# DelphinusLab/halo2-gpu-specific

Hardware: AMD Instinct MI355X
Metric: NTT Fr-ops/s @ k=24 (forward+inverse 2^24 BN254 Fr NTT; MSM G1-adds/s under 'msm') (higher is better)
Workload: dtype u32x8 (254-bit Montgomery, integer)

## Files before the change

### halo2-gpu-specific_amd/csrc/field.hpp

```cpp
#pragma once
#ifdef __HIPCC_RTC__
typedef unsigned char uint8_t;
typedef unsigned short uint16_t;
typedef unsigned int uint32_t;
typedef unsigned long uint64_t;
typedef int int32_t;
typedef long int64_t;
#else
#include <hip/hip_runtime.h>
#include <stdint.h>
#endif

namespace h2 {

struct FrParams {
    static constexpr uint32_t MOD[8] = {0xf0000001u, 0x43e1f593u, 0x79b97091u, 0x2833e848u,
                                        0x8181585du, 0xb85045b6u, 0xe131a029u, 0x30644e72u};
    static constexpr uint32_t MOD2[8] = {0xe0000002u, 0x87c3eb27u, 0xf372e122u, 0x5067d090u,
                                         0x0302b0bau, 0x70a08b6du, 0xc2634053u, 0x60c89ce5u};
    static constexpr uint32_t NMOD[8] = {0x0fffffffu, 0xbc1e0a6cu, 0x86468f6eu, 0xd7cc17b7u,
                                         0x7e7ea7a2u, 0x47afba49u, 0x1ece5fd6u, 0xcf9bb18du};
    static constexpr uint32_t PINV256[8] = {0xefffffffu, 0xc2e1f593u, 0x4c6911b3u, 0x6586864bu,
                                         0x99062391u, 0xe39a9828u, 0x0d8341b2u, 0x73f82f1du};
    static constexpr uint32_t INV = 0xefffffffu;
    static constexpr uint32_t ONE[8] = {0x4ffffffbu, 0xac96341cu, 0x9f60cd29u, 0x36fc7695u,
                                        0x7879462eu, 0x666ea36fu, 0x9a07df2fu, 0x0e0a77c1u};
    static constexpr uint32_t RR[8] = {0xae216da7u, 0x1bb8e645u, 0xe35c59e3u, 0x53fe3ab1u,
                                       0x53bb8085u, 0x8c49833du, 0x7f4e44a5u, 0x0216d0b1u};
};

struct FqParams {
    static constexpr uint32_t MOD[8] = {0xd87cfd47u, 0x3c208c16u, 0x6871ca8du, 0x97816a91u,
                                        0x8181585du, 0xb85045b6u, 0xe131a029u, 0x30644e72u};
    static constexpr uint32_t MOD2[8] = {0xb0f9fa8eu, 0x7841182du, 0xd0e3951au, 0x2f02d522u,
                                         0x0302b0bbu, 0x70a08b6du, 0xc2634053u, 0x60c89ce5u};
    static constexpr uint32_t NMOD[8] = {0x278302b9u, 0xc3df73e9u, 0x978e3572u, 0x687e956eu,
                                         0x7e7ea7a2u, 0x47afba49u, 0x1ece5fd6u, 0xcf9bb18du};
    static constexpr uint32_t PINV256[8] = {0xe4866389u, 0x87d20782u, 0x1eca6ac9u, 0x9ede7d65u,
                                         0x1833da80u, 0xd8afcbd0u, 0x91888c6bu, 0xf57a22b7u};
    static constexpr uint32_t INV = 0xe4866389u;
    static constexpr uint32_t ONE[8] = {0xc58f0d9du, 0xd35d438du, 0xf5c70b3du, 0x0a78eb28u,
                                        0x7879462cu, 0x666ea36fu, 0x9a07df2fu, 0x0e0a77c1u};
    static constexpr uint32_t RR[8] = {0x538afa89u, 0xf32cfc5bu, 0xd44501fbu, 0xb5e71911u,
                                       0x0a417ff6u, 0x47ab1effu, 0xcab8351fu, 0x06d89f71u};
};

template <class P>
struct alignas(16) Fp {
    uint32_t l[8];
};
using Fr = Fp<FrParams>;
using Fq = Fp<FqParams>;

#define H2_DEV __host__ __device__ __forceinline__

template <class P>
H2_DEV Fp<P> fp_load(const Fp<P>* p) {
    const uint4* q = reinterpret_cast<const uint4*>(p);
    uint4 a = q[0], b = q[1];
    Fp<P> r;
    r.l[0] = a.x; r.l[1] = a.y; r.l[2] = a.z; r.l[3] = a.w;
    r.l[4] = b.x; r.l[5] = b.y; r.l[6] = b.z; r.l[7] = b.w;
    return r;
}
template <class P>
H2_DEV void fp_store(Fp<P>* p, const Fp<P>& v) {
    uint4* q = reinterpret_cast<uint4*>(p);
    q[0] = make_uint4(v.l[0], v.l[1], v.l[2], v.l[3]);
    q[1] = make_uint4(v.l[4], v.l[5], v.l[6], v.l[7]);
}

template <class P>
H2_DEV Fp<P> fp_zero() {
    Fp<P> r;
#pragma unroll
    for (int i = 0; i < 8; i++) r.l[i] = 0;
    return r;
}
template <class P>
H2_DEV Fp<P> fp_one() {
    Fp<P> r;
#pragma unroll
    for (int i = 0; i < 8; i++) r.l[i] = P::ONE[i];
    return r;
}
template <class P>
H2_DEV bool fp_is_zero(const Fp<P>& a) {
    uint32_t o = 0;
#pragma unroll
    for (int i = 0; i < 8; i++) o |= a.l[i];
    return o == 0;
}
template <class P>
H2_DEV bool fp_eq(const Fp<P>& a, const Fp<P>& b) {
    uint32_t o = 0;
#pragma unroll
    for (int i = 0; i < 8; i++) o |= a.l[i] ^ b.l[i];
    return o == 0;
}

#if defined(__HIP_DEVICE_COMPILE__) && !defined(H2_PORTABLE_MUL)
#define H2_ASM_CHAINS 1
H2_DEV uint32_t add_co(uint32_t a, uint32_t b, uint64_t& c) {
    uint32_t r;
    asm("v_add_co_u32 %0, %1, %2, %3" : "=v"(r), "=s"(c) : "v"(a), "v"(b));
    return r;
}
H2_DEV uint32_t addc_co(uint32_t a, uint32_t b, uint64_t& c) {
    uint32_t r;
    asm("v_addc_co_u32 %0, %1, %2, %3, %1" : "=v"(r), "+s"(c) : "v"(a), "v"(b));
    return r;
}
H2_DEV uint32_t sub_co(uint32_t a, uint32_t b, uint64_t& c) {
    uint32_t r;
    asm("v_sub_co_u32 %0, %1, %2, %3" : "=v"(r), "=s"(c) : "v"(a), "v"(b));
    return r;
}
H2_DEV uint32_t subb_co(uint32_t a, uint32_t b, uint64_t& c) {
    uint32_t r;
    asm("v_subb_co_u32 %0, %1, %2, %3, %1" : "=v"(r), "+s"(c) : "v"(a), "v"(b));
    return r;
}
H2_DEV uint32_t sel_co(uint32_t y, uint32_t x, uint64_t mask) {
    uint32_t r;
    asm("v_cndmask_b32 %0, %1, %2, %3" : "=v"(r) : "v"(y), "v"(x), "s"(mask));
    return r;
}
#endif

template <class P>
H2_DEV Fp<P> fp_reduce_once(const Fp<P>& a) {
#ifdef H2_ASM_CHAINS
    Fp<P> t, r;
    uint64_t cb;
    t.l[0] = sub_co(a.l[0], P::MOD[0], cb);
#pragma unroll
    for (int i = 1; i < 8; i++) t.l[i] = subb_co(a.l[i], P::MOD[i], cb);
#pragma unroll
    for (int i = 0; i < 8; i++) r.l[i] = sel_co(t.l[i], a.l[i], cb);
    return r;
#else
    Fp<P> d;
    uint64_t borrow = 0;
#pragma unroll
    for (int i = 0; i < 8; i++) {
        uint64_t t = (uint64_t)a.l[i] - P::MOD[i] - borrow;
        d.l[i] = (uint32_t)t;
        borrow = (t >> 32) & 1;
    }
    Fp<P> r;
#pragma unroll
    for (int i = 0; i < 8; i++) r.l[i] = borrow ? a.l[i] : d.l[i];
    return r;
#endif
}

template <class P>
H2_DEV Fp<P> fp_add(const Fp<P>& a, const Fp<P>& b) {
#ifdef H2_ASM_CHAINS
    Fp<P> s, t, r;
    uint64_t ca, cb;
    s.l[0] = add_co(a.l[0], b.l[0], ca);
    s.l[1] = addc_co(a.l[1], b.l[1], ca);
    t.l[0] = sub_co(s.l[0], P::MOD[0], cb);
#pragma unroll
    for (int i = 2; i < 8; i++) {
        s.l[i] = addc_co(a.l[i], b.l[i], ca);
        t.l[i - 1] = subb_co(s.l[i - 1], P::MOD[i - 1], cb);
    }
    t.l[7] = subb_co(s.l[7], P::MOD[7], cb);
#pragma unroll
    for (int i = 0; i < 8; i++) r.l[i] = sel_co(t.l[i], s.l[i], cb);
    return r;
#else
    Fp<P> s;
    uint64_t c = 0;
#pragma unroll
    for (int i = 0; i < 8; i++) {
        c += (uint64_t)a.l[i] + b.l[i];
        s.l[i] = (uint32_t)c;
        c >>= 32;
    }
    return fp_reduce_once(s);
#endif
}

template <class P>
H2_DEV Fp<P> fp_sub(const Fp<P>& a, const Fp<P>& b) {
#ifdef H2_ASM_CHAINS
    Fp<P> d, u, r;
    uint64_t ca, cb;
    d.l[0] = sub_co(a.l[0], b.l[0], ca);
    d.l[1] = subb_co(a.l[1], b.l[1], ca);
    u.l[0] = add_co(d.l[0], P::MOD[0], cb);
#pragma unroll
    for (int i = 2; i < 8; i++) {
        d.l[i] = subb_co(a.l[i], b.l[i], ca);
// ... 7 lines not shown
    Fp<P> d;
    uint64_t borrow = 0;
#pragma unroll
    for (int i = 0; i < 8; i++) {
        uint64_t t = (uint64_t)a.l[i] - b.l[i] - borrow;
        d.l[i] = (uint32_t)t;
        borrow = (t >> 32) & 1;
    }
    uint32_t mask = borrow ? 0xffffffffu : 0u;
    uint64_t c = 0;
    Fp<P> r;
#pragma unroll
    for (int i = 0; i < 8; i++) {
        c += (uint64_t)d.l[i] + (P::MOD[i] & mask);
        r.l[i] = (uint32_t)c;
        c >>= 32;
    }
    return r;
#endif
}

template <class P>
H2_DEV Fp<P> fp_neg(const Fp<P>& a) {
    return fp_sub(fp_zero<P>(), a);
}
template <class P>
H2_DEV Fp<P> fp_dbl(const Fp<P>& a) {
    return fp_add(a, a);
}

template <class P>
H2_DEV Fp<P> fp_lazy_red2p(const Fp<P>& a) {
#ifdef H2_ASM_CHAINS
    Fp<P> t, r;
    uint64_t cb;
    t.l[0] = sub_co(a.l[0], P::MOD2[0], cb);
#pragma unroll
    for (int i = 1; i < 8; i++) t.l[i] = subb_co(a.l[i], P::MOD2[i], cb);
#pragma unroll
    for (int i = 0; i < 8; i++) r.l[i] = sel_co(t.l[i], a.l[i], cb);
    return r;
#else
    Fp<P> d;
    uint64_t borrow = 0;
#pragma unroll
    for (int i = 0; i < 8; i++) {
        uint64_t t = (uint64_t)a.l[i] - P::MOD2[i] - borrow;
        d.l[i] = (uint32_t)t;
        borrow = (t >> 32) & 1;
    }
    Fp<P> r;
#pragma unroll
    for (int i = 0; i < 8; i++) r.l[i] = borrow ? a.l[i] : d.l[i];
    return r;
#endif
}
template <class P>
H2_DEV Fp<P> fp_lazy_add(const Fp<P>& a, const Fp<P>& b) {
    Fp<P> s;
#ifdef H2_ASM_CHAINS
    uint64_t c;
    s.l[0] = add_co(a.l[0], b.l[0], c);
#pragma unroll
    for (int i = 1; i < 8; i++) s.l[i] = addc_co(a.l[i], b.l[i], c);
#else
    uint64_t c = 0;
#pragma unroll
    for (int i = 0; i < 8; i++) {
        c += (uint64_t)a.l[i] + b.l[i];
        s.l[i] = (uint32_t)c;
        c >>= 32;
    }
#endif
    return s;
}
template <class P>
H2_DEV Fp<P> fp_lazy_sub(const Fp<P>& a, const Fp<P>& b) {
    Fp<P> d, u;
#ifdef H2_ASM_CHAINS
    uint64_t ca, cb;
    d.l[0] = sub_co(a.l[0], b.l[0], ca);
    d.l[1] = subb_co(a.l[1], b.l[1], ca);
    u.l[0] = add_co(d.l[0], P::MOD2[0], cb);
#pragma unroll
    for (int i = 2; i < 8; i++) {
        d.l[i] = subb_co(a.l[i], b.l[i], ca);
        u.l[i - 1] = addc_co(d.l[i - 1], P::MOD2[i - 1], cb);
    }
    u.l[7] = addc_co(d.l[7], P::MOD2[7], cb);
#else
    uint64_t borrow = 0, c = 0;
#pragma unroll
    for (int i = 0; i < 8; i++) {
        uint64_t t = (uint64_t)a.l[i] - b.l[i] - borrow;
        d.l[i] = (uint32_t)t;
        borrow = (t >> 32) & 1;
    }
#pragma unroll
    for (int i = 0; i < 8; i++) {
        c += (uint64_t)d.l[i] + P::MOD2[i];
        u.l[i] = (uint32_t)c;
        c >>= 32;
    }
#endif
    return u;
}
template <class P>
H2_DEV Fp<P> fp_lazy_add_red(const Fp<P>& a, const Fp<P>& b) {
#ifdef H2_ASM_CHAINS
    Fp<P> s, t, r;
    uint64_t ca, cb;
    s.l[0] = add_co(a.l[0], b.l[0], ca);
    s.l[1] = addc_co(a.l[1], b.l[1], ca);
    t.l[0] = sub_co(s.l[0], P::MOD2[0], cb);
#pragma unroll
    for (int i = 2; i < 8; i++) {
        s.l[i] = addc_co(a.l[i], b.l[i], ca);
        t.l[i - 1] = subb_co(s.l[i - 1], P::MOD2[i - 1], cb);
    }
    t.l[7] = subb_co(s.l[7], P::MOD2[7], cb);
#pragma unroll
    for (int i = 0; i < 8; i++) r.l[i] = sel_co(t.l[i], s.l[i], cb);
    return r;
#else
    return fp_lazy_red2p(fp_lazy_add(a, b));
#endif
}
template <class P>
H2_DEV Fp<P> fp_lazy_sub_red(const Fp<P>& a, const Fp<P>& b) {
#ifdef H2_ASM_CHAINS
    Fp<P> d, u, r;
    uint64_t ca, cb;
    d.l[0] = sub_co(a.l[0], b.l[0], ca);
    d.l[1] = subb_co(a.l[1], b.l[1], ca);
    u.l[0] = add_co(d.l[0], P::MOD2[0], cb);
#pragma unroll
    for (int i = 2; i < 8; i++) {
        d.l[i] = subb_co(a.l[i], b.l[i], ca);
        u.l[i - 1] = addc_co(d.l[i - 1], P::MOD2[i - 1], cb);
    }
    u.l[7] = addc_co(d.l[7], P::MOD2[7], cb);
#pragma unroll
    for (int i = 0; i < 8; i++) r.l[i] = sel_co(d.l[i], u.l[i], ca);
    return r;
#else
    return fp_lazy_red2p(fp_lazy_sub(a, b));
#endif
}
template <class P>
H2_DEV Fp<P> fp_lazy_canon(const Fp<P>& a) {
    return fp_reduce_once(fp_lazy_red2p(a));
}

H2_DEV void mad_acc(uint64_t& lo, uint32_t& hi, uint32_t a, uint32_t b) {
#if defined(H2_PORTABLE_MUL) || !defined(__HIP_DEVICE_COMPILE__)
    uint64_t p = (uint64_t)a * b;
    uint64_t s = lo + p;
    hi += (s < p) ? 1u : 0u;
    lo = s;
#else
    uint64_t carry;
    asm("v_mad_u64_u32 %0, %1, %2, %3, %0" : "+v"(lo), "=s"(carry) : "v"(a), "v"(b));
    asm("v_addc_co_u32 %0, %1, %0, 0, %1" : "+v"(hi), "+s"(carry));
#endif
}

template <class P>
__device__ __forceinline__ Fp<P> fp_mul_dev(const Fp<P>& a, const Fp<P>& b);
template <class P>
__device__ __forceinline__ Fp<P> fp_sqr_dev(const Fp<P>& a);
template <class P>
__device__ __forceinline__ Fp<P> fp_mul2_dev(const Fp<P>& a, const Fp<P>& b, const Fp<P>& c, const Fp<P>& d);
template <class P>
__device__ __forceinline__ Fp<P> fp_mul_wide_dev(const Fp<P>& a, const Fp<P>& b);
template <class P>
__device__ __forceinline__ Fp<P> fp_mul_const_dev(const Fp<P>& a, const Fp<P>& w, const Fp<P>& wq);
#if defined(__HIP_DEVICE_COMPILE__) && !defined(H2_PORTABLE_MUL)
#include "fp_mul_gen.hpp"
#endif

template <class P>
H2_DEV Fp<P> fp_mul(const Fp<P>& a, const Fp<P>& b) {
#if !defined(__HIP_DEVICE_COMPILE__)
    {
        typedef unsigned __int128 u128;
        uint64_t x[4], y[4], p[4];
        for (int i = 0; i < 4; i++) {
            x[i] = (uint64_t)a.l[2 * i] | ((uint64_t)a.l[2 * i + 1] << 32);
            y[i] = (uint64_t)b.l[2 * i] | ((uint64_t)b.l[2 * i + 1] << 32);
            p[i] = (uint64_t)P::MOD[2 * i] | ((uint64_t)P::MOD[2 * i + 1] << 32);
        }
        uint64_t inv = p[0];
        for (int i = 0; i < 6; i++) inv *= 2 - p[0] * inv;
        inv = 0 - inv;
        uint64_t t[6] = {0, 0, 0, 0, 0, 0};
        for (int i = 0; i < 4; i++) {
            u128 c = 0;
            for (int j = 0; j < 4; j++) {
                c += (u128)t[j] + (u128)x[j] * y[i];
                t[j] = (uint64_t)c;
                c >>= 64;
            }
            c += t[4];
            t[4] = (uint64_t)c;
            t[5] = (uint64_t)(c >> 64);
            const uint64_t m = t[0] * inv;
            c = ((u128)t[0] + (u128)m * p[0]) >> 64;
            for (int j = 1; j < 4; j++) {
                c += (u128)t[j] + (u128)m * p[j];
                t[j - 1] = (uint64_t)c;
                c >>= 64;
            }
            c += t[4];
            t[3] = (uint64_t)c;
            t[4] = t[5] + (uint64_t)(c >> 64);
        }
        Fp<P> r;
        for (int i = 0; i < 4; i++) {
            r.l[2 * i] = (uint32_t)t[i];
            r.l[2 * i + 1] = (uint32_t)(t[i] >> 32);
        }
        return fp_reduce_once(r);
    }
#elif !defined(H2_PORTABLE_MUL)
    return fp_mul_dev(a, b);
#endif
    Fp<P> r;
    uint64_t lo = 0;
    uint32_t hi = 0;
    uint32_t m[8];
#pragma unroll
    for (int i = 0; i < 8; i++) {
#pragma unroll
        for (int j = 0; j <= i; j++) mad_acc(lo, hi, a.l[j], b.l[i - j]);
#pragma unroll
        for (int j = 0; j < i; j++) mad_acc(lo, hi, m[j], P::MOD[i - j]);
        m[i] = (uint32_t)lo * P::INV;
        mad_acc(lo, hi, m[i], P::MOD[0]);
        lo = (lo >> 32) | ((uint64_t)hi << 32);
        hi = 0;
    }
#pragma unroll
    for (int i = 8; i < 16; i++) {
#pragma unroll
        for (int j = i - 7; j < 8; j++) mad_acc(lo, hi, a.l[j], b.l[i - j]);
#pragma unroll
        for (int j = i - 7; j < 8; j++) mad_acc(lo, hi, m[j], P::MOD[i - j]);
        r.l[i - 8] = (uint32_t)lo;
        lo = (lo >> 32) | ((uint64_t)hi << 32);
        hi = 0;
    }
    return fp_reduce_once(r);
}

template <class P>
H2_DEV Fp<P> fp_sqr(const Fp<P>& a) {
#if defined(__HIP_DEVICE_COMPILE__) && !defined(H2_PORTABLE_MUL) && !defined(H2_NO_SQR)
    return fp_sqr_dev(a);
#else
    return fp_mul(a, a);
#endif
}

template <class P>
H2_DEV Fp<P> fp_mul2(const Fp<P>& a, const Fp<P>& b, const Fp<P>& c, const Fp<P>& d) {
#if defined(__HIP_DEVICE_COMPILE__) && !defined(H2_PORTABLE_MUL) && !defined(H2_NO_MUL2)
    return fp_mul2_dev(a, b, c, d);
#else
    return fp_add(fp_mul(a, b), fp_mul(c, d));
#endif
}

template <class P>
H2_DEV Fp<P> fp_mul_wide(const Fp<P>& a, const Fp<P>& b) {
#if defined(__HIP_DEVICE_COMPILE__) && !defined(H2_PORTABLE_MUL)
    return fp_mul_wide_dev(a, b);
#else
    Fp<P> r;
    uint64_t lo = 0;
    uint32_t hi = 0;
    uint32_t m[8];
    for (int i = 0; i < 8; i++) {
        for (int j = 0; j <= i; j++) mad_acc(lo, hi, a.l[j], b.l[i - j]);
        for (int j = 0; j < i; j++) mad_acc(lo, hi, m[j], P::MOD[i - j]);
        m[i] = (uint32_t)lo * P::INV;
        mad_acc(lo, hi, m[i], P::MOD[0]);
        lo = (lo >> 32) | ((uint64_t)hi << 32);
        hi = 0;
    }
    for (int i = 8; i < 16; i++) {
        for (int j = i - 7; j < 8; j++) mad_acc(lo, hi, a.l[j], b.l[i - j]);
        for (int j = i - 7; j < 8; j++) mad_acc(lo, hi, m[j], P::MOD[i - j]);
        r.l[i - 8] = (uint32_t)lo;
        lo = (lo >> 32) | ((uint64_t)hi << 32);
        hi = 0;
    }
    return r;
#endif
}

template <class P>
H2_DEV Fp<P> fp_mul_const(const Fp<P>& x, const Fp<P>& w, const Fp<P>& wq) {
#if defined(__HIP_DEVICE_COMPILE__) && !defined(H2_PORTABLE_MUL)
    Fp<P> r = fp_mul_const_dev(x, w, wq);
    if (__builtin_expect(r.l[7] >= P::MOD2[7], 0)) r = fp_lazy_red2p(r);
    return r;
#else
    uint32_t q[8];
    {
        uint64_t lo = 0;
        uint32_t hi = 0;
        for (int i = 0; i < 15; i++) {
            for (int j = (i > 7 ? i - 7 : 0); j <= (i < 7 ? i : 7); j++) mad_acc(lo, hi, x.l[j], wq.l[i - j]);
            if (i >= 8) q[i - 8] = (uint32_t)lo;
            lo = (lo >> 32) | ((uint64_t)hi << 32);
            hi = 0;
        }
        q[7] = (uint32_t)lo;
    }
    Fp<P> r;
    uint64_t lo = 0;
    uint32_t hi = 0;
    for (int i = 0; i < 8; i++) {
        for (int j = 0; j <= i; j++) {
            mad_acc(lo, hi, x.l[j], w.l[i - j]);
            mad_acc(lo, hi, q[j], P::NMOD[i - j]);
        }
        r.l[i] = (uint32_t)lo;
        lo = (lo >> 32) | ((uint64_t)hi << 32);
        hi = 0;
    }
    return r;
#endif
}
template <class P>
H2_DEV void fp_const_pair(const Fp<P>& w_mont, Fp<P>& w_plain, Fp<P>& wq) {
    w_plain = fp_from_mont(w_mont);
    uint64_t lo = 0;
    uint32_t hi = 0;
    for (int i = 0; i < 8; i++) {
        for (int j = 0; j <= i; j++) mad_acc(lo, hi, w_mont.l[j], P::PINV256[i - j]);
        wq.l[i] = (uint32_t)lo;
        lo = (lo >> 32) | ((uint64_t)hi << 32);
        hi = 0;
    }
}

template <class P>
H2_DEV Fp<P> fp_to_mont(const Fp<P>& canon) {
    Fp<P> rr;
#pragma unroll
    for (int i = 0; i < 8; i++) rr.l[i] = P::RR[i];
    return fp_reduce_once(fp_mul_wide(canon, rr));
}
template <class P>
H2_DEV Fp<P> fp_from_mont(const Fp<P>& a) {
    Fp<P> one = fp_zero<P>();
    one.l[0] = 1;
    return fp_reduce_once(fp_mul_wide(a, one));
}

template <class P>
H2_DEV Fp<P> fp_inv(const Fp<P>& a) {
    uint32_t u[8], v[8], r[8], s[8];
    uint32_t nz = 0;
#pragma unroll
    for (int i = 0; i < 8; i++) {
        u[i] = P::MOD[i];
        v[i] = a.l[i];
        r[i] = 0;
        s[i] = i == 0 ? 1u : 0u;
        nz |= a.l[i];
    }
    if (nz == 0) return a;
    uint32_t k = 0;
    auto halve = [](uint32_t* x) {
#pragma unroll
        for (int i = 0; i < 8; i++) x[i] = (x[i] >> 1) | (i < 7 ? x[i + 1] << 31 : 0u);
    };
    auto dbl = [](uint32_t* x) {
#pragma unroll
        for (int i = 7; i >= 0; i--) x[i] = (x[i] << 1) | (i ? x[i - 1] >> 31 : 0u);
    };
    auto sub = [](uint32_t* x, const uint32_t* y) {
        uint32_t bw = 0;
#pragma unroll
        for (int i = 0; i < 8; i++) {
            const uint32_t d = x[i] - y[i], b1 = x[i] < y[i] ? 1u : 0u, e = d - bw, b2 = d < bw ? 1u : 0u;
            x[i] = e;
            bw = b1 | b2;
        }
    };
    auto add = [](uint32_t* x, const uint32_t* y) {
        uint32_t cy = 0;
#pragma unroll
        for (int i = 0; i < 8; i++) {
            const uint32_t t = x[i] + y[i], c1 = t < y[i] ? 1u : 0u, e = t + cy, c2 = e < cy ? 1u : 0u;
            x[i] = e;
            cy = c1 | c2;
        }
    };
    auto greater = [](const uint32_t* x, const uint32_t* y) {
#pragma unroll
        for (int i = 7; i >= 0; i--)
            if (x[i] != y[i]) return x[i] > y[i];
        return false;
    };
    for (;;) {
        uint32_t vnz = 0;
#pragma unroll
        for (int i = 0; i < 8; i++) vnz |= v[i];
        if (vnz == 0) break;
        if ((u[0] & 1) == 0) {
            halve(u);
            dbl(s);
        } else if ((v[0] & 1) == 0) {
            halve(v);
            dbl(r);
        } else if (greater(u, v)) {
            sub(u, v);
            halve(u);
            add(r, s);
            dbl(s);
        } else {
            sub(v, u);
            halve(v);
            add(s, r);
            dbl(r);
        }
        k++;
    }
    Fp<P> x;
    {
        uint32_t d[8];
        uint64_t bw = 0;
#pragma unroll
        for (int i = 0; i < 8; i++) {
            uint64_t e = (uint64_t)r[i] - P::MOD[i] - bw;
            d[i] = (uint32_t)e;
            bw = (e >> 32) & 1;
        }
        uint64_t bw2 = 0;
#pragma unroll
        for (int i = 0; i < 8; i++) {
            const uint32_t rr = bw ? r[i] : d[i];
            uint64_t e = (uint64_t)P::MOD[i] - rr - bw2;
            x.l[i] = (uint32_t)e;
            bw2 = (e >> 32) & 1;
        }
    }
    x = fp_reduce_once(x);
    for (uint32_t i = k; i < 512; i++) x = fp_dbl(x);
    return x;
}

template <class P>
H2_DEV Fp<P> fp_pow_u32(const Fp<P>& a, uint32_t e) {
    if (e == 0) return fp_one<P>();
    Fp<P> acc = a;
    for (int i = 30 - __builtin_clz(e); i >= 0; i--) {
        acc = fp_sqr(acc);
        if ((e >> i) & 1) acc = fp_mul(acc, a);
    }
    return acc;
}

}
```

### halo2-gpu-specific_amd/csrc/fp_mul_gen.hpp

```cpp

template <>
__device__ __forceinline__ Fp<FrParams> fp_mul_dev<FrParams>(const Fp<FrParams>& a, const Fp<FrParams>& b) {
    using P = FrParams;
    Fp<P> r;
    uint64_t lo = 0, cy0, cy1, cy2;
    uint32_t hi = 0;
    asm("v_mad_u64_u32 %[lo], %[cy0], %[x0], %[x1], %[lo]\n\t"
        : [lo] "+v"(lo), [cy0] "=&s"(cy0)
        : [x0] "v"(a.l[0]), [x1] "v"(b.l[0]));
    const uint32_t m0 = (uint32_t)lo * P::INV;
    asm("v_mad_u64_u32 %[lo], %[cy0], %[x0], %[x1], %[lo]\n\t"
        "s_nop 1\n\t"
        "v_cndmask_b32 %[hi], 0, 1, %[cy0]\n\t"
        : [lo] "+v"(lo), [hi] "=&v"(hi), [cy0] "=&s"(cy0)
        : [x0] "v"(m0), [x1] "s"(P::MOD[0]));
    lo = (lo >> 32) | ((uint64_t)hi << 32);
    asm("v_mad_u64_u32 %[lo], %[cy0], %[x0], %[x1], %[lo]\n\t"
        "v_mad_u64_u32 %[lo], %[cy1], %[x2], %[x3], %[lo]\n\t"
        "v_mad_u64_u32 %[lo], %[cy2], %[x4], %[x5], %[lo]\n\t"
        "s_nop 0\n\t"
        "v_cndmask_b32 %[hi], 0, 1, %[cy1]\n\t"
        "v_addc_co_u32 %[hi], %[cy2], %[hi], 0, %[cy2]\n\t"
        : [lo] "+v"(lo), [hi] "=&v"(hi), [cy0] "=&s"(cy0), [cy1] "=&s"(cy1), [cy2] "=&s"(cy2)
        : [x0] "v"(m0), [x1] "s"(P::MOD[1]), [x2] "v"(a.l[0]), [x3] "v"(b.l[1]), [x4] "v"(a.l[1]), [x5] "v"(b.l[0]));
// ... 1508 lines not shown
        : [x0] "v"(q0), [x1] "s"(P::NMOD[0]), [x2] "v"(a.l[0]), [x3] "v"(b.l[0]));
    r.l[0] = (uint32_t)lo;
    lo = (lo >> 32) | ((uint64_t)hi << 32);
    asm("v_mad_u64_u32 %[lo], %[cy0], %[x0], %[x1], %[lo]\n\t"
        "v_mad_u64_u32 %[lo], %[cy1], %[x2], %[x3], %[lo]\n\t"
        "v_mad_u64_u32 %[lo], %[cy2], %[x4], %[x5], %[lo]\n\t"
        "v_mad_u64_u32 %[lo], %[cy0], %[x6], %[x7], %[lo]\n\t"
        "s_nop 0\n\t"
        "v_cndmask_b32 %[hi], 0, 1, %[cy2]\n\t"
        "v_addc_co_u32 %[hi], %[cy0], %[hi], 0, %[cy0]\n\t"
        : [lo] "+v"(lo), [hi] "=&v"(hi), [cy0] "=&s"(cy0), [cy1] "=&s"(cy1), [cy2] "=&s"(cy2)
        : [x0] "v"(q1), [x1] "s"(P::NMOD[0]), [x2] "v"(q0), [x3] "s"(P::NMOD[1]), [x4] "v"(a.l[0]), [x5] "v"(b.l[1]), [x6] "v"(a.l[1]), [x7] "v"(b.l[0]));
    r.l[1] = (uint32_t)lo;
    lo = (lo >> 32) | ((uint64_t)hi << 32);
    asm("v_mad_u64_u32 %[lo], %[cy0], %[x0], %[x1], %[lo]\n\t"
        "v_mad_u64_u32 %[lo], %[cy1], %[x2], %[x3], %[lo]\n\t"
        "v_mad_u64_u32 %[lo], %[cy2], %[x4], %[x5], %[lo]\n\t"
        "v_mad_u64_u32 %[lo], %[cy0], %[x6], %[x7], %[lo]\n\t"
        "v_mad_u64_u32 %[lo], %[cy1], %[x8], %[x9], %[lo]\n\t"
        "v_cndmask_b32 %[hi], 0, 1, %[cy2]\n\t"
        "v_addc_co_u32 %[hi], %[cy0], %[hi], 0, %[cy0]\n\t"
        "v_addc_co_u32 %[hi], %[cy1], %[hi], 0, %[cy1]\n\t"
        "v_mad_u64_u32 %[lo], %[cy2], %[x10], %[x11], %[lo]\n\t"
        "s_nop 1\n\t"
        "v_addc_co_u32 %[hi], %[cy2], %[hi], 0, %[cy2]\n\t"
        : [lo] "+v"(lo), [hi] "=&v"(hi), [cy0] "=&s"(cy0), [cy1] "=&s"(cy1), [cy2] "=&s"(cy2)
        : [x0] "v"(q2), [x1] "s"(P::NMOD[0]), [x2] "v"(q0), [x3] "s"(P::NMOD[2]), [x4] "v"(q1), [x5] "s"(P::NMOD[1]), [x6] "v"(a.l[0]), [x7] "v"(b.l[2]), [x8] "v"(a.l[1]), [x9] "v"(b.l[1]), [x10] "v"(a.l[2]), [x11] "v"(b.l[0]));
    r.l[2] = (uint32_t)lo;
    lo = (lo >> 32) | ((uint64_t)hi << 32);
    asm("v_mad_u64_u32 %[lo], %[cy0], %[x0], %[x1], %[lo]\n\t"
        "v_mad_u64_u32 %[lo], %[cy1], %[x2], %[x3], %[lo]\n\t"
        "v_mad_u64_u32 %[lo], %[cy2], %[x4], %[x5], %[lo]\n\t"
        "v_mad_u64_u32 %[lo], %[cy0], %[x6], %[x7], %[lo]\n\t"
        "v_mad_u64_u32 %[lo], %[cy1], %[x8], %[x9], %[lo]\n\t"
        "v_cndmask_b32 %[hi], 0, 1, %[cy2]\n\t"
        "v_addc_co_u32 %[hi], %[cy0], %[hi], 0, %[cy0]\n\t"
        "v_addc_co_u32 %[hi], %[cy1], %[hi], 0, %[cy1]\n\t"
        "v_mad_u64_u32 %[lo], %[cy2], %[x10], %[x11], %[lo]\n\t"
        "v_mad_u64_u32 %[lo], %[cy0], %[x12], %[x13], %[lo]\n\t"
        "v_mad_u64_u32 %[lo], %[cy1], %[x14], %[x15], %[lo]\n\t"
        "v_addc_co_u32 %[hi], %[cy2], %[hi], 0, %[cy2]\n\t"
        "v_addc_co_u32 %[hi], %[cy0], %[hi], 0, %[cy0]\n\t"
        "v_addc_co_u32 %[hi], %[cy1], %[hi], 0, %[cy1]\n\t"
        : [lo] "+v"(lo), [hi] "=&v"(hi), [cy0] "=&s"(cy0), [cy1] "=&s"(cy1), [cy2] "=&s"(cy2)
        : [x0] "v"(q3), [x1] "s"(P::NMOD[0]), [x2] "v"(q1), [x3] "s"(P::NMOD[2]), [x4] "v"(q2), [x5] "s"(P::NMOD[1]), [x6] "v"(q0), [x7] "s"(P::NMOD[3]), [x8] "v"(a.l[0]), [x9] "v"(b.l[3]), [x10] "v"(a.l[1]), [x11] "v"(b.l[2]), [x12] "v"(a.l[2]), [x13] "v"(b.l[1]), [x14] "v"(a.l[3]), [x15] "v"(b.l[0]));
    r.l[3] = (uint32_t)lo;
    lo = (lo >> 32) | ((uint64_t)hi << 32);
    asm("v_mad_u64_u32 %[lo], %[cy0], %[x0], %[x1], %[lo]\n\t"
        "v_mad_u64_u32 %[lo], %[cy1], %[x2], %[x3], %[lo]\n\t"
        "v_mad_u64_u32 %[lo], %[cy2], %[x4], %[x5], %[lo]\n\t"
        "v_mad_u64_u32 %[lo], %[cy0], %[x6], %[x7], %[lo]\n\t"
        "v_mad_u64_u32 %[lo], %[cy1], %[x8], %[x9], %[lo]\n\t"
        "v_cndmask_b32 %[hi], 0, 1, %[cy2]\n\t"
        "v_addc_co_u32 %[hi], %[cy0], %[hi], 0, %[cy0]\n\t"
        "v_addc_co_u32 %[hi], %[cy1], %[hi], 0, %[cy1]\n\t"
        "v_mad_u64_u32 %[lo], %[cy2], %[x10], %[x11], %[lo]\n\t"
        "v_mad_u64_u32 %[lo], %[cy0], %[x12], %[x13], %[lo]\n\t"
        "v_mad_u64_u32 %[lo], %[cy1], %[x14], %[x15], %[lo]\n\t"
        "v_addc_co_u32 %[hi], %[cy2], %[hi], 0, %[cy2]\n\t"
        "v_addc_co_u32 %[hi], %[cy0], %[hi], 0, %[cy0]\n\t"
        "v_addc_co_u32 %[hi], %[cy1], %[hi], 0, %[cy1]\n\t"
        "v_mad_u64_u32 %[lo], %[cy2], %[x16], %[x17], %[lo]\n\t"
        "v_mad_u64_u32 %[lo], %[cy0], %[x18], %[x19], %[lo]\n\t"
        "s_nop 0\n\t"
        "v_addc_co_u32 %[hi], %[cy2], %[hi], 0, %[cy2]\n\t"
        "v_addc_co_u32 %[hi], %[cy0], %[hi], 0, %[cy0]\n\t"
        : [lo] "+v"(lo), [hi] "=&v"(hi), [cy0] "=&s"(cy0), [cy1] "=&s"(cy1), [cy2] "=&s"(cy2)
        : [x0] "v"(q4), [x1] "s"(P::NMOD[0]), [x2] "v"(q0), [x3] "s"(P::NMOD[4]), [x4] "v"(q2), [x5] "s"(P::NMOD[2]), [x6] "v"(q3), [x7] "s"(P::NMOD[1]), [x8] "v"(q1), [x9] "s"(P::NMOD[3]), [x10] "v"(a.l[0]), [x11] "v"(b.l[4]), [x12] "v"(a.l[1]), [x13] "v"(b.l[3]), [x14] "v"(a.l[2]), [x15] "v"(b.l[2]), [x16] "v"(a.l[3]), [x17] "v"(b.l[1]), [x18] "v"(a.l[4]), [x19] "v"(b.l[0]));
    r.l[4] = (uint32_t)lo;
    lo = (lo >> 32) | ((uint64_t)hi << 32);
    asm("v_mad_u64_u32 %[lo], %[cy0], %[x0], %[x1], %[lo]\n\t"
        "v_mad_u64_u32 %[lo], %[cy1], %[x2], %[x3], %[lo]\n\t"
        "v_mad_u64_u32 %[lo], %[cy2], %[x4], %[x5], %[lo]\n\t"
        "v_mad_u64_u32 %[lo], %[cy0], %[x6], %[x7], %[lo]\n\t"
        "v_mad_u64_u32 %[lo], %[cy1], %[x8], %[x9], %[lo]\n\t"
        "v_mad_u64_u32 %[lo], %[cy2], %[x10], %[x11], %[lo]\n\t"
        "v_cndmask_b32 %[hi], 0, 1, %[cy0]\n\t"
        "v_addc_co_u32 %[hi], %[cy1], %[hi], 0, %[cy1]\n\t"
        "v_addc_co_u32 %[hi], %[cy2], %[hi], 0, %[cy2]\n\t"
        "v_mad_u64_u32 %[lo], %[cy0], %[x12], %[x13], %[lo]\n\t"
        "v_mad_u64_u32 %[lo], %[cy1], %[x14], %[x15], %[lo]\n\t"
        "v_mad_u64_u32 %[lo], %[cy2], %[x16], %[x17], %[lo]\n\t"
        "v_addc_co_u32 %[hi], %[cy0], %[hi], 0, %[cy0]\n\t"
        "v_addc_co_u32 %[hi], %[cy1], %[hi], 0, %[cy1]\n\t"
        "v_addc_co_u32 %[hi], %[cy2], %[hi], 0, %[cy2]\n\t"
        "v_mad_u64_u32 %[lo], %[cy0], %[x18], %[x19], %[lo]\n\t"
        "v_mad_u64_u32 %[lo], %[cy1], %[x20], %[x21], %[lo]\n\t"
        "v_mad_u64_u32 %[lo], %[cy2], %[x22], %[x23], %[lo]\n\t"
        "v_addc_co_u32 %[hi], %[cy0], %[hi], 0, %[cy0]\n\t"
        "v_addc_co_u32 %[hi], %[cy1], %[hi], 0, %[cy1]\n\t"
        "v_addc_co_u32 %[hi], %[cy2], %[hi], 0, %[cy2]\n\t"
        : [lo] "+v"(lo), [hi] "=&v"(hi), [cy0] "=&s"(cy0), [cy1] "=&s"(cy1), [cy2] "=&s"(cy2)
        : [x0] "v"(q5), [x1] "s"(P::NMOD[0]), [x2] "v"(q0), [x3] "s"(P::NMOD[5]), [x4] "v"(q1), [x5] "s"(P::NMOD[4]), [x6] "v"(q3), [x7] "s"(P::NMOD[2]), [x8] "v"(q4), [x9] "s"(P::NMOD[1]), [x10] "v"(q2), [x11] "s"(P::NMOD[3]), [x12] "v"(a.l[0]), [x13] "v"(b.l[5]), [x14] "v"(a.l[1]), [x15] "v"(b.l[4]), [x16] "v"(a.l[2]), [x17] "v"(b.l[3]), [x18] "v"(a.l[3]), [x19] "v"(b.l[2]), [x20] "v"(a.l[4]), [x21] "v"(b.l[1]), [x22] "v"(a.l[5]), [x23] "v"(b.l[0]));
    r.l[5] = (uint32_t)lo;
    lo = (lo >> 32) | ((uint64_t)hi << 32);
    asm("v_mad_u64_u32 %[lo], %[cy0], %[x0], %[x1], %[lo]\n\t"
        "v_mad_u64_u32 %[lo], %[cy1], %[x2], %[x3], %[lo]\n\t"
        "v_mad_u64_u32 %[lo], %[cy2], %[x4], %[x5], %[lo]\n\t"
        "v_mad_u64_u32 %[lo], %[cy0], %[x6], %[x7], %[lo]\n\t"
        "v_mad_u64_u32 %[lo], %[cy1], %[x8], %[x9], %[lo]\n\t"
        "v_mad_u64_u32 %[lo], %[cy2], %[x10], %[x11], %[lo]\n\t"
        "v_mad_u64_u32 %[lo], %[cy0], %[x12], %[x13], %[lo]\n\t"
        "v_cndmask_b32 %[hi], 0, 1, %[cy1]\n\t"
        "v_addc_co_u32 %[hi], %[cy2], %[hi], 0, %[cy2]\n\t"
        "v_addc_co_u32 %[hi], %[cy0], %[hi], 0, %[cy0]\n\t"
        "v_mad_u64_u32 %[lo], %[cy1], %[x14], %[x15], %[lo]\n\t"
        "v_mad_u64_u32 %[lo], %[cy2], %[x16], %[x17], %[lo]\n\t"
        "v_mad_u64_u32 %[lo], %[cy0], %[x18], %[x19], %[lo]\n\t"
        "v_addc_co_u32 %[hi], %[cy1], %[hi], 0, %[cy1]\n\t"
        "v_addc_co_u32 %[hi], %[cy2], %[hi], 0, %[cy2]\n\t"
        "v_addc_co_u32 %[hi], %[cy0], %[hi], 0, %[cy0]\n\t"
        "v_mad_u64_u32 %[lo], %[cy1], %[x20], %[x21], %[lo]\n\t"
        "v_mad_u64_u32 %[lo], %[cy2], %[x22], %[x23], %[lo]\n\t"
        "s_nop 0\n\t"
        "v_addc_co_u32 %[hi], %[cy1], %[hi], 0, %[cy1]\n\t"
        "v_addc_co_u32 %[hi], %[cy2], %[hi], 0, %[cy2]\n\t"
        : [lo] "+v"(lo), [hi] "=&v"(hi), [cy0] "=&s"(cy0), [cy1] "=&s"(cy1), [cy2] "=&s"(cy2)
        : [x0] "v"(q6), [x1] "s"(P::NMOD[0]), [x2] "v"(q0), [x3] "s"(P::NMOD[6]), [x4] "v"(q1), [x5] "s"(P::NMOD[5]), [x6] "v"(q2), [x7] "s"(P::NMOD[4]), [x8] "v"(q4), [x9] "s"(P::NMOD[2]), [x10] "v"(q5), [x11] "s"(P::NMOD[1]), [x12] "v"(q3), [x13] "s"(P::NMOD[3]), [x14] "v"(a.l[0]), [x15] "v"(b.l[6]), [x16] "v"(a.l[1]), [x17] "v"(b.l[5]), [x18] "v"(a.l[2]), [x19] "v"(b.l[4]), [x20] "v"(a.l[3]), [x21] "v"(b.l[3]), [x22] "v"(a.l[4]), [x23] "v"(b.l[2]));
    asm("v_mad_u64_u32 %[lo], %[cy0], %[x0], %[x1], %[lo]\n\t"
        "v_mad_u64_u32 %[lo], %[cy1], %[x2], %[x3], %[lo]\n\t"
        "s_nop 0\n\t"
        "v_addc_co_u32 %[hi], %[cy0], %[hi], 0, %[cy0]\n\t"
        "v_addc_co_u32 %[hi], %[cy1], %[hi], 0, %[cy1]\n\t"
        : [lo] "+v"(lo), [hi] "+v"(hi), [cy0] "=&s"(cy0), [cy1] "=&s"(cy1)
        : [x0] "v"(a.l[5]), [x1] "v"(b.l[1]), [x2] "v"(a.l[6]), [x3] "v"(b.l[0]));
    r.l[6] = (uint32_t)lo;
    lo = (lo >> 32) | ((uint64_t)hi << 32);
    asm("v_mad_u64_u32 %[lo], %[cy0], %[x0], %[x1], %[lo]\n\t"
        "v_mad_u64_u32 %[lo], %[cy1], %[x2], %[x3], %[lo]\n\t"
        "v_mad_u64_u32 %[lo], %[cy2], %[x4], %[x5], %[lo]\n\t"
        "v_mad_u64_u32 %[lo], %[cy0], %[x6], %[x7], %[lo]\n\t"
        "v_mad_u64_u32 %[lo], %[cy1], %[x8], %[x9], %[lo]\n\t"
        "v_mad_u64_u32 %[lo], %[cy2], %[x10], %[x11], %[lo]\n\t"
        "v_mad_u64_u32 %[lo], %[cy0], %[x12], %[x13], %[lo]\n\t"
        "v_mad_u64_u32 %[lo], %[cy1], %[x14], %[x15], %[lo]\n\t"
        "v_mad_u64_u32 %[lo], %[cy2], %[x16], %[x17], %[lo]\n\t"
        "v_mad_u64_u32 %[lo], %[cy0], %[x18], %[x19], %[lo]\n\t"
        "v_mad_u64_u32 %[lo], %[cy1], %[x20], %[x21], %[lo]\n\t"
        "v_mad_u64_u32 %[lo], %[cy2], %[x22], %[x23], %[lo]\n\t"
        : [lo] "+v"(lo), [cy0] "=&s"(cy0), [cy1] "=&s"(cy1), [cy2] "=&s"(cy2)
        : [x0] "v"(q7), [x1] "s"(P::NMOD[0]), [x2] "v"(q1), [x3] "s"(P::NMOD[6]), [x4] "v"(a.l[0]), [x5] "v"(b.l[7]), [x6] "v"(q2), [x7] "s"(P::NMOD[5]), [x8] "v"(q3), [x9] "s"(P::NMOD[4]), [x10] "v"(q5), [x11] "s"(P::NMOD[2]), [x12] "v"(q6), [x13] "s"(P::NMOD[1]), [x14] "v"(q0), [x15] "s"(P::NMOD[7]), [x16] "v"(q4), [x17] "s"(P::NMOD[3]), [x18] "v"(a.l[1]), [x19] "v"(b.l[6]), [x20] "v"(a.l[2]), [x21] "v"(b.l[5]), [x22] "v"(a.l[3]), [x23] "v"(b.l[4]));
    asm("v_mad_u64_u32 %[lo], %[cy0], %[x0], %[x1], %[lo]\n\t"
        "v_mad_u64_u32 %[lo], %[cy1], %[x2], %[x3], %[lo]\n\t"
        "v_mad_u64_u32 %[lo], %[cy2], %[x4], %[x5], %[lo]\n\t"
        "v_mad_u64_u32 %[lo], %[cy0], %[x6], %[x7], %[lo]\n\t"
        : [lo] "+v"(lo), [cy0] "=&s"(cy0), [cy1] "=&s"(cy1), [cy2] "=&s"(cy2)
        : [x0] "v"(a.l[4]), [x1] "v"(b.l[3]), [x2] "v"(a.l[5]), [x3] "v"(b.l[2]), [x4] "v"(a.l[6]), [x5] "v"(b.l[1]), [x6] "v"(a.l[7]), [x7] "v"(b.l[0]));
    r.l[7] = (uint32_t)lo;
    (void)cy0; (void)cy1; (void)cy2; (void)hi;
    return r;
}

template <>
__device__ __forceinline__ Fp<FqParams> fp_mul_dev<FqParams>(const Fp<FqParams>& a, const Fp<FqParams>& b) {
    using P = FqParams;
    Fp<P> r;
    uint64_t lo = 0, cy0, cy1, cy2;
    uint32_t hi = 0;
    asm("v_mad_u64_u32 %[lo], %[cy0], %[x0], %[x1], %[lo]\n\t"
        : [lo] "+v"(lo), [cy0] "=&s"(cy0)
        : [x0] "v"(a.l[0]), [x1] "v"(b.l[0]));
    const uint32_t m0 = (uint32_t)lo * P::INV;
    asm("v_mad_u64_u32 %[lo], %[cy0], %[x0], %[x1], %[lo]\n\t"
        "s_nop 1\n\t"
        "v_cndmask_b32 %[hi], 0, 1, %[cy0]\n\t"
        : [lo] "+v"(lo), [hi] "=&v"(hi), [cy0] "=&s"(cy0)
        : [x0] "v"(m0), [x1] "s"(P::MOD[0]));
    lo = (lo >> 32) | ((uint64_t)hi << 32);
    asm("v_mad_u64_u32 %[lo], %[cy0], %[x0], %[x1], %[lo]\n\t"
        "v_mad_u64_u32 %[lo], %[cy1], %[x2], %[x3], %[lo]\n\t"
        "v_mad_u64_u32 %[lo], %[cy2], %[x4], %[x5], %[lo]\n\t"
        "s_nop 0\n\t"
        "v_cndmask_b32 %[hi], 0, 1, %[cy1]\n\t"
        "v_addc_co_u32 %[hi], %[cy2], %[hi], 0, %[cy2]\n\t"
        : [lo] "+v"(lo), [hi] "=&v"(hi), [cy0] "=&s"(cy0), [cy1] "=&s"(cy1), [cy2] "=&s"(cy2)
        : [x0] "v"(m0), [x1] "s"(P::MOD[1]), [x2] "v"(a.l[0]), [x3] "v"(b.l[1]), [x4] "v"(a.l[1]), [x5] "v"(b.l[0]));
    const uint32_t m1 = (uint32_t)lo * P::INV;
    asm("v_mad_u64_u32 %[lo], %[cy0], %[x0], %[x1], %[lo]\n\t"
        "s_nop 1\n\t"
        "v_addc_co_u32 %[hi], %[cy0], %[hi], 0, %[cy0]\n\t"
        : [lo] "+v"(lo), [hi] "+v"(hi), [cy0] "=&s"(cy0)
        : [x0] "v"(m1), [x1] "s"(P::MOD[0]));
    lo = (lo >> 32) | ((uint64_t)hi << 32);
    asm("v_mad_u64_u32 %[lo], %[cy0], %[x0], %[x1], %[lo]\n\t"
        "v_mad_u64_u32 %[lo], %[cy1], %[x2], %[x3], %[lo]\n\t"
        "v_mad_u64_u32 %[lo], %[cy2], %[x4], %[x5], %[lo]\n\t"
        "v_mad_u64_u32 %[lo], %[cy0], %[x6], %[x7], %[lo]\n\t"
        "v_mad_u64_u32 %[lo], %[cy1], %[x8], %[x9], %[lo]\n\t"
        "v_cndmask_b32 %[hi], 0, 1, %[cy2]\n\t"
        "v_addc_co_u32 %[hi], %[cy0], %[hi], 0, %[cy0]\n\t"
        "v_addc_co_u32 %[hi], %[cy1], %[hi], 0, %[cy1]\n\t"
        : [lo] "+v"(lo), [hi] "=&v"(hi), [cy0] "=&s"(cy0), [cy1] "=&s"(cy1), [cy2] "=&s"(cy2)
        : [x0] "v"(m1), [x1] "s"(P::MOD[1]), [x2] "v"(m0), [x3] "s"(P::MOD[2]), [x4] "v"(a.l[0]), [x5] "v"(b.l[2]), [x6] "v"(a.l[1]), [x7] "v"(b.l[1]), [x8] "v"(a.l[2]), [x9] "v"(b.l[0]));
    const uint32_t m2 = (uint32_t)lo * P::INV;
    asm("v_mad_u64_u32 %[lo], %[cy0], %[x0], %[x1], %[lo]\n\t"
        "s_nop 1\n\t"
        "v_addc_co_u32 %[hi], %[cy0], %[hi], 0, %[cy0]\n\t"
        : [lo] "+v"(lo), [hi] "+v"(hi), [cy0] "=&s"(cy0)
        : [x0] "v"(m2), [x1] "s"(P::MOD[0]));
    lo = (lo >> 32) | ((uint64_t)hi << 32);
    asm("v_mad_u64_u32 %[lo], %[cy0], %[x0], %[x1], %[lo]\n\t"
        "v_mad_u64_u32 %[lo], %[cy1], %[x2], %[x3], %[lo]\n\t"
        "v_mad_u64_u32 %[lo], %[cy2], %[x4], %[x5], %[lo]\n\t"
        "v_mad_u64_u32 %[lo], %[cy0], %[x6], %[x7], %[lo]\n\t"
        "v_mad_u64_u32 %[lo], %[cy1], %[x8], %[x9], %[lo]\n\t"
        "v_cndmask_b32 %[hi], 0, 1, %[cy2]\n\t"
        "v_addc_co_u32 %[hi], %[cy0], %[hi], 0, %[cy0]\n\t"
        "v_addc_co_u32 %[hi], %[cy1], %[hi], 0, %[cy1]\n\t"
        "v_mad_u64_u32 %[lo], %[cy2], %[x10], %[x11], %[lo]\n\t"
        "v_mad_u64_u32 %[lo], %[cy0], %[x12], %[x13], %[lo]\n\t"
        "s_nop 0\n\t"
        "v_addc_co_u32 %[hi], %[cy2], %[hi], 0, %[cy2]\n\t"
        "v_addc_co_u32 %[hi], %[cy0], %[hi], 0, %[cy0]\n\t"
        : [lo] "+v"(lo), [hi] "=&v"(hi), [cy0] "=&s"(cy0), [cy1] "=&s"(cy1), [cy2] "=&s"(cy2)
        : [x0] "v"(m2), [x1] "s"(P::MOD[1]), [x2] "v"(m1), [x3] "s"(P::MOD[2]), [x4] "v"(m0), [x5] "s"(P::MOD[3]), [x6] "v"(a.l[0]), [x7] "v"(b.l[3]), [x8] "v"(a.l[1]), [x9] "v"(b.l[2]), [x10] "v"(a.l[2]), [x11] "v"(b.l[1]), [x12] "v"(a.l[3]), [x13] "v"(b.l[0]));
    const uint32_t m3 = (uint32_t)lo * P::INV;
    asm("v_mad_u64_u32 %[lo], %[cy0], %[x0], %[x1], %[lo]\n\t"
        "s_nop 1\n\t"
        "v_addc_co_u32 %[hi], %[cy0], %[hi], 0, %[cy0]\n\t"
        : [lo] "+v"(lo), [hi] "+v"(hi), [cy0] "=&s"(cy0)
        : [x0] "v"(m3), [x1] "s"(P::MOD[0]));
    lo = (lo >> 32) | ((uint64_t)hi << 32);
    asm("v_mad_u64_u32 %[lo], %[cy0], %[x0], %[x1], %[lo]\n\t"
        "v_mad_u64_u32 %[lo], %[cy1], %[x2], %[x3], %[lo]\n\t"
        "v_mad_u64_u32 %[lo], %[cy2], %[x4], %[x5], %[lo]\n\t"
        "v_mad_u64_u32 %[lo], %[cy0], %[x6], %[x7], %[lo]\n\t"
        "v_mad_u64_u32 %[lo], %[cy1], %[x8], %[x9], %[lo]\n\t"
        "v_cndmask_b32 %[hi], 0, 1, %[cy2]\n\t"
        "v_addc_co_u32 %[hi], %[cy0], %[hi], 0, %[cy0]\n\t"
        "v_addc_co_u32 %[hi], %[cy1], %[hi], 0, %[cy1]\n\t"
        "v_mad_u64_u32 %[lo], %[cy2], %[x10], %[x11], %[lo]\n\t"
        "v_mad_u64_u32 %[lo], %[cy0], %[x12], %[x13], %[lo]\n\t"
        "v_mad_u64_u32 %[lo], %[cy1], %[x14], %[x15], %[lo]\n\t"
        "v_addc_co_u32 %[hi], %[cy2], %[hi], 0, %[cy2]\n\t"
        "v_addc_co_u32 %[hi], %[cy0], %[hi], 0, %[cy0]\n\t"
        "v_addc_co_u32 %[hi], %[cy1], %[hi], 0, %[cy1]\n\t"
        "v_mad_u64_u32 %[lo], %[cy2], %[x16], %[x17], %[lo]\n\t"
        "s_nop 1\n\t"
        "v_addc_co_u32 %[hi], %[cy2], %[hi], 0, %[cy2]\n\t"
        : [lo] "+v"(lo), [hi] "=&v"(hi), [cy0] "=&s"(cy0), [cy1] "=&s"(cy1), [cy2] "=&s"(cy2)
        : [x0] "v"(m3), [x1] "s"(P::MOD[1]), [x2] "v"(m2), [x3] "s"(P::MOD[2]), [x4] "v"(m0), [x5] "s"(P::MOD[4]), [x6] "v"(m1), [x7] "s"(P::MOD[3]), [x8] "v"(a.l[0]), [x9] "v"(b.l[4]), [x10] "v"(a.l[1]), [x11] "v"(b.l[3]), [x12] "v"(a.l[2]), [x13] "v"(b.l[2]), [x14] "v"(a.l[3]), [x15] "v"(b.l[1]), [x16] "v"(a.l[4]), [x17] "v"(b.l[0]));
    const uint32_t m4 = (uint32_t)lo * P::INV;
    asm("v_mad_u64_u32 %[lo], %[cy0], %[x0], %[x1], %[lo]\n\t"
        "s_nop 1\n\t"
        "v_addc_co_u32 %[hi], %[cy0], %[hi], 0, %[cy0]\n\t"
        : [lo] "+v"(lo), [hi] "+v"(hi), [cy0] "=&s"(cy0)
        : [x0] "v"(m4), [x1] "s"(P::MOD[0]));
    lo = (lo >> 32) | ((uint64_t)hi << 32);
    asm("v_mad_u64_u32 %[lo], %[cy0], %[x0], %[x1], %[lo]\n\t"
        "v_mad_u64_u32 %[lo], %[cy1], %[x2], %[x3], %[lo]\n\t"
        "v_mad_u64_u32 %[lo], %[cy2], %[x4], %[x5], %[lo]\n\t"
        "v_mad_u64_u32 %[lo], %[cy0], %[x6], %[x7], %[lo]\n\t"
        "v_mad_u64_u32 %[lo], %[cy1], %[x8], %[x9], %[lo]\n\t"
        "v_cndmask_b32 %[hi], 0, 1, %[cy2]\n\t"
        "v_addc_co_u32 %[hi], %[cy0], %[hi], 0, %[cy0]\n\t"
        "v_addc_co_u32 %[hi], %[cy1], %[hi], 0, %[cy1]\n\t"
        "v_mad_u64_u32 %[lo], %[cy2], %[x10], %[x11], %[lo]\n\t"
        "v_mad_u64_u32 %[lo], %[cy0], %[x12], %[x13], %[lo]\n\t"
        "v_mad_u64_u32 %[lo], %[cy1], %[x14], %[x15], %[lo]\n\t"
        "v_addc_co_u32 %[hi], %[cy2], %[hi], 0, %[cy2]\n\t"
        "v_addc_co_u32 %[hi], %[cy0], %[hi], 0, %[cy0]\n\t"
        "v_addc_co_u32 %[hi], %[cy1], %[hi], 0, %[cy1]\n\t"
        "v_mad_u64_u32 %[lo], %[cy2], %[x16], %[x17], %[lo]\n\t"
        "v_mad_u64_u32 %[lo], %[cy0], %[x18], %[x19], %[lo]\n\t"
        "v_mad_u64_u32 %[lo], %[cy1], %[x20], %[x21], %[lo]\n\t"
        "v_addc_co_u32 %[hi], %[cy2], %[hi], 0, %[cy2]\n\t"
        "v_addc_co_u32 %[hi], %[cy0], %[hi], 0, %[cy0]\n\t"
        "v_addc_co_u32 %[hi], %[cy1], %[hi], 0, %[cy1]\n\t"
        : [lo] "+v"(lo), [hi] "=&v"(hi), [cy0] "=&s"(cy0), [cy1] "=&s"(cy1), [cy2] "=&s"(cy2)
        : [x0] "v"(m4), [x1] "s"(P::MOD[1]), [x2] "v"(m3), [x3] "s"(P::MOD[2]), [x4] "v"(m1), [x5] "s"(P::MOD[4]), [x6] "v"(m2), [x7] "s"(P::MOD[3]), [x8] "v"(m0), [x9] "s"(P::MOD[5]), [x10] "v"(a.l[0]), [x11] "v"(b.l[5]), [x12] "v"(a.l[1]), [x13] "v"(b.l[4]), [x14] "v"(a.l[2]), [x15] "v"(b.l[3]), [x16] "v"(a.l[3]), [x17] "v"(b.l[2]), [x18] "v"(a.l[4]), [x19] "v"(b.l[1]), [x20] "v"(a.l[5]), [x21] "v"(b.l[0]));
    const uint32_t m5 = (uint32_t)lo * P::INV;
    asm("v_mad_u64_u32 %[lo], %[cy0], %[x0], %[x1], %[lo]\n\t"
        "s_nop 1\n\t"
        "v_addc_co_u32 %[hi], %[cy0], %[hi], 0, %[cy0]\n\t"
        : [lo] "+v"(lo), [hi] "+v"(hi), [cy0] "=&s"(cy0)
        : [x0] "v"(m5), [x1] "s"(P::MOD[0]));
    lo = (lo >> 32) | ((uint64_t)hi << 32);
    asm("v_mad_u64_u32 %[lo], %[cy0], %[x0], %[x1], %[lo]\n\t"
        "v_mad_u64_u32 %[lo], %[cy1], %[x2], %[x3], %[lo]\n\t"
        "v_mad_u64_u32 %[lo], %[cy2], %[x4], %[x5], %[lo]\n\t"
        "v_mad_u64_u32 %[lo], %[cy0], %[x6], %[x7], %[lo]\n\t"
        "v_mad_u64_u32 %[lo], %[cy1], %[x8], %[x9], %[lo]\n\t"
        "v_cndmask_b32 %[hi], 0, 1, %[cy2]\n\t"
        "v_addc_co_u32 %[hi], %[cy0], %[hi], 0, %[cy0]\n\t"
        "v_addc_co_u32 %[hi], %[cy1], %[hi], 0, %[cy1]\n\t"
        "v_mad_u64_u32 %[lo], %[cy2], %[x10], %[x11], %[lo]\n\t"
        "v_mad_u64_u32 %[lo], %[cy0], %[x12], %[x13], %[lo]\n\t"
        "v_mad_u64_u32 %[lo], %[cy1], %[x14], %[x15], %[lo]\n\t"
        "v_addc_co_u32 %[hi], %[cy2], %[hi], 0, %[cy2]\n\t"
        "v_addc_co_u32 %[hi], %[cy0], %[hi], 0, %[cy0]\n\t"
        "v_addc_co_u32 %[hi], %[cy1], %[hi], 0, %[cy1]\n\t"
        "v_mad_u64_u32 %[lo], %[cy2], %[x16], %[x17], %[lo]\n\t"
        "v_mad_u64_u32 %[lo], %[cy0], %[x18], %[x19], %[lo]\n\t"
        "v_mad_u64_u32 %[lo], %[cy1], %[x20], %[x21], %[lo]\n\t"
        "v_addc_co_u32 %[hi], %[cy2], %[hi], 0, %[cy2]\n\t"
        "v_addc_co_u32 %[hi], %[cy0], %[hi], 0, %[cy0]\n\t"
        "v_addc_co_u32 %[hi], %[cy1], %[hi], 0, %[cy1]\n\t"
        "v_mad_u64_u32 %[lo], %[cy2], %[x22], %[x23], %[lo]\n\t"
        "s_nop 1\n\t"
        "v_addc_co_u32 %[hi], %[cy2], %[hi], 0, %[cy2]\n\t"
        : [lo] "+v"(lo), [hi] "=&v"(hi), [cy0] "=&s"(cy0), [cy1] "=&s"(cy1), [cy2] "=&s"(cy2)
        : [x0] "v"(m5), [x1] "s"(P::MOD[1]), [x2] "v"(m4), [x3] "s"(P::MOD[2]), [x4] "v"(m2), [x5] "s"(P::MOD[4]), [x6] "v"(m3), [x7] "s"(P::MOD[3]), [x8] "v"(m1), [x9] "s"(P::MOD[5]), [x10] "v"(m0), [x11] "s"(P::MOD[6]), [x12] "v"(a.l[0]), [x13] "v"(b.l[6]), [x14] "v"(a.l[1]), [x15] "v"(b.l[5]), [x16] "v"(a.l[2]), [x17] "v"(b.l[4]), [x18] "v"(a.l[3]), [x19] "v"(b.l[3]), [x20] "v"(a.l[4]), [x21] "v"(b.l[2]), [x22] "v"(a.l[5]), [x23] "v"(b.l[1]));
    asm("v_mad_u64_u32 %[lo], %[cy0], %[x0], %[x1], %[lo]\n\t"
        "s_nop 1\n\t"
        "v_addc_co_u32 %[hi], %[cy0], %[hi], 0, %[cy0]\n\t"
        : [lo] "+v"(lo), [hi] "+v"(hi), [cy0] "=&s"(cy0)
// ... 1398 lines not shown
        "v_cndmask_b32 %[hi], 0, 1, %[cy1]\n\t"
        : [lo] "+v"(lo), [hi] "=&v"(hi), [cy0] "=&s"(cy0), [cy1] "=&s"(cy1)
        : [x0] "v"(q0), [x1] "s"(P::NMOD[0]), [x2] "v"(a.l[0]), [x3] "v"(b.l[0]));
    r.l[0] = (uint32_t)lo;
    lo = (lo >> 32) | ((uint64_t)hi << 32);
    asm("v_mad_u64_u32 %[lo], %[cy0], %[x0], %[x1], %[lo]\n\t"
        "v_mad_u64_u32 %[lo], %[cy1], %[x2], %[x3], %[lo]\n\t"
        "v_mad_u64_u32 %[lo], %[cy2], %[x4], %[x5], %[lo]\n\t"
        "v_mad_u64_u32 %[lo], %[cy0], %[x6], %[x7], %[lo]\n\t"
        "s_nop 0\n\t"
        "v_cndmask_b32 %[hi], 0, 1, %[cy2]\n\t"
        "v_addc_co_u32 %[hi], %[cy0], %[hi], 0, %[cy0]\n\t"
        : [lo] "+v"(lo), [hi] "=&v"(hi), [cy0] "=&s"(cy0), [cy1] "=&s"(cy1), [cy2] "=&s"(cy2)
        : [x0] "v"(q1), [x1] "s"(P::NMOD[0]), [x2] "v"(q0), [x3] "s"(P::NMOD[1]), [x4] "v"(a.l[0]), [x5] "v"(b.l[1]), [x6] "v"(a.l[1]), [x7] "v"(b.l[0]));
    r.l[1] = (uint32_t)lo;
    lo = (lo >> 32) | ((uint64_t)hi << 32);
    asm("v_mad_u64_u32 %[lo], %[cy0], %[x0], %[x1], %[lo]\n\t"
        "v_mad_u64_u32 %[lo], %[cy1], %[x2], %[x3], %[lo]\n\t"
        "v_mad_u64_u32 %[lo], %[cy2], %[x4], %[x5], %[lo]\n\t"
        "v_mad_u64_u32 %[lo], %[cy0], %[x6], %[x7], %[lo]\n\t"
        "v_mad_u64_u32 %[lo], %[cy1], %[x8], %[x9], %[lo]\n\t"
        "v_cndmask_b32 %[hi], 0, 1, %[cy2]\n\t"
        "v_addc_co_u32 %[hi], %[cy0], %[hi], 0, %[cy0]\n\t"
        "v_addc_co_u32 %[hi], %[cy1], %[hi], 0, %[cy1]\n\t"
        "v_mad_u64_u32 %[lo], %[cy2], %[x10], %[x11], %[lo]\n\t"
        "s_nop 1\n\t"
        "v_addc_co_u32 %[hi], %[cy2], %[hi], 0, %[cy2]\n\t"
        : [lo] "+v"(lo), [hi] "=&v"(hi), [cy0] "=&s"(cy0), [cy1] "=&s"(cy1), [cy2] "=&s"(cy2)
        : [x0] "v"(q2), [x1] "s"(P::NMOD[0]), [x2] "v"(q0), [x3] "s"(P::NMOD[2]), [x4] "v"(q1), [x5] "s"(P::NMOD[1]), [x6] "v"(a.l[0]), [x7] "v"(b.l[2]), [x8] "v"(a.l[1]), [x9] "v"(b.l[1]), [x10] "v"(a.l[2]), [x11] "v"(b.l[0]));
    r.l[2] = (uint32_t)lo;
    lo = (lo >> 32) | ((uint64_t)hi << 32);
    asm("v_mad_u64_u32 %[lo], %[cy0], %[x0], %[x1], %[lo]\n\t"
        "v_mad_u64_u32 %[lo], %[cy1], %[x2], %[x3], %[lo]\n\t"
        "v_mad_u64_u32 %[lo], %[cy2], %[x4], %[x5], %[lo]\n\t"
        "v_mad_u64_u32 %[lo], %[cy0], %[x6], %[x7], %[lo]\n\t"
        "v_mad_u64_u32 %[lo], %[cy1], %[x8], %[x9], %[lo]\n\t"
        "v_cndmask_b32 %[hi], 0, 1, %[cy2]\n\t"
        "v_addc_co_u32 %[hi], %[cy0], %[hi], 0, %[cy0]\n\t"
        "v_addc_co_u32 %[hi], %[cy1], %[hi], 0, %[cy1]\n\t"
        "v_mad_u64_u32 %[lo], %[cy2], %[x10], %[x11], %[lo]\n\t"
        "v_mad_u64_u32 %[lo], %[cy0], %[x12], %[x13], %[lo]\n\t"
        "v_mad_u64_u32 %[lo], %[cy1], %[x14], %[x15], %[lo]\n\t"
        "v_addc_co_u32 %[hi], %[cy2], %[hi], 0, %[cy2]\n\t"
        "v_addc_co_u32 %[hi], %[cy0], %[hi], 0, %[cy0]\n\t"
        "v_addc_co_u32 %[hi], %[cy1], %[hi], 0, %[cy1]\n\t"
        : [lo] "+v"(lo), [hi] "=&v"(hi), [cy0] "=&s"(cy0), [cy1] "=&s"(cy1), [cy2] "=&s"(cy2)
        : [x0] "v"(q3), [x1] "s"(P::NMOD[0]), [x2] "v"(q0), [x3] "s"(P::NMOD[3]), [x4] "v"(q1), [x5] "s"(P::NMOD[2]), [x6] "v"(q2), [x7] "s"(P::NMOD[1]), [x8] "v"(a.l[0]), [x9] "v"(b.l[3]), [x10] "v"(a.l[1]), [x11] "v"(b.l[2]), [x12] "v"(a.l[2]), [x13] "v"(b.l[1]), [x14] "v"(a.l[3]), [x15] "v"(b.l[0]));
    r.l[3] = (uint32_t)lo;
    lo = (lo >> 32) | ((uint64_t)hi << 32);
    asm("v_mad_u64_u32 %[lo], %[cy0], %[x0], %[x1], %[lo]\n\t"
        "v_mad_u64_u32 %[lo], %[cy1], %[x2], %[x3], %[lo]\n\t"
        "v_mad_u64_u32 %[lo], %[cy2], %[x4], %[x5], %[lo]\n\t"
        "v_mad_u64_u32 %[lo], %[cy0], %[x6], %[x7], %[lo]\n\t"
        "v_mad_u64_u32 %[lo], %[cy1], %[x8], %[x9], %[lo]\n\t"
        "v_cndmask_b32 %[hi], 0, 1, %[cy2]\n\t"
        "v_addc_co_u32 %[hi], %[cy0], %[hi], 0, %[cy0]\n\t"
        "v_addc_co_u32 %[hi], %[cy1], %[hi], 0, %[cy1]\n\t"
        "v_mad_u64_u32 %[lo], %[cy2], %[x10], %[x11], %[lo]\n\t"
        "v_mad_u64_u32 %[lo], %[cy0], %[x12], %[x13], %[lo]\n\t"
        "v_mad_u64_u32 %[lo], %[cy1], %[x14], %[x15], %[lo]\n\t"
        "v_addc_co_u32 %[hi], %[cy2], %[hi], 0, %[cy2]\n\t"
        "v_addc_co_u32 %[hi], %[cy0], %[hi], 0, %[cy0]\n\t"
        "v_addc_co_u32 %[hi], %[cy1], %[hi], 0, %[cy1]\n\t"
        "v_mad_u64_u32 %[lo], %[cy2], %[x16], %[x17], %[lo]\n\t"
        "v_mad_u64_u32 %[lo], %[cy0], %[x18], %[x19], %[lo]\n\t"
        "s_nop 0\n\t"
        "v_addc_co_u32 %[hi], %[cy2], %[hi], 0, %[cy2]\n\t"
        "v_addc_co_u32 %[hi], %[cy0], %[hi], 0, %[cy0]\n\t"
        : [lo] "+v"(lo), [hi] "=&v"(hi), [cy0] "=&s"(cy0), [cy1] "=&s"(cy1), [cy2] "=&s"(cy2)
        : [x0] "v"(q4), [x1] "s"(P::NMOD[0]), [x2] "v"(q1), [x3] "s"(P::NMOD[3]), [x4] "v"(q0), [x5] "s"(P::NMOD[4]), [x6] "v"(q2), [x7] "s"(P::NMOD[2]), [x8] "v"(q3), [x9] "s"(P::NMOD[1]), [x10] "v"(a.l[0]), [x11] "v"(b.l[4]), [x12] "v"(a.l[1]), [x13] "v"(b.l[3]), [x14] "v"(a.l[2]), [x15] "v"(b.l[2]), [x16] "v"(a.l[3]), [x17] "v"(b.l[1]), [x18] "v"(a.l[4]), [x19] "v"(b.l[0]));
    r.l[4] = (uint32_t)lo;
    lo = (lo >> 32) | ((uint64_t)hi << 32);
    asm("v_mad_u64_u32 %[lo], %[cy0], %[x0], %[x1], %[lo]\n\t"
        "v_mad_u64_u32 %[lo], %[cy1], %[x2], %[x3], %[lo]\n\t"
        "v_mad_u64_u32 %[lo], %[cy2], %[x4], %[x5], %[lo]\n\t"
        "v_mad_u64_u32 %[lo], %[cy0], %[x6], %[x7], %[lo]\n\t"
        "v_mad_u64_u32 %[lo], %[cy1], %[x8], %[x9], %[lo]\n\t"
        "v_mad_u64_u32 %[lo], %[cy2], %[x10], %[x11], %[lo]\n\t"
        "v_cndmask_b32 %[hi], 0, 1, %[cy0]\n\t"
        "v_addc_co_u32 %[hi], %[cy1], %[hi], 0, %[cy1]\n\t"
        "v_addc_co_u32 %[hi], %[cy2], %[hi], 0, %[cy2]\n\t"
        "v_mad_u64_u32 %[lo], %[cy0], %[x12], %[x13], %[lo]\n\t"
        "v_mad_u64_u32 %[lo], %[cy1], %[x14], %[x15], %[lo]\n\t"
        "v_mad_u64_u32 %[lo], %[cy2], %[x16], %[x17], %[lo]\n\t"
        "v_addc_co_u32 %[hi], %[cy0], %[hi], 0, %[cy0]\n\t"
        "v_addc_co_u32 %[hi], %[cy1], %[hi], 0, %[cy1]\n\t"
        "v_addc_co_u32 %[hi], %[cy2], %[hi], 0, %[cy2]\n\t"
        "v_mad_u64_u32 %[lo], %[cy0], %[x18], %[x19], %[lo]\n\t"
        "v_mad_u64_u32 %[lo], %[cy1], %[x20], %[x21], %[lo]\n\t"
        "v_mad_u64_u32 %[lo], %[cy2], %[x22], %[x23], %[lo]\n\t"
        "v_addc_co_u32 %[hi], %[cy0], %[hi], 0, %[cy0]\n\t"
        "v_addc_co_u32 %[hi], %[cy1], %[hi], 0, %[cy1]\n\t"
        "v_addc_co_u32 %[hi], %[cy2], %[hi], 0, %[cy2]\n\t"
        : [lo] "+v"(lo), [hi] "=&v"(hi), [cy0] "=&s"(cy0), [cy1] "=&s"(cy1), [cy2] "=&s"(cy2)
        : [x0] "v"(q5), [x1] "s"(P::NMOD[0]), [x2] "v"(q0), [x3] "s"(P::NMOD[5]), [x4] "v"(q2), [x5] "s"(P::NMOD[3]), [x6] "v"(q1), [x7] "s"(P::NMOD[4]), [x8] "v"(q3), [x9] "s"(P::NMOD[2]), [x10] "v"(q4), [x11] "s"(P::NMOD[1]), [x12] "v"(a.l[0]), [x13] "v"(b.l[5]), [x14] "v"(a.l[1]), [x15] "v"(b.l[4]), [x16] "v"(a.l[2]), [x17] "v"(b.l[3]), [x18] "v"(a.l[3]), [x19] "v"(b.l[2]), [x20] "v"(a.l[4]), [x21] "v"(b.l[1]), [x22] "v"(a.l[5]), [x23] "v"(b.l[0]));
    r.l[5] = (uint32_t)lo;
    lo = (lo >> 32) | ((uint64_t)hi << 32);
    asm("v_mad_u64_u32 %[lo], %[cy0], %[x0], %[x1], %[lo]\n\t"
        "v_mad_u64_u32 %[lo], %[cy1], %[x2], %[x3], %[lo]\n\t"
        "v_mad_u64_u32 %[lo], %[cy2], %[x4], %[x5], %[lo]\n\t"
        "v_mad_u64_u32 %[lo], %[cy0], %[x6], %[x7], %[lo]\n\t"
        "v_mad_u64_u32 %[lo], %[cy1], %[x8], %[x9], %[lo]\n\t"
        "v_mad_u64_u32 %[lo], %[cy2], %[x10], %[x11], %[lo]\n\t"
        "v_mad_u64_u32 %[lo], %[cy0], %[x12], %[x13], %[lo]\n\t"
        "v_cndmask_b32 %[hi], 0, 1, %[cy1]\n\t"
        "v_addc_co_u32 %[hi], %[cy2], %[hi], 0, %[cy2]\n\t"
        "v_addc_co_u32 %[hi], %[cy0], %[hi], 0, %[cy0]\n\t"
        "v_mad_u64_u32 %[lo], %[cy1], %[x14], %[x15], %[lo]\n\t"
        "v_mad_u64_u32 %[lo], %[cy2], %[x16], %[x17], %[lo]\n\t"
        "v_mad_u64_u32 %[lo], %[cy0], %[x18], %[x19], %[lo]\n\t"
        "v_addc_co_u32 %[hi], %[cy1], %[hi], 0, %[cy1]\n\t"
        "v_addc_co_u32 %[hi], %[cy2], %[hi], 0, %[cy2]\n\t"
        "v_addc_co_u32 %[hi], %[cy0], %[hi], 0, %[cy0]\n\t"
        "v_mad_u64_u32 %[lo], %[cy1], %[x20], %[x21], %[lo]\n\t"
        "v_mad_u64_u32 %[lo], %[cy2], %[x22], %[x23], %[lo]\n\t"
        "s_nop 0\n\t"
        "v_addc_co_u32 %[hi], %[cy1], %[hi], 0, %[cy1]\n\t"
        "v_addc_co_u32 %[hi], %[cy2], %[hi], 0, %[cy2]\n\t"
        : [lo] "+v"(lo), [hi] "=&v"(hi), [cy0] "=&s"(cy0), [cy1] "=&s"(cy1), [cy2] "=&s"(cy2)
        : [x0] "v"(q0), [x1] "s"(P::NMOD[6]), [x2] "v"(q6), [x3] "s"(P::NMOD[0]), [x4] "v"(q1), [x5] "s"(P::NMOD[5]), [x6] "v"(q3), [x7] "s"(P::NMOD[3]), [x8] "v"(q2), [x9] "s"(P::NMOD[4]), [x10] "v"(q4), [x11] "s"(P::NMOD[2]), [x12] "v"(q5), [x13] "s"(P::NMOD[1]), [x14] "v"(a.l[0]), [x15] "v"(b.l[6]), [x16] "v"(a.l[1]), [x17] "v"(b.l[5]), [x18] "v"(a.l[2]), [x19] "v"(b.l[4]), [x20] "v"(a.l[3]), [x21] "v"(b.l[3]), [x22] "v"(a.l[4]), [x23] "v"(b.l[2]));
    asm("v_mad_u64_u32 %[lo], %[cy0], %[x0], %[x1], %[lo]\n\t"
        "v_mad_u64_u32 %[lo], %[cy1], %[x2], %[x3], %[lo]\n\t"
        "s_nop 0\n\t"
        "v_addc_co_u32 %[hi], %[cy0], %[hi], 0, %[cy0]\n\t"
        "v_addc_co_u32 %[hi], %[cy1], %[hi], 0, %[cy1]\n\t"
        : [lo] "+v"(lo), [hi] "+v"(hi), [cy0] "=&s"(cy0), [cy1] "=&s"(cy1)
        : [x0] "v"(a.l[5]), [x1] "v"(b.l[1]), [x2] "v"(a.l[6]), [x3] "v"(b.l[0]));
    r.l[6] = (uint32_t)lo;
    lo = (lo >> 32) | ((uint64_t)hi << 32);
    asm("v_mad_u64_u32 %[lo], %[cy0], %[x0], %[x1], %[lo]\n\t"
        "v_mad_u64_u32 %[lo], %[cy1], %[x2], %[x3], %[lo]\n\t"
        "v_mad_u64_u32 %[lo], %[cy2], %[x4], %[x5], %[lo]\n\t"
        "v_mad_u64_u32 %[lo], %[cy0], %[x6], %[x7], %[lo]\n\t"
        "v_mad_u64_u32 %[lo], %[cy1], %[x8], %[x9], %[lo]\n\t"
        "v_mad_u64_u32 %[lo], %[cy2], %[x10], %[x11], %[lo]\n\t"
        "v_mad_u64_u32 %[lo], %[cy0], %[x12], %[x13], %[lo]\n\t"
        "v_mad_u64_u32 %[lo], %[cy1], %[x14], %[x15], %[lo]\n\t"
        "v_mad_u64_u32 %[lo], %[cy2], %[x16], %[x17], %[lo]\n\t"
        "v_mad_u64_u32 %[lo], %[cy0], %[x18], %[x19], %[lo]\n\t"
        "v_mad_u64_u32 %[lo], %[cy1], %[x20], %[x21], %[lo]\n\t"
        "v_mad_u64_u32 %[lo], %[cy2], %[x22], %[x23], %[lo]\n\t"
        : [lo] "+v"(lo), [cy0] "=&s"(cy0), [cy1] "=&s"(cy1), [cy2] "=&s"(cy2)
        : [x0] "v"(q1), [x1] "s"(P::NMOD[6]), [x2] "v"(q7), [x3] "s"(P::NMOD[0]), [x4] "v"(a.l[0]), [x5] "v"(b.l[7]), [x6] "v"(q2), [x7] "s"(P::NMOD[5]), [x8] "v"(q4), [x9] "s"(P::NMOD[3]), [x10] "v"(q3), [x11] "s"(P::NMOD[4]), [x12] "v"(q5), [x13] "s"(P::NMOD[2]), [x14] "v"(q6), [x15] "s"(P::NMOD[1]), [x16] "v"(q0), [x17] "s"(P::NMOD[7]), [x18] "v"(a.l[1]), [x19] "v"(b.l[6]), [x20] "v"(a.l[2]), [x21] "v"(b.l[5]), [x22] "v"(a.l[3]), [x23] "v"(b.l[4]));
    asm("v_mad_u64_u32 %[lo], %[cy0], %[x0], %[x1], %[lo]\n\t"
        "v_mad_u64_u32 %[lo], %[cy1], %[x2], %[x3], %[lo]\n\t"
        "v_mad_u64_u32 %[lo], %[cy2], %[x4], %[x5], %[lo]\n\t"
        "v_mad_u64_u32 %[lo], %[cy0], %[x6], %[x7], %[lo]\n\t"
        : [lo] "+v"(lo), [cy0] "=&s"(cy0), [cy1] "=&s"(cy1), [cy2] "=&s"(cy2)
        : [x0] "v"(a.l[4]), [x1] "v"(b.l[3]), [x2] "v"(a.l[5]), [x3] "v"(b.l[2]), [x4] "v"(a.l[6]), [x5] "v"(b.l[1]), [x6] "v"(a.l[7]), [x7] "v"(b.l[0]));
    r.l[7] = (uint32_t)lo;
    (void)cy0; (void)cy1; (void)cy2; (void)hi;
    return r;
}
```

### halo2-gpu-specific_amd/csrc/ntt.hip

```cpp
#include <algorithm>
#include <cstdlib>

#include "common.hpp"
#include "ntt.hpp"

namespace h2 {

static constexpr int NTT_BATCH_MAX = 16;
static constexpr int LO_BITS = 12;

__device__ __forceinline__ void tw_store(Fr* out, uint32_t i, const Fr& w_mont, uint32_t pair) {
    if (!pair) {
        fp_store(out + i, w_mont);
        return;
    }
    Fr w, q;
    fp_const_pair(w_mont, w, q);
    fp_store(out + 2 * (size_t)i, w);
    fp_store(out + 2 * (size_t)i + 1, q);
}

__global__ void __launch_bounds__(256) k_pow_table(Fr* out, Fr base, uint32_t mul, uint32_t count, uint32_t pair) {
    uint32_t i = blockIdx.x * blockDim.x + threadIdx.x;
    if (i >= count) return;
    tw_store(out, i, fp_pow_u32(base, i * mul), pair);
}

__global__ void __launch_bounds__(256) k_direct_table(Fr* out, Fr base, uint32_t kbits, uint32_t s_log, uint32_t log_n,
                                                      uint32_t count, uint32_t pair) {
    uint32_t i = blockIdx.x * blockDim.x + threadIdx.x;
    if (i >= count) return;
    uint32_t rho = i >> kbits, K = i & ((1u << kbits) - 1);
    uint32_t e = (uint32_t)(((uint64_t)rho * K) << s_log) & ((1u << log_n) - 1);
    tw_store(out, i, fp_pow_u32(base, e), pair);
}

__global__ void __launch_bounds__(256) k_last_table(Fr* out, Fr base, uint32_t bits, uint32_t log_n, Fr d, uint32_t scale,
                                                    uint32_t pair) {
    const uint32_t i = blockIdx.x * blockDim.x + threadIdx.x;
    const uint32_t rho = i & ((1u << bits) - 1), K = i >> bits;
    const uint32_t e = (uint32_t)((uint64_t)rho * K) & ((1u << log_n) - 1);
    Fr w = fp_pow_u32(base, e);
    if (scale) w = fp_mul(w, d);
    tw_store(out, i, w, pair);
}

__global__ void __launch_bounds__(256) k_scale_table(Fr* out, const Fr* in, Fr d, uint32_t count) {
    uint32_t i = blockIdx.x * blockDim.x + threadIdx.x;
    if (i < count) fp_store(out + i, fp_mul(fp_load(in + i), d));
}

struct PassArgs {
    const Fr* in;
    Fr* out;
    const Fr* tw_bfly;
    const Fr* tw_lo;
    const Fr* tw_hi;
    const Fr* tw_direct;
    uint32_t direct_kmajor;
    uint32_t hi_scaled;
    Fr pre3[3];
    Fr post3[3];
    uint32_t has_pre3, has_post3, post3_uniform;
    uint32_t log_n, B, s_log, t_log;
    uint32_t nprev;
    uint32_t prevB[4];
    uint32_t prevT[4];
    uint32_t is_last, in_len, log_c;
    const Fr* sc_lo;
    const Fr* sc_hi;
    uint32_t scale_mode;
    uint32_t batch;
    const Fr* in_b[NTT_BATCH_MAX];
    Fr* out_b[NTT_BATCH_MAX];
    uint32_t zskip;
    uint32_t radix4;
};

__device__ __forceinline__ uint32_t bitrev(uint32_t x, uint32_t bits) {
    return bits == 0 ? 0u : (__brev(x) >> (32 - bits));
}

__device__ __forceinline__ uint32_t hi_to_K(uint32_t hi, const PassArgs& a) {
    uint32_t K = 0;
    for (int q = (int)a.nprev - 1; q >= 0; q--) {
        uint32_t d = hi & ((1u << a.prevB[q]) - 1);
        hi >>= a.prevB[q];
        K |= d << a.prevT[q];
    }
    return K;
}
__device__ __forceinline__ uint32_t K_to_hi(uint32_t K, const PassArgs& a) {
    uint32_t hi = 0;
    for (uint32_t q = 0; q < a.nprev; q++) {
        uint32_t d = (K >> a.prevT[q]) & ((1u << a.prevB[q]) - 1);
        hi = (hi << a.prevB[q]) | d;
    }
    return hi;
}

__device__ __forceinline__ Fr twiddle_pow(const PassArgs& a, uint32_t e) {
    if (a.log_n <= LO_BITS) return fp_load(a.tw_lo + e);
    Fr lo = fp_load(a.tw_lo + (e & ((1u << LO_BITS) - 1)));
    Fr hi = fp_load(a.tw_hi + (e >> LO_BITS));
    return fp_mul(lo, hi);
}

extern __shared__ __attribute__((aligned(16))) uint4 h2_smem[];

__device__ __forceinline__ Fr lds_get(const uint4* lo, const uint4* hi, uint32_t i) {
    uint4 a = lo[i], b = hi[i];
    Fr r;
    r.l[0] = a.x; r.l[1] = a.y; r.l[2] = a.z; r.l[3] = a.w;
    r.l[4] = b.x; r.l[5] = b.y; r.l[6] = b.z; r.l[7] = b.w;
    return r;
}
__device__ __forceinline__ void lds_put(uint4* lo, uint4* hi, uint32_t i, const Fr& v) {
    lo[i] = make_uint4(v.l[0], v.l[1], v.l[2], v.l[3]);
    hi[i] = make_uint4(v.l[4], v.l[5], v.l[6], v.l[7]);
}

template <bool RADIX4, bool DP = false>
__global__ void __launch_bounds__(512, 4) k_ntt_pass(PassArgs a) {
    constexpr bool CW = RADIX4;
    static_assert(!DP || CW, "pairs in tw_direct only next to pairs in tw_bfly");
    auto tmul = [](const Fr& x, const Fr& w) -> Fr { return fp_mul_wide(x, w); };
    const uint32_t B = a.B, R = 1u << B, log_c = a.log_c, C = 1u << log_c;
    const uint32_t zskip = a.zskip;
    uint4* t_lo = h2_smem;
    uint4* t_hi = t_lo + (R << log_c);
    uint4* w_lo = t_hi + (R << log_c);
    uint4* w_hi = w_lo + (R >> 1) + (CW ? 0 : 1);
    uint4* q_lo = w_hi + (R >> 1);
    uint4* q_hi = q_lo + (R >> 1);
    struct Tw {
        Fr w, q;
    };
    auto tw_get = [&](uint32_t i) __attribute__((always_inline)) -> Tw {
        Tw t;
        t.w = lds_get(w_lo, w_hi, i);
        if constexpr (CW) t.q = lds_get(q_lo, q_hi, i);
        return t;
    };
    auto bmul = [](const Fr& x, const Tw& t) __attribute__((always_inline)) -> Fr {
        if constexpr (CW) return fp_mul_const(x, t.w, t.q);
        else return fp_mul_wide(x, t.w);
    };
    const uint32_t nthreads = blockDim.x;
    const uint32_t tid = threadIdx.x;
    const Fr* const in_p = a.batch ? a.in_b[blockIdx.y] : a.in;
    Fr* const out_p = a.batch ? a.out_b[blockIdx.y] : a.out;
    const uint32_t n_mask = (a.log_n >= 32) ? 0xffffffffu : ((1u << a.log_n) - 1);

    for (uint32_t i = tid; i < (R >> 1); i += nthreads) {
        if constexpr (CW) {
            lds_put(w_lo, w_hi, i, fp_load(a.tw_bfly + 2 * i));
            lds_put(q_lo, q_hi, i, fp_load(a.tw_bfly + 2 * i + 1));
        } else {
            lds_put(w_lo, w_hi, i, fp_load(a.tw_bfly + i));
        }
    }

    const uint32_t tile_id = blockIdx.x;
    const uint32_t total = R << log_c;

    uint32_t base = 0, K_uniform = 0;
    const uint32_t S = 1u << a.s_log;
    if (!a.is_last) {
        uint32_t chunks_per_hi = S >> log_c;
        uint32_t hi = tile_id / chunks_per_hi, lo0 = (tile_id % chunks_per_hi) << log_c;
        base = (hi << (B + a.s_log)) + lo0;
        K_uniform = hi_to_K(hi, a);
    }

    constexpr uint32_t NE = RADIX4 ? 4 : 2;
    for (uint32_t e0 = tid; e0 < total; e0 += NE * nthreads) {
        uint32_t rho[NE], col[NE], idx[NE], Kk[NE];
        bool live[NE];
        Fr x[NE];
#pragma unroll
        for (uint32_t q = 0; q < NE; q++) {
            const uint32_t e = e0 + q * nthreads;
            if (!a.is_last) {
                col[q] = e & (C - 1);
                rho[q] = (e >> log_c) & (R - 1);
                idx[q] = base + (rho[q] << a.s_log) + col[q];
                Kk[q] = K_uniform;
            } else {
                rho[q] = e & (R - 1);
                col[q] = (e >> B) & (C - 1);
                Kk[q] = (tile_id << log_c) + col[q];
                idx[q] = (K_to_hi(Kk[q], a) << B) + rho[q];
            }
            live[q] = e < total && !(zskip && rho[q] >= (R >> zskip));
        }
#pragma unroll
        for (uint32_t q = 0; q < NE; q++) {
            x[q] = fp_zero<FrParams>();
            if (live[q] && idx[q] < a.in_len) x[q] = fp_load(in_p + idx[q]);
        }
        if (a.has_pre3) {
#pragma unroll
            for (uint32_t q = 0; q < NE; q++) {
                const uint32_t m = idx[q] % 3;
                Fr w;
#pragma unroll
                for (int l = 0; l < 8; l++) w.l[l] = m == 1 ? a.pre3[1].l[l] : a.pre3[2].l[l];
                if (m != 0) x[q] = tmul(x[q], w);
// ... 24 lines not shown
#pragma unroll
                for (uint32_t q = 0; q < NE; q++) {
                    const uint32_t ex = (uint32_t)(((uint64_t)rho[q] * Kk[q]) << a.s_log) & n_mask;
                    x[q] = tmul(x[q], fp_load(a.tw_lo + ex));
                }
            } else {
                const Fr* const two_lo = pre_scale ? a.sc_lo : a.tw_lo;
                const Fr* const two_hi = pre_scale ? a.sc_hi : a.tw_hi;
#pragma unroll
                for (uint32_t q0 = 0; q0 < NE; q0 += 2) {
                    Fr wl[2], wh[2];
#pragma unroll
                    for (uint32_t q = 0; q < 2; q++) {
                        const uint32_t ex = pre_scale ? (idx[q0 + q] & n_mask)
                                                      : ((uint32_t)(((uint64_t)rho[q0 + q] * Kk[q0 + q]) << a.s_log) & n_mask);
                        wl[q] = fp_load(two_lo + (ex & ((1u << LO_BITS) - 1)));
                        wh[q] = fp_load(two_hi + (ex >> LO_BITS));
                    }
#pragma unroll
                    for (uint32_t q = 0; q < 2; q++) x[q0 + q] = tmul(x[q0 + q], fp_mul(wl[q], wh[q]));
                }
            }
        }
#pragma unroll
        for (uint32_t q = 0; q < NE; q++) {
            const uint32_t e = e0 + q * nthreads;
            const uint32_t r_q = a.is_last ? (e & (R - 1)) : ((e >> log_c) & (R - 1));
            const uint32_t c_q = a.is_last ? ((e >> B) & (C - 1)) : (e & (C - 1));
            if (e >= total || (zskip && r_q >= (R >> zskip))) continue;
            if (zskip) {
                for (uint32_t m = 0; m < (1u << zskip); m++) lds_put(t_lo, t_hi, ((bitrev(r_q, B) | m) << log_c) + c_q, x[q]);
            } else {
                lds_put(t_lo, t_hi, (bitrev(r_q, B) << log_c) + c_q, x[q]);
            }
        }
    }
    __syncthreads();

    uint32_t s0 = zskip;
    if constexpr (RADIX4) {
        const uint32_t nunits = total >> 2;
        auto round4 = [&](const uint32_t s) __attribute__((always_inline)) {
            const uint32_t h = 1u << s;
            const uint32_t log_per = (B - 2 + log_c) - s;
            const bool by_r = s != 0 && log_per >= 6 && (nthreads & 63) == 0;
            for (uint32_t t = tid; t < nunits; t += nthreads) {
                uint32_t c, r, p;
                if (by_r) {
                    r = t >> log_per;
                    const uint32_t j = t & ((1u << log_per) - 1);
                    c = j & (C - 1);
                    p = ((j >> log_c) << (s + 2)) | r;
                } else {
                    c = t & (C - 1);
                    const uint32_t b = t >> log_c;
                    r = b & (h - 1);
                    p = ((b >> s) << (s + 2)) | r;
                }
                const uint32_t i0 = (p << log_c) + c, step = h << log_c;
                Fr x0 = lds_get(t_lo, t_hi, i0), x1 = lds_get(t_lo, t_hi, i0 + step);
                Fr x2 = lds_get(t_lo, t_hi, i0 + 2 * step), x3 = lds_get(t_lo, t_hi, i0 + 3 * step);
                const bool unit = s == 0 || (by_r && r == 0);
                x0 = fp_lazy_red2p(x0);
                x2 = fp_lazy_red2p(x2);
                if (!unit) {
                    const Tw wa = tw_get(r << (B - 1 - s));
                    x1 = bmul(x1, wa);
                    x3 = bmul(x3, wa);
                } else {
                    x1 = fp_lazy_red2p(x1);
                    x3 = fp_lazy_red2p(x3);
                }
                const Fr y0 = fp_lazy_add_red(x0, x1), y1 = fp_lazy_sub_red(x0, x1);
                Fr y2 = fp_lazy_add(x2, x3), y3 = fp_lazy_sub(x2, x3);
                y2 = unit ? fp_lazy_red2p(y2) : bmul(y2, tw_get(r << (B - 2 - s)));
                y3 = bmul(y3, tw_get((r + h) << (B - 2 - s)));
                lds_put(t_lo, t_hi, i0, fp_lazy_add(y0, y2));
                lds_put(t_lo, t_hi, i0 + 2 * step, fp_lazy_sub(y0, y2));
                lds_put(t_lo, t_hi, i0 + step, fp_lazy_add(y1, y3));
                lds_put(t_lo, t_hi, i0 + 3 * step, fp_lazy_sub(y1, y3));
            }
            __syncthreads();
        };
        for (; s0 + 1 < B; s0 += 2) round4(s0);
    }
    const uint32_t nbf = total >> 1;
    for (uint32_t s = s0; s < B; s++) {
        const uint32_t h = 1u << s;
        const uint32_t log_per = (B - 1 + log_c) - s;
        const bool by_r = s != 0 && log_per >= 6 && (nthreads & 63) == 0;
        for (uint32_t t = tid; t < nbf; t += nthreads) {
            uint32_t c, r, i;
            if (by_r) {
                r = t >> log_per;
                uint32_t j = t & ((1u << log_per) - 1);
                c = j & (C - 1);
                i = ((j >> log_c) << (s + 1)) | r;
            } else {
                c = t & (C - 1);
                uint32_t b = t >> log_c;
                r = b & (h - 1);
                i = ((b >> s) << (s + 1)) | r;
            }
            const uint32_t iu = (i << log_c) + c, iv = ((i + h) << log_c) + c;
            Fr u = lds_get(t_lo, t_hi, iu), v = lds_get(t_lo, t_hi, iv);
            const bool skip = s == 0 || (by_r && r == 0);
            u = fp_lazy_red2p(u);
            v = skip ? fp_lazy_red2p(v) : bmul(v, tw_get(r << (B - 1 - s)));
            lds_put(t_lo, t_hi, iu, fp_lazy_add(u, v));
            lds_put(t_lo, t_hi, iv, fp_lazy_sub(u, v));
        }
        __syncthreads();
    }

    for (uint32_t e0 = tid; e0 < total; e0 += NE * nthreads) {
        Fr y[NE];
        uint32_t idx[NE];
#pragma unroll
        for (uint32_t q = 0; q < NE; q++) {
            const uint32_t e = e0 + q * nthreads;
            const uint32_t c = e & (C - 1), k = (e >> log_c) & (R - 1);
            if (!a.is_last)
                idx[q] = base + (k << a.s_log) + c;
            else
                idx[q] = ((tile_id << log_c) + c) + (k << a.t_log);
            y[q] = lds_get(t_lo, t_hi, (k << log_c) + c);
        }
        if (a.is_last && a.scale_mode == 2u) {
#pragma unroll
            for (uint32_t q = 0; q < NE; q++) {
                const uint32_t i = idx[q] & n_mask;
                const Fr w = fp_mul(fp_load(a.sc_lo + (i & ((1u << LO_BITS) - 1))), fp_load(a.sc_hi + (i >> LO_BITS)));
                y[q] = fp_reduce_once(fp_mul_wide(y[q], w));
            }
        } else if (a.is_last && a.has_post3 && !a.hi_scaled) {
#pragma unroll
            for (uint32_t q = 0; q < NE; q++) {
                const uint32_t m = idx[q] % 3;
                Fr w;
#pragma unroll
                for (int l = 0; l < 8; l++) w.l[l] = m == 0 ? a.post3[0].l[l] : (m == 1 ? a.post3[1].l[l] : a.post3[2].l[l]);
                y[q] = fp_reduce_once(fp_mul_wide(y[q], w));
            }
        } else if (a.is_last) {
#pragma unroll
            for (uint32_t q = 0; q < NE; q++) y[q] = fp_lazy_canon(y[q]);
        }
#pragma unroll
        for (uint32_t q = 0; q < NE; q++)
            if (e0 + q * nthreads < total) fp_store(out_p + idx[q], y[q]);
    }
}

template <bool DP>
__global__ void __launch_bounds__(256, 4) k_ntt_pass8(PassArgs a) {
    constexpr uint32_t B = 8, R = 1u << B, log_c = 2, C = 1u << log_c;
    auto tmul = [](const Fr& x, const Fr& w) -> Fr { return fp_mul_wide(x, w); };
    uint4* t_lo = h2_smem;
    uint4* t_hi = t_lo + (R << log_c);
    uint4* w_lo = t_hi + (R << log_c);
    uint4* w_hi = w_lo + (R >> 1);
    uint4* q_lo = w_hi + (R >> 1);
    uint4* q_hi = q_lo + (R >> 1);
    struct Tw {
        Fr w, q;
    };
    auto tw_get = [&](uint32_t i) __attribute__((always_inline)) -> Tw {
        Tw t;
        t.w = lds_get(w_lo, w_hi, i);
        t.q = lds_get(q_lo, q_hi, i);
        return t;
    };
    auto bmul = [](const Fr& x, const Tw& t) __attribute__((always_inline)) -> Fr { return fp_mul_const(x, t.w, t.q); };
    auto unit4 = [&](Fr& x0, Fr& x1, Fr& x2, Fr& x3, const uint32_t s, const uint32_t r, const bool unit, const Tw* w3 = nullptr) __attribute__((always_inline)) {
        const uint32_t h = 1u << s;
        x0 = fp_lazy_red2p(x0);
        x2 = fp_lazy_red2p(x2);
        if (!unit) {
            const Tw wa = tw_get(r << (B - 1 - s));
            x1 = bmul(x1, wa);
            x3 = bmul(x3, wa);
        } else {
            x1 = fp_lazy_red2p(x1);
            x3 = fp_lazy_red2p(x3);
        }
        const Fr y0 = fp_lazy_add_red(x0, x1), y1 = fp_lazy_sub_red(x0, x1);
        Fr y2 = fp_lazy_add(x2, x3), y3 = fp_lazy_sub(x2, x3);
        y2 = unit ? fp_lazy_red2p(y2) : bmul(y2, tw_get(r << (B - 2 - s)));
        y3 = bmul(y3, w3 ? *w3 : tw_get((r + h) << (B - 2 - s)));
        x0 = fp_lazy_add(y0, y2);
        x1 = fp_lazy_add(y1, y3);
        x2 = fp_lazy_sub(y0, y2);
        x3 = fp_lazy_sub(y1, y3);
    };
    auto unit_of = [](const uint32_t tid, const uint32_t s, uint32_t& i0, uint32_t& r, bool& unit) __attribute__((always_inline)) {
        const uint32_t h = 1u << s, log_per = (B - 2 + log_c) - s;
        const bool by_r = s != 0 && log_per >= 6;
        uint32_t c, p;
        if (by_r) {
            r = tid >> log_per;
            const uint32_t j = tid & ((1u << log_per) - 1);
            c = j & (C - 1);
            p = ((j >> log_c) << (s + 2)) | r;
        } else {
            c = tid & (C - 1);
            const uint32_t b = tid >> log_c;
            r = b & (h - 1);
            p = ((b >> s) << (s + 2)) | r;
        }
        i0 = (p << log_c) + c;
        unit = s == 0 || (by_r && r == 0);
    };
    const uint32_t tid = threadIdx.x;
    auto round4 = [&](const uint32_t s) __attribute__((always_inline)) {
        uint32_t i0, r;
        bool unit;
        unit_of(tid, s, i0, r, unit);
        const uint32_t step = (1u << s) << log_c;
        Fr x0 = lds_get(t_lo, t_hi, i0), x1 = lds_get(t_lo, t_hi, i0 + step);
        Fr x2 = lds_get(t_lo, t_hi, i0 + 2 * step), x3 = lds_get(t_lo, t_hi, i0 + 3 * step);
        unit4(x0, x1, x2, x3, s, r, unit);
        lds_put(t_lo, t_hi, i0, x0);
        lds_put(t_lo, t_hi, i0 + 2 * step, x2);
        lds_put(t_lo, t_hi, i0 + step, x1);
        lds_put(t_lo, t_hi, i0 + 3 * step, x3);
        __syncthreads();
    };
    const bool is_last = DP ? false : a.is_last != 0;
    const uint32_t n_mask = (a.log_n >= 32) ? 0xffffffffu : ((1u << a.log_n) - 1);

    if (tid < (R >> 1)) {
        lds_put(w_lo, w_hi, tid, fp_load(a.tw_bfly + 2 * tid));
        lds_put(q_lo, q_hi, tid, fp_load(a.tw_bfly + 2 * tid + 1));
    }

    Tw tw64;
    tw64.w = fp_load(a.tw_bfly + 2 * (R >> 2));
    tw64.q = fp_load(a.tw_bfly + 2 * (R >> 2) + 1);

    constexpr uint32_t NE = 4;
    {
        const uint32_t tile_id = blockIdx.x;
        const Fr* const in_p = a.batch ? a.in_b[blockIdx.y] : a.in;
        Fr* const out_p = a.batch ? a.out_b[blockIdx.y] : a.out;
        uint32_t base = 0, K_uniform = 0;
        if (!is_last) {
            const uint32_t chunks_per_hi = (1u << a.s_log) >> log_c;
            const uint32_t hi = tile_id / chunks_per_hi, lo0 = (tile_id % chunks_per_hi) << log_c;
            base = (hi << (B + a.s_log)) + lo0;
            K_uniform = hi_to_K(hi, a);
        }

        {
            uint32_t rho[NE], col[NE], idx[NE], Kk[NE];
            Fr x[NE];
#pragma unroll
            for (uint32_t q = 0; q < NE; q++) {
                if (!is_last) {
                    col[q] = tid & (C - 1);
                    rho[q] = bitrev(tid >> log_c, B - 2) + (q << (B - 2));
                    idx[q] = base + (rho[q] << a.s_log) + col[q];
                    Kk[q] = K_uniform;
                } else {
                    rho[q] = (tid & 63) + (q << (B - 2));
                    col[q] = tid >> 6;
                    Kk[q] = (tile_id << log_c) + col[q];
                    idx[q] = (K_to_hi(Kk[q], a) << B) + rho[q];
                }
            }
#pragma unroll
            for (uint32_t q = 0; q < NE; q++) {
                x[q] = fp_zero<FrParams>();
                if (idx[q] < a.in_len) x[q] = fp_load(in_p + idx[q]);
            }
            if (a.has_pre3) {
#pragma unroll
                for (uint32_t q = 0; q < NE; q++) {
                    const uint32_t m = idx[q] % 3;
                    Fr w;
#pragma unroll
                    for (int l = 0; l < 8; l++) w.l[l] = m == 1 ? a.pre3[1].l[l] : a.pre3[2].l[l];
                    if (m != 0) x[q] = tmul(x[q], w);
                }
            }
            const bool pre_scale = a.scale_mode == 1u && a.nprev == 0;
            if (a.nprev != 0 || pre_scale) {
                if (a.tw_direct != nullptr && !pre_scale) {
#pragma unroll
                    for (uint32_t q0 = 0; q0 < NE; q0 += 2) {
                        if constexpr (DP) {
#pragma unroll
                            for (uint32_t q = q0; q < q0 + 2; q++) {
                                const size_t at = a.direct_kmajor ? ((Kk[q] << B) | rho[q]) : ((rho[q] << a.t_log) | Kk[q]);
                                const Fr w = fp_load(a.tw_direct + 2 * at), wq = fp_load(a.tw_direct + 2 * at + 1);
                                x[q] = fp_mul_const(x[q], w, wq);
                            }
                        } else {
                            Fr w[2];
#pragma unroll
                            for (uint32_t q = 0; q < 2; q++)
                                w[q] = fp_load(a.tw_direct + (a.direct_kmajor ? ((Kk[q0 + q] << B) | rho[q0 + q]) : ((rho[q0 + q] << a.t_log) | Kk[q0 + q])));
#pragma unroll
                            for (uint32_t q = 0; q < 2; q++) x[q0 + q] = tmul(x[q0 + q], w[q]);
                        }
                    }
                } else if (a.log_n <= LO_BITS && !pre_scale) {
#pragma unroll
                    for (uint32_t q = 0; q < NE; q++) {
                        const uint32_t ex = (uint32_t)(((uint64_t)rho[q] * Kk[q]) << a.s_log) & n_mask;
                        x[q] = tmul(x[q], fp_load(a.tw_lo + ex));
                    }
                } else {
                    const Fr* const two_lo = pre_scale ? a.sc_lo : a.tw_lo;
                    const Fr* const two_hi = pre_scale ? a.sc_hi : a.tw_hi;
#pragma unroll
                    for (uint32_t q0 = 0; q0 < NE; q0 += 2) {
                        Fr wl[2], wh[2];
#pragma unroll
                        for (uint32_t q = 0; q < 2; q++) {
                            const uint32_t ex = pre_scale ? (idx[q0 + q] & n_mask)
                                                          : ((uint32_t)(((uint64_t)rho[q0 + q] * Kk[q0 + q]) << a.s_log) & n_mask);
                            wl[q] = fp_load(two_lo + (ex & ((1u << LO_BITS) - 1)));
                            wh[q] = fp_load(two_hi + (ex >> LO_BITS));
                        }
#pragma unroll
                        for (uint32_t q = 0; q < 2; q++) x[q0 + q] = tmul(x[q0 + q], fp_mul(wl[q], wh[q]));
                    }
                }
            }
            const uint32_t b = is_last ? bitrev(tid & 63, B - 2) : (tid >> log_c);
            const uint32_t i0 = (b << (2 + log_c)) + (is_last ? (tid >> 6) : (tid & (C - 1)));
            unit4(x[0], x[2], x[1], x[3], 0, 0, true, &tw64);
            lds_put(t_lo, t_hi, i0, x[0]);
            lds_put(t_lo, t_hi, i0 + 2 * C, x[1]);
            lds_put(t_lo, t_hi, i0 + C, x[2]);
            lds_put(t_lo, t_hi, i0 + 3 * C, x[3]);
        }
        __syncthreads();
        round4(2);
        round4(4);

        Fr y[NE];
        {
            uint32_t i0, r;
            bool unit;
            unit_of(tid, 6, i0, r, unit);
#pragma unroll
            for (uint32_t q = 0; q < NE; q++) y[q] = lds_get(t_lo, t_hi, i0 + q * (R << log_c) / NE);
            unit4(y[0], y[1], y[2], y[3], 6, r, unit);
        }
        uint32_t idx[NE];
#pragma unroll
        for (uint32_t q = 0; q < NE; q++) {
            const uint32_t c = tid & (C - 1), k = (tid >> log_c) + q * (R / NE);
            if (!is_last)
                idx[q] = base + (k << a.s_log) + c;
            else
                idx[q] = ((tile_id << log_c) + c) + (k << a.t_log);
        }
        if (is_last && a.scale_mode == 2u) {
#pragma unroll
            for (uint32_t q = 0; q < NE; q++) {
                const uint32_t i = idx[q] & n_mask;
                const Fr w = fp_mul(fp_load(a.sc_lo + (i & ((1u << LO_BITS) - 1))), fp_load(a.sc_hi + (i >> LO_BITS)));
                y[q] = fp_reduce_once(fp_mul_wide(y[q], w));
            }
        } else if (is_last && a.has_post3 && !a.hi_scaled) {
#pragma unroll
            for (uint32_t q = 0; q < NE; q++) {
                const uint32_t m = idx[q] % 3;
                Fr w;
#pragma unroll
                for (int l = 0; l < 8; l++) w.l[l] = m == 0 ? a.post3[0].l[l] : (m == 1 ? a.post3[1].l[l] : a.post3[2].l[l]);
                y[q] = fp_reduce_once(fp_mul_wide(y[q], w));
            }
        } else if (is_last) {
#pragma unroll
            for (uint32_t q = 0; q < NE; q++) y[q] = fp_lazy_canon(y[q]);
        }
#pragma unroll
        for (uint32_t q = 0; q < NE; q++) fp_store(out_p + idx[q], y[q]);
    }
}


struct PassShape {
    uint32_t log_c, threads;
    bool radix4;
    bool fixed;
};
static PassShape pass_shape(uint32_t L, uint32_t B, uint32_t avail) {
// ... 134 lines not shown
        it = ctx->plans.erase(it);
    }
    return bytes;
}

void ntt_free_plans(std::vector<NttPlan*>& gone) {
    if (gone.empty()) return;
    hipError_t e = hipDeviceSynchronize();
    for (NttPlan* pl : gone) free_plan(pl);
    gone.clear();
    H2_HIP(e);
}

size_t ntt_release_plans(DeviceCtx* ctx) {
    std::vector<NttPlan*> gone;
    size_t bytes = ntt_detach_idle_plans(ctx, gone);
    ntt_free_plans(gone);
    return bytes;
}

size_t ntt_plan_bytes(DeviceCtx* ctx) {
    std::lock_guard<std::mutex> g(g_tab_mu);
    size_t bytes = 0;
    for (auto& kv : ctx->plans) {
        NttPlan* pl = kv.second;
        bytes += pl->table_bytes;
        for (auto& t : pl->last_direct) bytes += t.second.bytes;
        bytes += pl->scaled_hi.size() * ((sizeof(Fr) << pl->log_n) >> LO_BITS);
    }
    return bytes;
}

static bool last_table_make_room(DeviceCtx* ctx, size_t need, bool allow_evict) {
    const size_t budget = ntt_table_budget(ctx);
    if (need > budget) return false;
    std::vector<Fr*> gone;
    {
        std::lock_guard<std::mutex> g(g_tab_mu);
        if (!allow_evict) return ctx->ntt_last_table_bytes + need <= budget;
        while (ctx->ntt_last_table_bytes + need > budget) {
            NttPlan::LastTable* victim = nullptr;
            NttPlan* owner = nullptr;
            std::string vkey;
            for (auto& pk : ctx->plans)
                for (auto& kv : pk.second->last_direct)
                    if (kv.second.ptr && kv.second.users == 0 && (!victim || kv.second.last_use < victim->last_use)) {
                        victim = &kv.second;
                        owner = pk.second;
                        vkey = kv.first;
                    }
            if (!victim) break;
            gone.push_back(victim->ptr);
            ctx->ntt_last_table_bytes -= victim->bytes;
            owner->last_direct.erase(vkey);
        }
        if (ctx->ntt_last_table_bytes + need > budget && gone.empty()) return false;
    }
    if (!gone.empty()) {
        H2_HIP(hipDeviceSynchronize());
        for (Fr* t : gone) (void)hipFree(t);
    }
    std::lock_guard<std::mutex> g(g_tab_mu);
    return ctx->ntt_last_table_bytes + need <= budget;
}

struct LastTablePin {
    NttPlan::LastTable* t = nullptr;
    LastTablePin() = default;
    LastTablePin(LastTablePin&& o) noexcept : t(o.t) { o.t = nullptr; }
    LastTablePin& operator=(LastTablePin&& o) noexcept {
        std::swap(t, o.t);
        return *this;
    }
    ~LastTablePin() {
        if (t) {
            std::lock_guard<std::mutex> g(g_tab_mu);
            t->users--;
        }
    }
};

static LastTablePin last_table_pin(DeviceCtx* ctx, NttPlan* pl, uint32_t B, const Fr* d, hipStream_t stream) {
    static const bool last_table = !(getenv("H2_NTT_LAST_TABLE") && atoi(getenv("H2_NTT_LAST_TABLE")) == 0);
    static const uint32_t last_table_max = getenv("H2_NTT_LAST_TABLE_MAX_LOG") ? (uint32_t)atoi(getenv("H2_NTT_LAST_TABLE_MAX_LOG")) : 26u;
    const uint32_t L = pl->log_n;
    LastTablePin pinned;
    if (!last_table || L < 18 || L > last_table_max) return pinned;
    const std::string key = d ? fr_key(*d) : std::string();
    const size_t bytes = sizeof(Fr) << L;
    auto pin = [&]() -> NttPlan::LastTable* {
        auto it = pl->last_direct.find(key);
        if (it == pl->last_direct.end() || it->second.ptr == nullptr) return nullptr;
        it->second.users++;
        it->second.last_use = ++g_tick;
        return &it->second;
    };
    bool may_evict = false;
    {
        std::lock_guard<std::mutex> g(g_tab_mu);
        pinned.t = pin();
        if (!pinned.t) may_evict = ++pl->last_misses[key] >= 2;
    }
    if (pinned.t || !last_table_make_room(ctx, bytes, may_evict)) return pinned;
    Fr* tab = nullptr;
    if (hipMalloc(&tab, bytes) != hipSuccess) {
        (void)hipGetLastError();
        tab = nullptr;
    } else {
        hipLaunchKernelGGL(k_last_table, dim3((1u << L) / 256), dim3(256), 0, stream, tab, pl->w, B, L, d ? *d : pl->w,
                           d ? 1u : 0u, 0u);
        H2_HIP(hipStreamSynchronize(stream));
    }
    Fr* loser = nullptr;
    {
        std::lock_guard<std::mutex> g(g_tab_mu);
        pinned.t = pin();
        if (pinned.t) {
            loser = tab;
        } else if (tab) {
            NttPlan::LastTable& e = pl->last_direct[key];
            e.ptr = tab;
            e.bytes = bytes;
            ctx->ntt_last_table_bytes += bytes;
            pl->last_misses[key] = 0;
            pinned.t = pin();
        }
    }
    if (loser) (void)hipFree(loser);
    return pinned;
}

PlanRef ntt_get_plan(DeviceCtx* ctx, uint32_t log_n, const uint64_t omega[4], hipStream_t stream) {
    std::string key = plan_key(log_n, omega);
    {
        std::lock_guard<std::mutex> g(g_tab_mu);
        auto it = ctx->plans.find(key);
        if (it != ctx->plans.end()) {
            it->second->users.fetch_add(1);
            it->second->last_use = ++g_tick;
            return PlanRef(it->second);
        }
    }

    NttPlan* pl = new NttPlan();
    pl->log_n = log_n;
    ntt_split(log_n, pl->bits);
    Fr w = fr_from_u64x4(omega);
    pl->w = w;
    const uint32_t n = 1u << log_n;
    uint32_t lo_count = n < (1u << LO_BITS) ? n : (1u << LO_BITS);
    uint32_t hi_count = log_n > LO_BITS ? (n >> LO_BITS) : 0;
    size_t total = lo_count + hi_count;
    std::vector<uint32_t> bf_off;
    {
        uint32_t consumed = 0;
        for (size_t p = 0; p < pl->bits.size(); p++) {
            const uint32_t B = pl->bits[p];
            const bool last = p + 1 == pl->bits.size();
            pl->cw.push_back(pass_shape(log_n, B, last ? consumed : log_n - consumed - B).radix4 ? 1 : 0);
            consumed += B;
        }
    }
    for (size_t p = 0; p < pl->bits.size(); p++) {
        const uint32_t b = pl->bits[p];
        bf_off.push_back((uint32_t)total);
        total += ((1u << b) >> 1 ? (1u << b) >> 1 : 1) * (pl->cw[p] ? 2u : 1u);
    }
    H2_HIP(hipMalloc(&pl->tables, total * sizeof(Fr)));
    pl->table_bytes = total * sizeof(Fr);
    pl->tw_lo = pl->tables;
    pl->tw_hi = pl->tables + lo_count;
    hipLaunchKernelGGL(k_pow_table, dim3((lo_count + 255) / 256), dim3(256), 0, stream, pl->tables, w, 1u, lo_count, 0u);
    if (hi_count)
        hipLaunchKernelGGL(k_pow_table, dim3((hi_count + 255) / 256), dim3(256), 0, stream, pl->tables + lo_count, w,
                           1u << LO_BITS, hi_count, 0u);
    for (size_t p = 0; p < pl->bits.size(); p++) {
        uint32_t R = 1u << pl->bits[p], half = R >> 1;
        pl->tw_bfly.push_back(pl->tables + bf_off[p]);
        if (half)
            hipLaunchKernelGGL(k_pow_table, dim3((half + 255) / 256), dim3(256), 0, stream, pl->tables + bf_off[p], w,
                               n >> pl->bits[p], half, (uint32_t)pl->cw[p]);
    }
    {
        uint32_t consumed = 0;
        for (size_t p = 0; p < pl->bits.size(); p++) {
            const uint32_t B = pl->bits[p];
            const bool last = p + 1 == pl->bits.size();
            Fr* tab = nullptr;
            if (p > 0 && !last && B + consumed <= 16) {
                uint32_t cnt = 1u << (B + consumed);
                const size_t tab_bytes = (size_t)cnt * sizeof(Fr) * (pl->cw[p] ? 2 : 1);
                H2_HIP(hipMalloc(&tab, tab_bytes));
                pl->table_bytes += tab_bytes;
                hipLaunchKernelGGL(k_direct_table, dim3((cnt + 255) / 256), dim3(256), 0, stream, tab, w, consumed,
                                   log_n - consumed - B, log_n, cnt, (uint32_t)pl->cw[p]);
            }
            pl->tw_direct.push_back(tab);
            consumed += B;
        }
    }
    H2_HIP(hipGetLastError());
    H2_HIP(hipStreamSynchronize(stream));
    std::lock_guard<std::mutex> g(g_tab_mu);
    auto raced = ctx->plans.find(key);
    if (raced != ctx->plans.end()) {
        free_plan(pl);
        raced->second->users.fetch_add(1);
        raced->second->last_use = ++g_tick;
        return PlanRef(raced->second);
    }
    pl->users.fetch_add(1);
    pl->last_use = ++g_tick;
    ctx->plans[key] = pl;
    return PlanRef(pl);
}

static void set_scale3(PassArgs& a, const Fr* pre3, const Fr* post3) {
    a.has_pre3 = pre3 != nullptr;
    a.has_post3 = post3 != nullptr;
    a.post3_uniform = post3 && fp_eq(post3[0], post3[1]) && fp_eq(post3[0], post3[2]);
    for (int i = 0; i < 3; i++) {
        if (pre3) a.pre3[i] = pre3[i];
        if (post3) a.post3[i] = post3[i];
    }
}

static void ntt_run_chunk(DeviceCtx* ctx, NttPlan* pl, const Fr* const* srcs, Fr* const* dsts, Fr* const* tmps, uint32_t cnt,
                          uint32_t in_len, const Fr* pre3, const Fr* post3, hipStream_t stream, const Fr* scale_tab,
                          uint32_t scale_mode);

ScaleTabRef ntt_scale_table(NttPlan* pl, const Fr& g, const Fr* d, hipStream_t stream) {
    const std::string key = d ? fr_key(g) + '*' + fr_key(*d) : fr_key(g) + '.';
    {
        std::lock_guard<std::mutex> lk(pl->mu);
        auto it = pl->scale_tabs.find(key);
        if (it != pl->scale_tabs.end()) {
            it->second.users++;
            it->second.last_use = ++pl->scale_clock;
            return ScaleTabRef(pl, &it->second);
        }
    }
    const uint32_t n = 1u << pl->log_n;
    const uint32_t lo_count = n < (1u << LO_BITS) ? n : (1u << LO_BITS);
    const uint32_t hi_count = pl->log_n > LO_BITS ? (n >> LO_BITS) : 1u;
    const size_t bytes = ((size_t)(1u << LO_BITS) + hi_count) * sizeof(Fr);
    struct Block {
        Fr* p = nullptr;
        ~Block() {
            if (p) (void)hipFree(p);
        }
    } block;
    H2_HIP(hipMalloc((void**)&block.p, bytes));
    hipLaunchKernelGGL(k_pow_table, dim3((lo_count + 255) / 256), dim3(256), 0, stream, block.p, g, 1u, lo_count, 0u);
    Fr* hi = block.p + (1u << LO_BITS);
    hipLaunchKernelGGL(k_pow_table, dim3((hi_count + 255) / 256), dim3(256), 0, stream, hi, g, 1u << LO_BITS, hi_count, 0u);
    if (d) hipLaunchKernelGGL(k_scale_table, dim3((hi_count + 255) / 256), dim3(256), 0, stream, hi, hi, *d, hi_count);
    H2_HIP(hipGetLastError());
    H2_HIP(hipStreamSynchronize(stream));
    std::vector<Fr*> evicted;
    size_t evicted_bytes = 0;
    NttPlan::ScaleTab* entry = nullptr;
    {
        std::lock_guard<std::mutex> lk(pl->mu);
        auto it = pl->scale_tabs.find(key);
        if (it != pl->scale_tabs.end()) {
            it->second.users++;
            it->second.last_use = ++pl->scale_clock;
            return ScaleTabRef(pl, &it->second);
        }
        while (pl->scale_tabs.size() >= NttPlan::SCALE_TABS_MAX) {
            auto lru = pl->scale_tabs.end();
            for (auto jt = pl->scale_tabs.begin(); jt != pl->scale_tabs.end(); ++jt)
                if (jt->second.users == 0 && (lru == pl->scale_tabs.end() || jt->second.last_use < lru->second.last_use)) lru = jt;
            if (lru == pl->scale_tabs.end()) break;
            evicted.push_back(lru->second.ptr);
            evicted_bytes += lru->second.bytes;
            pl->scale_tabs.erase(lru);
        }
        NttPlan::ScaleTab& e = pl->scale_tabs[key];
        e.ptr = block.p;
        e.bytes = bytes;
        e.users = 1;
        e.last_use = ++pl->scale_clock;
        block.p = nullptr;
        entry = &e;
    }
    {
        std::lock_guard<std::mutex> g2(g_tab_mu);
        pl->table_bytes += bytes;
        pl->table_bytes -= std::min(pl->table_bytes, evicted_bytes);
    }
    for (Fr* q : evicted) (void)hipFree(q);
    return ScaleTabRef(pl, entry);
}

void ntt_run(DeviceCtx* ctx, NttPlan* pl, const Fr* src, Fr* dst, Fr* tmp, uint32_t in_len, const Fr* pre3,
             const Fr* post3, hipStream_t stream, const Fr* scale_tab, uint32_t scale_mode) {
    ntt_run_many(ctx, pl, &src, &dst, &tmp, 1, in_len, pre3, post3, stream, scale_tab, scale_mode);
}

void ntt_run_many(DeviceCtx* ctx, NttPlan* pl, const Fr* const* srcs, Fr* const* dsts, Fr* const* tmps, size_t count,
                  uint32_t in_len, const Fr* pre3, const Fr* post3, hipStream_t stream, const Fr* scale_tab,
                  uint32_t scale_mode) {
    for (size_t c0 = 0; c0 < count; c0 += NTT_BATCH_MAX) {
        const uint32_t cnt = (uint32_t)std::min<size_t>(NTT_BATCH_MAX, count - c0);
        ntt_run_chunk(ctx, pl, srcs + c0, dsts + c0, tmps + c0, cnt, in_len, pre3, post3, stream, scale_tab, scale_mode);
    }
}

static void ntt_run_chunk(DeviceCtx* ctx, NttPlan* pl, const Fr* const* srcs, Fr* const* dsts, Fr* const* tmps, uint32_t cnt,
                          uint32_t in_len, const Fr* pre3, const Fr* post3, hipStream_t stream, const Fr* scale_tab,
                          uint32_t scale_mode) {
    const Fr* const src = srcs[0];
    Fr* const dst = dsts[0];
    Fr* const tmp = tmps[0];
    const uint32_t L = pl->log_n;
    if (L == 0) {
        PassArgs a{};
        a.in = src; a.out = dst; a.tw_bfly = pl->tables; a.tw_lo = pl->tw_lo; a.tw_hi = pl->tw_hi;
        set_scale3(a, pre3, post3); a.log_n = 0; a.B = 0; a.s_log = 0; a.t_log = 0; a.nprev = 0;
        a.is_last = 1; a.in_len = in_len; a.log_c = 0;
        a.sc_lo = scale_tab; a.sc_hi = scale_tab ? scale_tab + (1u << LO_BITS) : nullptr; a.scale_mode = scale_tab ? scale_mode : 0u;
        if (cnt > 1) {
            a.batch = cnt;
            for (uint32_t i = 0; i < cnt; i++) { a.in_b[i] = srcs[i]; a.out_b[i] = dsts[i]; }
        }
        hipLaunchKernelGGL(pass_fn[NK_R2], dim3(1, cnt), dim3(64), 4 * sizeof(Fr), stream, a);
        H2_HIP(hipGetLastError());
        return;
    }
    const size_t P = pl->bits.size();
    Fr* work = (P >= 2) ? tmp : nullptr;
    uint32_t consumed = 0;
    for (size_t p = 0; p < P; p++) {
        PassArgs a{};
        const uint32_t B = pl->bits[p];
        const bool last = (p + 1 == P);
        a.in = (p == 0) ? src : work;
        a.out = last ? dst : work;
        if (cnt > 1) {
            a.batch = cnt;
            for (uint32_t i = 0; i < cnt; i++) {
                Fr* const work_i = (P >= 2) ? tmps[i] : nullptr;
                a.in_b[i] = (p == 0) ? srcs[i] : work_i;
                a.out_b[i] = last ? dsts[i] : work_i;
            }
        }
        a.tw_bfly = pl->tw_bfly[p];
        a.tw_lo = pl->tw_lo;
        a.tw_hi = pl->tw_hi;
        a.tw_direct = pl->tw_direct[p];
        set_scale3(a, (p == 0) ? pre3 : nullptr, last ? post3 : nullptr);
        a.log_n = L;
        a.B = B;
        a.s_log = L - consumed - B;
        a.t_log = consumed;
        a.nprev = (uint32_t)p;
        uint32_t t = 0;
        for (size_t q = 0; q < p; q++) {
            a.prevB[q] = pl->bits[q];
            a.prevT[q] = t;
            t += pl->bits[q];
        }
        a.is_last = last ? 1 : 0;
        a.in_len = (p == 0) ? in_len : (1u << L);
        a.sc_lo = scale_tab;
        a.sc_hi = scale_tab ? scale_tab + (1u << LO_BITS) : nullptr;
        a.scale_mode = (scale_tab && ((scale_mode == 1u && p == 0) || (scale_mode == 2u && last))) ? scale_mode : 0u;
        a.zskip = pass_zskip(L, B, p, last, in_len);
        if (last && p > 0 && a.post3_uniform && L > LO_BITS) {
            const std::string key = fr_key(post3[0]);
            Fr* scaled = nullptr;
            {
                std::lock_guard<std::mutex> g(pl->mu);
                auto it = pl->scaled_hi.find(key);
                if (it == pl->scaled_hi.end()) {
                    uint32_t cnt = (1u << L) >> LO_BITS;
                    H2_HIP(hipMalloc(&scaled, cnt * sizeof(Fr)));
                    hipLaunchKernelGGL(k_scale_table, dim3((cnt + 255) / 256), dim3(256), 0, stream, scaled, pl->tw_hi,
                                       post3[0], cnt);
                    H2_HIP(hipStreamSynchronize(stream));
                    pl->scaled_hi[key] = scaled;
                } else {
                    scaled = it->second;
                }
            }
            a.tw_hi = scaled;
            a.hi_scaled = 1;
        }
        LastTablePin last_tab;
        if (last && p > 0) last_tab = last_table_pin(ctx, pl, B, a.hi_scaled ? &post3[0] : nullptr, stream);
        if (last_tab.t != nullptr) {
            a.tw_direct = last_tab.t->ptr;
            a.direct_kmajor = 1;
        }
        {
            const PassShape sh = pass_shape(L, B, last ? consumed : a.s_log);
            const bool cw = pl->cw[p] != 0;
            a.log_c = sh.log_c;
            a.radix4 = sh.radix4 ? 1u : 0u;
            const uint32_t R = 1u << B, C = 1u << sh.log_c, threads = sh.threads;
            const uint32_t ntiles = (1u << L) / (R * C);
            const size_t lds = cw ? ((size_t)R * C + R) * sizeof(Fr) : ((size_t)R * C + (R >> 1) + 2) * sizeof(Fr);
            if (lds > 64 * 1024) {
                static bool raised[64] = {};
                const int dev = ctx->device;
                if (dev < 0 || dev >= 64 || !raised[dev]) {
                    for (NttKernel k : {NK_R4_DP, NK_R4, NK_R2})
                        H2_HIP(hipFuncSetAttribute((const void*)pass_fn[k], hipFuncAttributeMaxDynamicSharedMemorySize, 160 * 1024));
                    if (dev >= 0 && dev < 64) raised[dev] = true;
                }
            }
            hipLaunchKernelGGL(pass_fn[pass_kernel(sh, a.zskip, last)], dim3(ntiles, cnt), dim3(threads), lds, stream, a);
        }
        consumed += B;
    }
    H2_HIP(hipGetLastError());
}

size_t ntt_shape_query(uint32_t log_n, uint32_t in_log, uint32_t* out, size_t cap) {
    std::vector<uint32_t> bits;
    ntt_split(log_n, bits);
    uint32_t consumed = 0;
    for (size_t p = 0; p < bits.size() && p < cap; p++) {
        const uint32_t B = bits[p];
        const bool last = p + 1 == bits.size();
        const PassShape sh = pass_shape(log_n, B, last ? consumed : log_n - consumed - B);
        const uint32_t zskip = pass_zskip(log_n, B, p, last, 1u << in_log);
        const uint32_t row[7] = {B, sh.log_c, sh.threads, sh.radix4, sh.fixed, zskip, (uint32_t)pass_kernel(sh, zskip, last)};
        for (int i = 0; i < 7; i++) out[7 * p + i] = row[i];
        consumed += B;
    }
    return bits.size();
}

}
```

### halo2-gpu-specific_amd/csrc/ntt.hpp

```cpp
#pragma once
#include <atomic>
#include <vector>

#include "common.hpp"

namespace h2 {

struct NttPlan {
    uint32_t log_n = 0;
    Fr w;
    std::vector<uint32_t> bits;
    Fr* tables = nullptr;
    const Fr* tw_lo = nullptr;
    const Fr* tw_hi = nullptr;
    std::vector<const Fr*> tw_bfly;
    std::vector<const Fr*> tw_direct;
    std::vector<uint8_t> cw;
    size_t table_bytes = 0;
    std::mutex mu;
    std::map<std::string, Fr*> scaled_hi;
    struct ScaleTab {
        Fr* ptr = nullptr;
        size_t bytes = 0;
        uint64_t last_use = 0;
        int users = 0;
    };
    static constexpr size_t SCALE_TABS_MAX = 32;
    std::map<std::string, ScaleTab> scale_tabs;
    uint64_t scale_clock = 0;
    struct LastTable {
        Fr* ptr = nullptr;
        size_t bytes = 0;
        uint64_t last_use = 0;
        int users = 0;
    };
    std::map<std::string, LastTable> last_direct;
    std::map<std::string, int> last_misses;
    std::atomic<int> users{0};
    uint64_t last_use = 0;
};

struct PlanRef {
    NttPlan* pl = nullptr;
    PlanRef() = default;
    explicit PlanRef(NttPlan* p) : pl(p) {}
    PlanRef(PlanRef&& o) noexcept : pl(o.pl) { o.pl = nullptr; }
    PlanRef& operator=(PlanRef&& o) noexcept {
        if (this != &o) {
            if (pl) pl->users.fetch_sub(1);
            pl = o.pl;
            o.pl = nullptr;
        }
        return *this;
    }
    PlanRef(const PlanRef&) = delete;
    PlanRef& operator=(const PlanRef&) = delete;
    ~PlanRef() {
        if (pl) pl->users.fetch_sub(1);
    }
    NttPlan* operator->() const { return pl; }
    NttPlan* get() const { return pl; }
};

void ntt_split(uint32_t log_n, std::vector<uint32_t>& bits);
PlanRef ntt_get_plan(DeviceCtx* ctx, uint32_t log_n, const uint64_t omega[4], hipStream_t stream);
size_t ntt_release_plans(DeviceCtx* ctx);
size_t ntt_detach_idle_plans(DeviceCtx* ctx, std::vector<NttPlan*>& gone);
void ntt_free_plans(std::vector<NttPlan*>& gone);
size_t ntt_plan_bytes(DeviceCtx* ctx);
size_t ntt_table_budget(DeviceCtx* ctx);
void ntt_set_table_budget(size_t bytes);
void ntt_run(DeviceCtx* ctx, NttPlan* pl, const Fr* src, Fr* dst, Fr* tmp, uint32_t in_len, const Fr* pre3,
             const Fr* post3, hipStream_t stream, const Fr* scale_tab = nullptr, uint32_t scale_mode = 0);
struct ScaleTabRef {
    NttPlan* pl = nullptr;
    NttPlan::ScaleTab* tab = nullptr;
    ScaleTabRef() = default;
    ScaleTabRef(NttPlan* p, NttPlan::ScaleTab* t) : pl(p), tab(t) {}
    ScaleTabRef(ScaleTabRef&& o) noexcept : pl(o.pl), tab(o.tab) { o.pl = nullptr; o.tab = nullptr; }
    ScaleTabRef& operator=(ScaleTabRef&& o) noexcept {
        if (this != &o) {
            drop();
            pl = o.pl;
            tab = o.tab;
            o.pl = nullptr;
            o.tab = nullptr;
        }
        return *this;
    }
    ScaleTabRef(const ScaleTabRef&) = delete;
    ScaleTabRef& operator=(const ScaleTabRef&) = delete;
    ~ScaleTabRef() { drop(); }
    const Fr* get() const { return tab ? tab->ptr : nullptr; }
    void drop() {
        if (tab) {
            std::lock_guard<std::mutex> g(pl->mu);
            tab->users--;
        }
        tab = nullptr;
    }
};
ScaleTabRef ntt_scale_table(NttPlan* pl, const Fr& g, const Fr* d, hipStream_t stream);
void ntt_run_many(DeviceCtx* ctx, NttPlan* pl, const Fr* const* srcs, Fr* const* dsts, Fr* const* tmps, size_t count,
                  uint32_t in_len, const Fr* pre3, const Fr* post3, hipStream_t stream, const Fr* scale_tab = nullptr,
                  uint32_t scale_mode = 0);
Fr fr_from_u64x4(const uint64_t v[4]);
size_t ntt_shape_query(uint32_t log_n, uint32_t in_log, uint32_t* out, size_t cap);

}
```

Before: 389.5 billion.

## Use chunked precomputed twiddle tables for constant multiplication in radix-256 NTT pass

Adds a new constant-multiplication form in which each twiddle is expanded into a 2-limb-chunk table (w times powers of 2^64 shifts, precomputed per twiddle), so Montgomery reduction needs only 3 quotient digits instead of 8. Twiddle tables for the fixed-geometry passes are generated in this format. The pass8 kernel loads a subset of them into LDS and reads the last-stage twiddles directly from global memory. This trades a larger twiddle table (4 Fr per twiddle) and more memory or LDS traffic for fewer multiply-adds per butterfly, and it sets a fixed LDS size per launch.

```diff
diff --git a/halo2-gpu-specific_amd/csrc/field.hpp b/halo2-gpu-specific_amd/csrc/field.hpp
--- a/halo2-gpu-specific_amd/csrc/field.hpp
+++ b/halo2-gpu-specific_amd/csrc/field.hpp
@@ -27,6 +27,15 @@
                                         0x7879462eu, 0x666ea36fu, 0x9a07df2fu, 0x0e0a77c1u};
     static constexpr uint32_t RR[8] = {0xae216da7u, 0x1bb8e645u, 0xe35c59e3u, 0x53fe3ab1u,
                                        0x53bb8085u, 0x8c49833du, 0x7f4e44a5u, 0x0216d0b1u};
+    static constexpr uint32_t CHUNK_POW[8][8] = {
+        {0x7c5fb586u, 0xb4c6edf9u, 0xbfeb93beu, 0x708c8d50u, 0x04f7e0efu, 0x9ffd1de4u, 0x9a392866u, 0x215b02acu},
+        {0xaf8b5a7au, 0x54c81065u, 0x97aa45f6u, 0x2b82a1efu, 0x330a5a6du, 0xbe492693u, 0x8229aff4u, 0x1847e486u},
+        {0xef8cfeb9u, 0xb075da81u, 0xa5b6cd8cu, 0xa7f12accu, 0x7957bf7bu, 0x32c47504u, 0x48ffa25eu, 0x03d581d7u},
+        {0xebb7ae00u, 0xee881bd8u, 0x483e9406u, 0x076add9cu, 0x184bf72du, 0xe590c2b8u, 0xff54fbf4u, 0x1df79fc3u},
+        {0xc177f51au, 0x5665c3b5u, 0xde75c713u, 0x00e7f02au, 0x2f747168u, 0xb09192e5u, 0xcccdc65du, 0x0621c0bbu},
+        {0x8f8fc595u, 0x41a9cbe4u, 0x0a58dc0fu, 0x9f36d601u, 0x440ad260u, 0xa6132126u, 0x093f81ddu, 0x2ab23b99u},
+        {0xae216da7u, 0x1bb8e645u, 0xe35c59e3u, 0x53fe3ab1u, 0x53bb8085u, 0x8c49833du, 0x7f4e44a5u, 0x0216d0b1u},
+        {0x04f2bf4fu, 0x6dae765eu, 0xa11298d6u, 0x347d7b17u, 0xf603929eu, 0x70f88a97u, 0x83e5893eu, 0x0ad4bd84u}};
 };
 
 struct FqParams {
@@ -43,6 +52,15 @@
                                         0x7879462cu, 0x666ea36fu, 0x9a07df2fu, 0x0e0a77c1u};
     static constexpr uint32_t RR[8] = {0x538afa89u, 0xf32cfc5bu, 0xd44501fbu, 0xb5e71911u,
                                        0x0a417ff6u, 0x47ab1effu, 0xcab8351fu, 0x06d89f71u};
+    static constexpr uint32_t CHUNK_POW[8][8] = {
+        {0xb1d8c62au, 0x2d9e3b3fu, 0xeb3c74f7u, 0x1be5d753u, 0x5d840e23u, 0x532e2dcfu, 0x9a392864u, 0x215b02acu},
+        {0x8b28a9d6u, 0x0f54b1e8u, 0x492b8e82u, 0xf21d65b8u, 0x91aba3c7u, 0x16d553c6u, 0x355abfe0u, 0x1847e484u},
+        {0x2fcc56eau, 0x70bb1707u, 0x583ff802u, 0xe0e407c3u, 0x9bab3e80u, 0xed7948a3u, 0x1110f1afu, 0x2c1e8d98u},
+        {0xcfc4da46u, 0xcd9e8446u, 0xd3cf3fbcu, 0x608145f0u, 0x74c97a69u, 0x7c85e319u, 0x599e034bu, 0x1798cd75u},
+        {0xcdd22cd6u, 0xd9e291c2u, 0xa40f0271u, 0xc722ccf2u, 0x11a2ac87u, 0xa49e35d6u, 0x8c993ec8u, 0x2e104397u},
+        {0xd86ece59u, 0xa021026fu, 0x6b59411bu, 0xb4c74c43u, 0x4bce7022u, 0xcd5b0ab0u, 0xaef5cf59u, 0x1d7bcfc4u},
+        {0x538afa89u, 0xf32cfc5bu, 0xd44501fbu, 0xb5e71911u, 0x0a417ff6u, 0x47ab1effu, 0xcab8351fu, 0x06d89f71u},
+        {0x83478424u, 0x52592227u, 0x602ec2ddu, 0xd71cacedu, 0xcede48f3u, 0x541fc3cfu, 0x96a02082u, 0x0fc6dd09u}};
 };
 
 template <class P>
@@ -356,6 +374,11 @@
     return fp_reduce_once(fp_lazy_red2p(a));
 }
 
+template <int CL>
+struct alignas(16) FpChunk {
+    uint32_t w[64 / CL];
+};
+
 H2_DEV void mad_acc(uint64_t& lo, uint32_t& hi, uint32_t a, uint32_t b) {
 #if defined(H2_PORTABLE_MUL) || !defined(__HIP_DEVICE_COMPILE__)
     uint64_t p = (uint64_t)a * b;
@@ -379,6 +402,8 @@
 __device__ __forceinline__ Fp<P> fp_mul_wide_dev(const Fp<P>& a, const Fp<P>& b);
 template <class P>
 __device__ __forceinline__ Fp<P> fp_mul_const_dev(const Fp<P>& a, const Fp<P>& w, const Fp<P>& wq);
+template <class P, int CL>
+__device__ __forceinline__ Fp<P> fp_mul_chunk_dev(const Fp<P>& a, const FpChunk<CL>& t);
 #if defined(__HIP_DEVICE_COMPILE__) && !defined(H2_PORTABLE_MUL)
 #include "fp_mul_gen.hpp"
 #endif
@@ -550,6 +575,48 @@
     }
 }
 
+template <int CL, class P>
+H2_DEV Fp<P> fp_mul_chunk(const Fp<P>& x, const FpChunk<CL>& t) {
+#if defined(__HIP_DEVICE_COMPILE__) && !defined(H2_PORTABLE_MUL)
+    return fp_mul_chunk_dev<P, CL>(x, t);
+#else
+    constexpr int NC = 8 / CL, NM = CL + 1;
+    Fp<P> r;
+    uint64_t lo = 0;
+    uint32_t hi = 0;
+    uint32_t m[NM];
+    for (int i = 0; i < NM + 7; i++) {
+        for (int j = 0; j < 8; j++) {
+            const int l = i - j % CL;
+            if (l >= 0 && l <= 7) mad_acc(lo, hi, x.l[j], t.w[l * NC + j / CL]);
+        }
+        for (int j = 0; j < NM && j < i; j++)
+            if (i - j <= 7) mad_acc(lo, hi, m[j], P::MOD[i - j]);
+        if (i < NM) {
+            m[i] = (uint32_t)lo * P::INV;
+            mad_acc(lo, hi, m[i], P::MOD[0]);
+        } else {
+            r.l[i - NM] = (uint32_t)lo;
+        }
+        lo = (lo >> 32) | ((uint64_t)hi << 32);
+        hi = 0;
+    }
+    r.l[7] = (uint32_t)lo;
+    return r;
+#endif
+}
+template <int CL, class P>
+H2_DEV void fp_chunk_table(const Fp<P>& w_mont, FpChunk<CL>& out) {
+    constexpr int NC = 8 / CL;
+    const Fp<P> w_plain = fp_from_mont(w_mont);
+    for (int k = 0; k < NC; k++) {
+        Fp<P> c;
+        for (int l = 0; l < 8; l++) c.l[l] = P::CHUNK_POW[CL * k + CL - 1][l];
+        const Fp<P> t = fp_mul(w_plain, c);
+        for (int l = 0; l < 8; l++) out.w[l * NC + k] = t.l[l];
+    }
+}
+
 template <class P>
 H2_DEV Fp<P> fp_to_mont(const Fp<P>& canon) {
     Fp<P> rr;
diff --git a/halo2-gpu-specific_amd/csrc/fp_mul_gen.hpp b/halo2-gpu-specific_amd/csrc/fp_mul_gen.hpp
--- a/halo2-gpu-specific_amd/csrc/fp_mul_gen.hpp
+++ b/halo2-gpu-specific_amd/csrc/fp_mul_gen.hpp
@@ -1684,6 +1684,224 @@
 }
 
 template <>
+__device__ __forceinline__ Fp<FrParams> fp_mul_chunk_dev<FrParams, 2>(const Fp<FrParams>& a, const FpChunk<2>& t) {
+    using P = FrParams;
+    Fp<P> r;
+    uint64_t lo = 0, cy0, cy1, cy2;
+    uint32_t hi = 0;
+    asm("v_mad_u64_u32 %[lo], %[cy0], %[x0], %[x1], %[lo]\n\t"
+        "v_mad_u64_u32 %[lo], %[cy1], %[x2], %[x3], %[lo]\n\t"
+        "v_mad_u64_u32 %[lo], %[cy2], %[x4], %[x5], %[lo]\n\t"
+        "v_mad_u64_u32 %[lo], %[cy0], %[x6], %[x7], %[lo]\n\t"
+        "v_cndmask_b32 %[hi], 0, 1, %[cy1]\n\t"
+        "v_addc_co_u32 %[hi], %[cy2], %[hi], 0, %[cy2]\n\t"
+        "v_addc_co_u32 %[hi], %[cy0], %[hi], 0, %[cy0]\n\t"
+        : [lo] "+v"(lo), [hi] "=&v"(hi), [cy0] "=&s"(cy0), [cy1] "=&s"(cy1), [cy2] "=&s"(cy2)
+        : [x0] "v"(a.l[0]), [x1] "v"(t.w[0]), [x2] "v"(a.l[2]), [x3] "v"(t.w[1]), [x4] "v"(a.l[4]), [x5] "v"(t.w[2]), [x6] "v"(a.l[6]), [x7] "v"(t.w[3]));
+    const uint32_t m0 = (uint32_t)lo * P::INV;
+    asm("v_mad_u64_u32 %[lo], %[cy0], %[x0], %[x1], %[lo]\n\t"
+        "s_nop 1\n\t"
+        "v_addc_co_u32 %[hi], %[cy0], %[hi], 0, %[cy0]\n\t"
+        : [lo] "+v"(lo), [hi] "+v"(hi), [cy0] "=&s"(cy0)
+        : [x0] "v"(m0), [x1] "s"(P::MOD[0]));
+    lo = (lo >> 32) | ((uint64_t)hi << 32);
+    asm("v_mad_u64_u32 %[lo], %[cy0], %[x0], %[x1], %[lo]\n\t"
+        "v_mad_u64_u32 %[lo], %[cy1], %[x2], %[x3], %[lo]\n\t"
+        "v_mad_u64_u32 %[lo], %[cy2], %[x4], %[x5], %[lo]\n\t"
+        "v_mad_u64_u32 %[lo], %[cy0], %[x6], %[x7], %[lo]\n\t"
+        "v_cndmask_b32 %[hi], 0, 1, %[cy1]\n\t"
+        "v_addc_co_u32 %[hi], %[cy2], %[hi], 0, %[cy2]\n\t"
+        "v_addc_co_u32 %[hi], %[cy0], %[hi], 0, %[cy0]\n\t"
+        "v_mad_u64_u32 %[lo], %[cy1], %[x8], %[x9], %[lo]\n\t"
+        "v_mad_u64_u32 %[lo], %[cy2], %[x10], %[x11], %[lo]\n\t"
+        "v_mad_u64_u32 %[lo], %[cy0], %[x12], %[x13], %[lo]\n\t"
+        "v_addc_co_u32 %[hi], %[cy1], %[hi], 0, %[cy1]\n\t"
+        "v_addc_co_u32 %[hi], %[cy2], %[hi], 0, %[cy2]\n\t"
+        "v_addc_co_u32 %[hi], %[cy0], %[hi], 0, %[cy0]\n\t"
+        "v_mad_u64_u32 %[lo], %[cy1], %[x14], %[x15], %[lo]\n\t"
+        "v_mad_u64_u32 %[lo], %[cy2], %[x16], %[x17], %[lo]\n\t"
+        "s_nop 0\n\t"
+        "v_addc_co_u32 %[hi], %[cy1], %[hi], 0, %[cy1]\n\t"
+        "v_addc_co_u32 %[hi], %[cy2], %[hi], 0, %[cy2]\n\t"
+        : [lo] "+v"(lo), [hi] "=&v"(hi), [cy0] "=&s"(cy0), [cy1] "=&s"(cy1), [cy2] "=&s"(cy2)
+        : [x0] "v"(m0), [x1] "s"(P::MOD[1]), [x2] "v"(a.l[0]), [x3] "v"(t.w[4]), [x4] "v"(a.l[1]), [x5] "v"(t.w[0]), [x6] "v"(a.l[2]), [x7] "v"(t.w[5]), [x8] "v"(a.l[3]), [x9] "v"(t.w[1]), [x10] "v"(a.l[4]), [x11] "v"(t.w[6]), [x12] "v"(a.l[5]), [x13] "v"(t.w[2]), [x14] "v"(a.l[6]), [x15] "v"(t.w[7]), [x16] "v"(a.l[7]), [x17] "v"(t.w[3]));
+    const uint32_t m1 = (uint32_t)lo * P::INV;
+    asm("v_mad_u64_u32 %[lo], %[cy0], %[x0], %[x1], %[lo]\n\t"
+        "s_nop 1\n\t"
+        "v_addc_co_u32 %[hi], %[cy0], %[hi], 0, %[cy0]\n\t"
+        : [lo] "+v"(lo), [hi] "+v"(hi), [cy0] "=&s"(cy0)
+        : [x0] "v"(m1), [x1] "s"(P::MOD[0]));
+    lo = (lo >> 32) | ((uint64_t)hi << 32);
+    asm("v_mad_u64_u32 %[lo], %[cy0], %[x0], %[x1], %[lo]\n\t"
+        "v_mad_u64_u32 %[lo], %[cy1], %[x2], %[x3], %[lo]\n\t"
+        "v_mad_u64_u32 %[lo], %[cy2], %[x4], %[x5], %[lo]\n\t"
+        "v_mad_u64_u32 %[lo], %[cy0], %[x6], %[x7], %[lo]\n\t"
+        "v_mad_u64_u32 %[lo], %[cy1], %[x8], %[x9], %[lo]\n\t"
+        "v_cndmask_b32 %[hi], 0, 1, %[cy2]\n\t"
+        "v_addc_co_u32 %[hi], %[cy0], %[hi], 0, %[cy0]\n\t"
+        "v_addc_co_u32 %[hi], %[cy1], %[hi], 0, %[cy1]\n\t"
+        "v_mad_u64_u32 %[lo], %[cy2], %[x10], %[x11], %[lo]\n\t"
+        "v_mad_u64_u32 %[lo], %[cy0], %[x12], %[x13], %[lo]\n\t"
+        "v_mad_u64_u32 %[lo], %[cy1], %[x14], %[x15], %[lo]\n\t"
+        "v_addc_co_u32 %[hi], %[cy2], %[hi], 0, %[cy2]\n\t"
+        "v_addc_co_u32 %[hi], %[cy0], %[hi], 0, %[cy0]\n\t"
+        "v_addc_co_u32 %[hi], %[cy1], %[hi], 0, %[cy1]\n\t"
+        "v_mad_u64_u32 %[lo], %[cy2], %[x16], %[x17], %[lo]\n\t"
+        "v_mad_u64_u32 %[lo], %[cy0], %[x18], %[x19], %[lo]\n\t"
+        "s_nop 0\n\t"
+        "v_addc_co_u32 %[hi], %[cy2], %[hi], 0, %[cy2]\n\t"
+        "v_addc_co_u32 %[hi], %[cy0], %[hi], 0, %[cy0]\n\t"
+        : [lo] "+v"(lo), [hi] "=&v"(hi), [cy0] "=&s"(cy0), [cy1] "=&s"(cy1), [cy2] "=&s"(cy2)
+        : [x0] "v"(m1), [x1] "s"(P::MOD[1]), [x2] "v"(m0), [x3] "s"(P::MOD[2]), [x4] "v"(a.l[0]), [x5] "v"(t.w[8]), [x6] "v"(a.l[1]), [x7] "v"(t.w[4]), [x8] "v"(a.l[2]), [x9] "v"(t.w[9]), [x10] "v"(a.l[3]), [x11] "v"(t.w[5]), [x12] "v"(a.l[4]), [x13] "v"(t.w[10]), [x14] "v"(a.l[5]), [x15] "v"(t.w[6]), [x16] "v"(a.l[6]), [x17] "v"(t.w[11]), [x18] "v"(a.l[7]), [x19] "v"(t.w[7]));
+    const uint32_t m2 = (uint32_t)lo * P::INV;
+    asm("v_mad_u64_u32 %[lo], %[cy0], %[x0], %[x1], %[lo]\n\t"
+        "s_nop 1\n\t"
+        "v_addc_co_u32 %[hi], %[cy0], %[hi], 0, %[cy0]\n\t"
+        : [lo] "+v"(lo), [hi] "+v"(hi), [cy0] "=&s"(cy0)
+        : [x0] "v"(m2), [x1] "s"(P::MOD[0]));
+    lo = (lo >> 32) | ((uint64_t)hi << 32);
+    asm("v_mad_u64_u32 %[lo], %[cy0], %[x0], %[x1], %[lo]\n\t"
+        "v_mad_u64_u32 %[lo], %[cy1], %[x2], %[x3], %[lo]\n\t"
+        "v_mad_u64_u32 %[lo], %[cy2], %[x4], %[x5], %[lo]\n\t"
+        "v_mad_u64_u32 %[lo], %[cy0], %[x6], %[x7], %[lo]\n\t"
+        "v_mad_u64_u32 %[lo], %[cy1], %[x8], %[x9], %[lo]\n\t"
+        "v_mad_u64_u32 %[lo], %[cy2], %[x10], %[x11], %[lo]\n\t"
+        "v_cndmask_b32 %[hi], 0, 1, %[cy0]\n\t"
+        "v_addc_co_u32 %[hi], %[cy1], %[hi], 0, %[cy1]\n\t"
+        "v_addc_co_u32 %[hi], %[cy2], %[hi], 0, %[cy2]\n\t"
+        "v_mad_u64_u32 %[lo], %[cy0], %[x12], %[x13], %[lo]\n\t"
+        "v_mad_u64_u32 %[lo], %[cy1], %[x14], %[x15], %[lo]\n\t"
+        "v_mad_u64_u32 %[lo], %[cy2], %[x16], %[x17], %[lo]\n\t"
+        "v_addc_co_u32 %[hi], %[cy0], %[hi], 0, %[cy0]\n\t"
+        "v_addc_co_u32 %[hi], %[cy1], %[hi], 0, %[cy1]\n\t"
+        "v_addc_co_u32 %[hi], %[cy2], %[hi], 0, %[cy2]\n\t"
+        "v_mad_u64_u32 %[lo], %[cy0], %[x18], %[x19], %[lo]\n\t"
+        "v_mad_u64_u32 %[lo], %[cy1], %[x20], %[x21], %[lo]\n\t"
+        "s_nop 0\n\t"
+        "v_addc_co_u32 %[hi], %[cy0], %[hi], 0, %[cy0]\n\t"
+        "v_addc_co_u32 %[hi], %[cy1], %[hi], 0, %[cy1]\n\t"
+        : [lo] "+v"(lo), [hi] "=&v"(hi), [cy0] "=&s"(cy0), [cy1] "=&s"(cy1), [cy2] "=&s"(cy2)
+        : [x0] "v"(m0), [x1] "s"(P::MOD[3]), [x2] "v"(m2), [x3] "s"(P::MOD[1]), [x4] "v"(m1), [x5] "s"(P::MOD[2]), [x6] "v"(a.l[0]), [x7] "v"(t.w[12]), [x8] "v"(a.l[1]), [x9] "v"(t.w[8]), [x10] "v"(a.l[2]), [x11] "v"(t.w[13]), [x12] "v"(a.l[3]), [x13] "v"(t.w[9]), [x14] "v"(a.l[4]), [x15] "v"(t.w[14]), [x16] "v"(a.l[5]), [x17] "v"(t.w[10]), [x18] "v"(a.l[6]), [x19] "v"(t.w[15]), [x20] "v"(a.l[7]), [x21] "v"(t.w[11]));
+    r.l[0] = (uint32_t)lo;
+    lo = (lo >> 32) | ((uint64_t)hi << 32);
+    asm("v_mad_u64_u32 %[lo], %[cy0], %[x0], %[x1], %[lo]\n\t"
+        "v_mad_u64_u32 %[lo], %[cy1], %[x2], %[x3], %[lo]\n\t"
+        "v_mad_u64_u32 %[lo], %[cy2], %[x4], %[x5], %[lo]\n\t"
+        "v_mad_u64_u32 %[lo], %[cy0], %[x6], %[x7], %[lo]\n\t"
+        "v_mad_u64_u32 %[lo], %[cy1], %[x8], %[x9], %[lo]\n\t"
+        "v_cndmask_b32 %[hi], 0, 1, %[cy2]\n\t"
+        "v_addc_co_u32 %[hi], %[cy0], %[hi], 0, %[cy0]\n\t"
+        "v_addc_co_u32 %[hi], %[cy1], %[hi], 0, %[cy1]\n\t"
+        "v_mad_u64_u32 %[lo], %[cy2], %[x10], %[x11], %[lo]\n\t"
+        "v_mad_u64_u32 %[lo], %[cy0], %[x12], %[x13], %[lo]\n\t"
+        "v_mad_u64_u32 %[lo], %[cy1], %[x14], %[x15], %[lo]\n\t"
+        "v_addc_co_u32 %[hi], %[cy2], %[hi], 0, %[cy2]\n\t"
+        "v_addc_co_u32 %[hi], %[cy0], %[hi], 0, %[cy0]\n\t"
+        "v_addc_co_u32 %[hi], %[cy1], %[hi], 0, %[cy1]\n\t"
+        "v_mad_u64_u32 %[lo], %[cy2], %[x16], %[x17], %[lo]\n\t"
+        "v_mad_u64_u32 %[lo], %[cy0], %[x18], %[x19], %[lo]\n\t"
+        "v_mad_u64_u32 %[lo], %[cy1], %[x20], %[x21], %[lo]\n\t"
+        "v_addc_co_u32 %[hi], %[cy2], %[hi], 0, %[cy2]\n\t"
+        "v_addc_co_u32 %[hi], %[cy0], %[hi], 0, %[cy0]\n\t"
+        "v_addc_co_u32 %[hi], %[cy1], %[hi], 0, %[cy1]\n\t"
+        : [lo] "+v"(lo), [hi] "=&v"(hi), [cy0] "=&s"(cy0), [cy1] "=&s"(cy1), [cy2] "=&s"(cy2)
+        : [x0] "v"(m1), [x1] "s"(P::MOD[3]), [x2] "v"(m2), [x3] "s"(P::MOD[2]), [x4] "v"(m0), [x5] "s"(P::MOD[4]), [x6] "v"(a.l[0]), [x7] "v"(t.w[16]), [x8] "v"(a.l[1]), [x9] "v"(t.w[12]), [x10] "v"(a.l[2]), [x11] "v"(t.w[17]), [x12] "v"(a.l[3]), [x13] "v"(t.w[13]), [x14] "v"(a.l[4]), [x15] "v"(t.w[18]), [x16] "v"(a.l[5]), [x17] "v"(t.w[14]), [x18] "v"(a.l[6]), [x19] "v"(t.w[19]), [x20] "v"(a.l[7]), [x21] "v"(t.w[15]));
+    r.l[1] = (uint32_t)lo;
+    lo = (lo >> 32) | ((uint64_t)hi << 32);
+    asm("v_mad_u64_u32 %[lo], %[cy0], %[x0], %[x1], %[lo]\n\t"
+        "v_mad_u64_u32 %[lo], %[cy1], %[x2], %[x3], %[lo]\n\t"
+        "v_mad_u64_u32 %[lo], %[cy2], %[x4], %[x5], %[lo]\n\t"
+        "v_mad_u64_u32 %[lo], %[cy0], %[x6], %[x7], %[lo]\n\t"
+        "v_mad_u64_u32 %[lo], %[cy1], %[x8], %[x9], %[lo]\n\t"
+        "v_cndmask_b32 %[hi], 0, 1, %[cy2]\n\t"
+        "v_addc_co_u32 %[hi], %[cy0], %[hi], 0, %[cy0]\n\t"
+        "v_addc_co_u32 %[hi], %[cy1], %[hi], 0, %[cy1]\n\t"
+        "v_mad_u64_u32 %[lo], %[cy2], %[x10], %[x11], %[lo]\n\t"
+        "v_mad_u64_u32 %[lo], %[cy0], %[x12], %[x13], %[lo]\n\t"
+        "v_mad_u64_u32 %[lo], %[cy1], %[x14], %[x15], %[lo]\n\t"
+        "v_addc_co_u32 %[hi], %[cy2], %[hi], 0, %[cy2]\n\t"
+        "v_addc_co_u32 %[hi], %[cy0], %[hi], 0, %[cy0]\n\t"
+        "v_addc_co_u32 %[hi], %[cy1], %[hi], 0, %[cy1]\n\t"
+        "v_mad_u64_u32 %[lo], %[cy2], %[x16], %[x17], %[lo]\n\t"
+        "v_mad_u64_u32 %[lo], %[cy0], %[x18], %[x19], %[lo]\n\t"
+        "v_mad_u64_u32 %[lo], %[cy1], %[x20], %[x21], %[lo]\n\t"
+        "v_addc_co_u32 %[hi], %[cy2], %[hi], 0, %[cy2]\n\t"
+        "v_addc_co_u32 %[hi], %[cy0], %[hi], 0, %[cy0]\n\t"
+        "v_addc_co_u32 %[hi], %[cy1], %[hi], 0, %[cy1]\n\t"
+        : [lo] "+v"(lo), [hi] "=&v"(hi), [cy0] "=&s"(cy0), [cy1] "=&s"(cy1), [cy2] "=&s"(cy2)
+        : [x0] "v"(m2), [x1] "s"(P::MOD[3]), [x2] "v"(m1), [x3] "s"(P::MOD[4]), [x4] "v"(m0), [x5] "s"(P::MOD[5]), [x6] "v"(a.l[0]), [x7] "v"(t.w[20]), [x8] "v"(a.l[1]), [x9] "v"(t.w[16]), [x10] "v"(a.l[2]), [x11] "v"(t.w[21]), [x12] "v"(a.l[3]), [x13] "v"(t.w[17]), [x14] "v"(a.l[4]), [x15] "v"(t.w[22]), [x16] "v"(a.l[5]), [x17] "v"(t.w[18]), [x18] "v"(a.l[6]), [x19] "v"(t.w[23]), [x20] "v"(a.l[7]), [x21] "v"(t.w[19]));
+    r.l[2] = (uint32_t)lo;
+    lo = (lo >> 32) | ((uint64_t)hi << 32);
+    asm("v_mad_u64_u32 %[lo], %[cy0], %[x0], %[x1], %[lo]\n\t"
+        "v_mad_u64_u32 %[lo], %[cy1], %[x2], %[x3], %[lo]\n\t"
+        "v_mad_u64_u32 %[lo], %[cy2], %[x4], %[x5], %[lo]\n\t"
+        "v_mad_u64_u32 %[lo], %[cy0], %[x6], %[x7], %[lo]\n\t"
+        "v_cndmask_b32 %[hi], 0, 1, %[cy1]\n\t"
+        "v_addc_co_u32 %[hi], %[cy2], %[hi], 0, %[cy2]\n\t"
+        "v_addc_co_u32 %[hi], %[cy0], %[hi], 0, %[cy0]\n\t"
+        "v_mad_u64_u32 %[lo], %[cy1], %[x8], %[x9], %[lo]\n\t"
+        "v_mad_u64_u32 %[lo], %[cy2], %[x10], %[x11], %[lo]\n\t"
+        "v_mad_u64_u32 %[lo], %[cy0], %[x12], %[x13], %[lo]\n\t"
+        "v_addc_co_u32 %[hi], %[cy1], %[hi], 0, %[cy1]\n\t"
+        "v_addc_co_u32 %[hi], %[cy2], %[hi], 0, %[cy2]\n\t"
+        "v_addc_co_u32 %[hi], %[cy0], %[hi], 0, %[cy0]\n\t"
+        "v_mad_u64_u32 %[lo], %[cy1], %[x14], %[x15], %[lo]\n\t"
+        "v_mad_u64_u32 %[lo], %[cy2], %[x16], %[x17], %[lo]\n\t"
+        "v_mad_u64_u32 %[lo], %[cy0], %[x18], %[x19], %[lo]\n\t"
+        "v_addc_co_u32 %[hi], %[cy1], %[hi], 0, %[cy1]\n\t"
+        "v_addc_co_u32 %[hi], %[cy2], %[hi], 0, %[cy2]\n\t"
+        "v_addc_co_u32 %[hi], %[cy0], %[hi], 0, %[cy0]\n\t"
+        "v_mad_u64_u32 %[lo], %[cy1], %[x20], %[x21], %[lo]\n\t"
+        "s_nop 1\n\t"
+        "v_addc_co_u32 %[hi], %[cy1], %[hi], 0, %[cy1]\n\t"
+        : [lo] "+v"(lo), [hi] "=&v"(hi), [cy0] "=&s"(cy0), [cy1] "=&s"(cy1), [cy2] "=&s"(cy2)
+        : [x0] "v"(m2), [x1] "s"(P::MOD[4]), [x2] "v"(m1), [x3] "s"(P::MOD[5]), [x4] "v"(m0), [x5] "s"(P::MOD[6]), [x6] "v"(a.l[0]), [x7] "v"(t.w[24]), [x8] "v"(a.l[1]), [x9] "v"(t.w[20]), [x10] "v"(a.l[2]), [x11] "v"(t.w[25]), [x12] "v"(a.l[3]), [x13] "v"(t.w[21]), [x14] "v"(a.l[4]), [x15] "v"(t.w[26]), [x16] "v"(a.l[5]), [x17] "v"(t.w[22]), [x18] "v"(a.l[6]), [x19] "v"(t.w[27]), [x20] "v"(a.l[7]), [x21] "v"(t.w[23]));
+    r.l[3] = (uint32_t)lo;
+    lo = (lo >> 32) | ((uint64_t)hi << 32);
+    asm("v_mad_u64_u32 %[lo], %[cy0], %[x0], %[x1], %[lo]\n\t"
+        "v_mad_u64_u32 %[lo], %[cy1], %[x2], %[x3], %[lo]\n\t"
+        "v_mad_u64_u32 %[lo], %[cy2], %[x4], %[x5], %[lo]\n\t"
+        "v_mad_u64_u32 %[lo], %[cy0], %[x6], %[x7], %[lo]\n\t"
+        "v_mad_u64_u32 %[lo], %[cy1], %[x8], %[x9], %[lo]\n\t"
+        "v_mad_u64_u32 %[lo], %[cy2], %[x10], %[x11], %[lo]\n\t"
+        "v_mad_u64_u32 %[lo], %[cy0], %[x12], %[x13], %[lo]\n\t"
+        "v_mad_u64_u32 %[lo], %[cy1], %[x14], %[x15], %[lo]\n\t"
+        "v_cndmask_b32 %[hi], 0, 1, %[cy2]\n\t"
+        "v_addc_co_u32 %[hi], %[cy0], %[hi], 0, %[cy0]\n\t"
+        "v_addc_co_u32 %[hi], %[cy1], %[hi], 0, %[cy1]\n\t"
+        "v_mad_u64_u32 %[lo], %[cy2], %[x16], %[x17], %[lo]\n\t"
+        "v_mad_u64_u32 %[lo], %[cy0], %[x18], %[x19], %[lo]\n\t"
+        "v_mad_u64_u32 %[lo], %[cy1], %[x20], %[x21], %[lo]\n\t"
+        "v_addc_co_u32 %[hi], %[cy2], %[hi], 0, %[cy2]\n\t"
+        "v_addc_co_u32 %[hi], %[cy0], %[hi], 0, %[cy0]\n\t"
+        "v_addc_co_u32 %[hi], %[cy1], %[hi], 0, %[cy1]\n\t"
+        : [lo] "+v"(lo), [hi] "=&v"(hi), [cy0] "=&s"(cy0), [cy1] "=&s"(cy1), [cy2] "=&s"(cy2)
+        : [x0] "v"(a.l[0]), [x1] "v"(t.w[28]), [x2] "v"(a.l[2]), [x3] "v"(t.w[29]), [x4] "v"(a.l[4]), [x5] "v"(t.w[30]), [x6] "v"(a.l[6]), [x7] "v"(t.w[31]), [x8] "v"(m0), [x9] "s"(P::MOD[7]), [x10] "v"(m2), [x11] "s"(P::MOD[5]), [x12] "v"(m1), [x13] "s"(P::MOD[6]), [x14] "v"(a.l[1]), [x15] "v"(t.w[24]), [x16] "v"(a.l[3]), [x17] "v"(t.w[25]), [x18] "v"(a.l[5]), [x19] "v"(t.w[26]), [x20] "v"(a.l[7]), [x21] "v"(t.w[27]));
+    r.l[4] = (uint32_t)lo;
+    lo = (lo >> 32) | ((uint64_t)hi << 32);
+    asm("v_mad_u64_u32 %[lo], %[cy0], %[x0], %[x1], %[lo]\n\t"
+        "v_mad_u64_u32 %[lo], %[cy1], %[x2], %[x3], %[lo]\n\t"
+        "v_mad_u64_u32 %[lo], %[cy2], %[x4], %[x5], %[lo]\n\t"
+        "v_mad_u64_u32 %[lo], %[cy0], %[x6], %[x7], %[lo]\n\t"
+        "v_mad_u64_u32 %[lo], %[cy1], %[x8], %[x9], %[lo]\n\t"
+        "v_mad_u64_u32 %[lo], %[cy2], %[x10], %[x11], %[lo]\n\t"
+        "s_nop 1\n\t"
+        "v_cndmask_b32 %[hi], 0, 1, %[cy2]\n\t"
+        : [lo] "+v"(lo), [hi] "=&v"(hi), [cy0] "=&s"(cy0), [cy1] "=&s"(cy1), [cy2] "=&s"(cy2)
+        : [x0] "v"(a.l[1]), [x1] "v"(t.w[28]), [x2] "v"(a.l[3]), [x3] "v"(t.w[29]), [x4] "v"(a.l[5]), [x5] "v"(t.w[30]), [x6] "v"(a.l[7]), [x7] "v"(t.w[31]), [x8] "v"(m1), [x9] "s"(P::MOD[7]), [x10] "v"(m2), [x11] "s"(P::MOD[6]));
+    r.l[5] = (uint32_t)lo;
+    lo = (lo >> 32) | ((uint64_t)hi << 32);
+    asm("v_mad_u64_u32 %[lo], %[cy0], %[x0], %[x1], %[lo]\n\t"
+        : [lo] "+v"(lo), [cy0] "=&s"(cy0)
+        : [x0] "v"(m2), [x1] "s"(P::MOD[7]));
+    r.l[6] = (uint32_t)lo;
+    lo >>= 32;
+    r.l[7] = (uint32_t)lo;
+    (void)cy0; (void)cy1; (void)cy2; (void)hi;
+    return r;
+}
+
+template <>
 __device__ __forceinline__ Fp<FqParams> fp_mul_dev<FqParams>(const Fp<FqParams>& a, const Fp<FqParams>& b) {
     using P = FqParams;
     Fp<P> r;
@@ -3388,3 +3606,223 @@
     (void)cy0; (void)cy1; (void)cy2; (void)hi;
     return r;
 }
+
+template <>
+__device__ __forceinline__ Fp<FqParams> fp_mul_chunk_dev<FqParams, 2>(const Fp<FqParams>& a, const FpChunk<2>& t) {
+    using P = FqParams;
+    Fp<P> r;
+    uint64_t lo = 0, cy0, cy1, cy2;
+    uint32_t hi = 0;
+    asm("v_mad_u64_u32 %[lo], %[cy0], %[x0], %[x1], %[lo]\n\t"
+        "v_mad_u64_u32 %[lo], %[cy1], %[x2], %[x3], %[lo]\n\t"
+        "v_mad_u64_u32 %[lo], %[cy2], %[x4], %[x5], %[lo]\n\t"
+        "v_mad_u64_u32 %[lo], %[cy0], %[x6], %[x7], %[lo]\n\t"
+        "v_cndmask_b32 %[hi], 0, 1, %[cy1]\n\t"
+        "v_addc_co_u32 %[hi], %[cy2], %[hi], 0, %[cy2]\n\t"
+        "v_addc_co_u32 %[hi], %[cy0], %[hi], 0, %[cy0]\n\t"
+        : [lo] "+v"(lo), [hi] "=&v"(hi), [cy0] "=&s"(cy0), [cy1] "=&s"(cy1), [cy2] "=&s"(cy2)
+        : [x0] "v"(a.l[0]), [x1] "v"(t.w[0]), [x2] "v"(a.l[2]), [x3] "v"(t.w[1]), [x4] "v"(a.l[4]), [x5] "v"(t.w[2]), [x6] "v"(a.l[6]), [x7] "v"(t.w[3]));
+    const uint32_t m0 = (uint32_t)lo * P::INV;
+    asm("v_mad_u64_u32 %[lo], %[cy0], %[x0], %[x1], %[lo]\n\t"
+        "s_nop 1\n\t"
+        "v_addc_co_u32 %[hi], %[cy0], %[hi], 0, %[cy0]\n\t"
+        : [lo] "+v"(lo), [hi] "+v"(hi), [cy0] "=&s"(cy0)
+        : [x0] "v"(m0), [x1] "s"(P::MOD[0]));
+    lo = (lo >> 32) | ((uint64_t)hi << 32);
+    asm("v_mad_u64_u32 %[lo], %[cy0], %[x0], %[x1], %[lo]\n\t"
+        "v_mad_u64_u32 %[lo], %[cy1], %[x2], %[x3], %[lo]\n\t"
+        "v_mad_u64_u32 %[lo], %[cy2], %[x4], %[x5], %[lo]\n\t"
+        "v_mad_u64_u32 %[lo], %[cy0], %[x6], %[x7], %[lo]\n\t"
+        "v_cndmask_b32 %[hi], 0, 1, %[cy1]\n\t"
+        "v_addc_co_u32 %[hi], %[cy2], %[hi], 0, %[cy2]\n\t"
+        "v_addc_co_u32 %[hi], %[cy0], %[hi], 0, %[cy0]\n\t"
+        "v_mad_u64_u32 %[lo], %[cy1], %[x8], %[x9], %[lo]\n\t"
+        "v_mad_u64_u32 %[lo], %[cy2], %[x10], %[x11], %[lo]\n\t"
+        "v_mad_u64_u32 %[lo], %[cy0], %[x12], %[x13], %[lo]\n\t"
+        "v_addc_co_u32 %[hi], %[cy1], %[hi], 0, %[cy1]\n\t"
+        "v_addc_co_u32 %[hi], %[cy2], %[hi], 0, %[cy2]\n\t"
+        "v_addc_co_u32 %[hi], %[cy0], %[hi], 0, %[cy0]\n\t"
+        "v_mad_u64_u32 %[lo], %[cy1], %[x14], %[x15], %[lo]\n\t"
+        "v_mad_u64_u32 %[lo], %[cy2], %[x16], %[x17], %[lo]\n\t"
+        "s_nop 0\n\t"
+        "v_addc_co_u32 %[hi], %[cy1], %[hi], 0, %[cy1]\n\t"
+        "v_addc_co_u32 %[hi], %[cy2], %[hi], 0, %[cy2]\n\t"
+        : [lo] "+v"(lo), [hi] "=&v"(hi), [cy0] "=&s"(cy0), [cy1] "=&s"(cy1), [cy2] "=&s"(cy2)
+        : [x0] "v"(m0), [x1] "s"(P::MOD[1]), [x2] "v"(a.l[0]), [x3] "v"(t.w[4]), [x4] "v"(a.l[1]), [x5] "v"(t.w[0]), [x6] "v"(a.l[2]), [x7] "v"(t.w[5]), [x8] "v"(a.l[3]), [x9] "v"(t.w[1]), [x10] "v"(a.l[4]), [x11] "v"(t.w[6]), [x12] "v"(a.l[5]), [x13] "v"(t.w[2]), [x14] "v"(a.l[6]), [x15] "v"(t.w[7]), [x16] "v"(a.l[7]), [x17] "v"(t.w[3]));
+    const uint32_t m1 = (uint32_t)lo * P::INV;
+    asm("v_mad_u64_u32 %[lo], %[cy0], %[x0], %[x1], %[lo]\n\t"
+        "s_nop 1\n\t"
+        "v_addc_co_u32 %[hi], %[cy0], %[hi], 0, %[cy0]\n\t"
+        : [lo] "+v"(lo), [hi] "+v"(hi), [cy0] "=&s"(cy0)
+        : [x0] "v"(m1), [x1] "s"(P::MOD[0]));
+    lo = (lo >> 32) | ((uint64_t)hi << 32);
+    asm("v_mad_u64_u32 %[lo], %[cy0], %[x0], %[x1], %[lo]\n\t"
+        "v_mad_u64_u32 %[lo], %[cy1], %[x2], %[x3], %[lo]\n\t"
+        "v_mad_u64_u32 %[lo], %[cy2], %[x4], %[x5], %[lo]\n\t"
+        "v_mad_u64_u32 %[lo], %[cy0], %[x6], %[x7], %[lo]\n\t"
+        "v_mad_u64_u32 %[lo], %[cy1], %[x8], %[x9], %[lo]\n\t"
+        "v_cndmask_b32 %[hi], 0, 1, %[cy2]\n\t"
+        "v_addc_co_u32 %[hi], %[cy0], %[hi], 0, %[cy0]\n\t"
+        "v_addc_co_u32 %[hi], %[cy1], %[hi], 0, %[cy1]\n\t"
+        "v_mad_u64_u32 %[lo], %[cy2], %[x10], %[x11], %[lo]\n\t"
+        "v_mad_u64_u32 %[lo], %[cy0], %[x12], %[x13], %[lo]\n\t"
+        "v_mad_u64_u32 %[lo], %[cy1], %[x14], %[x15], %[lo]\n\t"
+        "v_addc_co_u32 %[hi], %[cy2], %[hi], 0, %[cy2]\n\t"
+        "v_addc_co_u32 %[hi], %[cy0], %[hi], 0, %[cy0]\n\t"
+        "v_addc_co_u32 %[hi], %[cy1], %[hi], 0, %[cy1]\n\t"
+        "v_mad_u64_u32 %[lo], %[cy2], %[x16], %[x17], %[lo]\n\t"
+        "v_mad_u64_u32 %[lo], %[cy0], %[x18], %[x19], %[lo]\n\t"
+        "s_nop 0\n\t"
+        "v_addc_co_u32 %[hi], %[cy2], %[hi], 0, %[cy2]\n\t"
+        "v_addc_co_u32 %[hi], %[cy0], %[hi], 0, %[cy0]\n\t"
+        : [lo] "+v"(lo), [hi] "=&v"(hi), [cy0] "=&s"(cy0), [cy1] "=&s"(cy1), [cy2] "=&s"(cy2)
+        : [x0] "v"(m1), [x1] "s"(P::MOD[1]), [x2] "v"(m0), [x3] "s"(P::MOD[2]), [x4] "v"(a.l[0]), [x5] "v"(t.w[8]), [x6] "v"(a.l[1]), [x7] "v"(t.w[4]), [x8] "v"(a.l[2]), [x9] "v"(t.w[9]), [x10] "v"(a.l[3]), [x11] "v"(t.w[5]), [x12] "v"(a.l[4]), [x13] "v"(t.w[10]), [x14] "v"(a.l[5]), [x15] "v"(t.w[6]), [x16] "v"(a.l[6]), [x17] "v"(t.w[11]), [x18] "v"(a.l[7]), [x19] "v"(t.w[7]));
+    const uint32_t m2 = (uint32_t)lo * P::INV;
+    asm("v_mad_u64_u32 %[lo], %[cy0], %[x0], %[x1], %[lo]\n\t"
+        "s_nop 1\n\t"
+        "v_addc_co_u32 %[hi], %[cy0], %[hi], 0, %[cy0]\n\t"
+        : [lo] "+v"(lo), [hi] "+v"(hi), [cy0] "=&s"(cy0)
+        : [x0] "v"(m2), [x1] "s"(P::MOD[0]));
+    lo = (lo >> 32) | ((uint64_t)hi << 32);
+    asm("v_mad_u64_u32 %[lo], %[cy0], %[x0], %[x1], %[lo]\n\t"
+        "v_mad_u64_u32 %[lo], %[cy1], %[x2], %[x3], %[lo]\n\t"
+        "v_mad_u64_u32 %[lo], %[cy2], %[x4], %[x5], %[lo]\n\t"
+        "v_mad_u64_u32 %[lo], %[cy0], %[x6], %[x7], %[lo]\n\t"
+        "v_mad_u64_u32 %[lo], %[cy1], %[x8], %[x9], %[lo]\n\t"
+        "v_cndmask_b32 %[hi], 0, 1, %[cy2]\n\t"
+        "v_addc_co_u32 %[hi], %[cy0], %[hi], 0, %[cy0]\n\t"
+        "v_addc_co_u32 %[hi], %[cy1], %[hi], 0, %[cy1]\n\t"
+        "v_mad_u64_u32 %[lo], %[cy2], %[x10], %[x11], %[lo]\n\t"
+        "v_mad_u64_u32 %[lo], %[cy0], %[x12], %[x13], %[lo]\n\t"
+        "v_mad_u64_u32 %[lo], %[cy1], %[x14], %[x15], %[lo]\n\t"
+        "v_addc_co_u32 %[hi], %[cy2], %[hi], 0, %[cy2]\n\t"
+        "v_addc_co_u32 %[hi], %[cy0], %[hi], 0, %[cy0]\n\t"
+        "v_addc_co_u32 %[hi], %[cy1], %[hi], 0, %[cy1]\n\t"
+        "v_mad_u64_u32 %[lo], %[cy2], %[x16], %[x17], %[lo]\n\t"
+        "v_mad_u64_u32 %[lo], %[cy0], %[x18], %[x19], %[lo]\n\t"
+        "v_mad_u64_u32 %[lo], %[cy1], %[x20], %[x21], %[lo]\n\t"
+        "v_addc_co_u32 %[hi], %[cy2], %[hi], 0, %[cy2]\n\t"
+        "v_addc_co_u32 %[hi], %[cy0], %[hi], 0, %[cy0]\n\t"
+        "v_addc_co_u32 %[hi], %[cy1], %[hi], 0, %[cy1]\n\t"
+        : [lo] "+v"(lo), [hi] "=&v"(hi), [cy0] "=&s"(cy0), [cy1] "=&s"(cy1), [cy2] "=&s"(cy2)
+        : [x0] "v"(m2), [x1] "s"(P::MOD[1]), [x2] "v"(m1), [x3] "s"(P::MOD[2]), [x4] "v"(m0), [x5] "s"(P::MOD[3]), [x6] "v"(a.l[0]), [x7] "v"(t.w[12]), [x8] "v"(a.l[1]), [x9] "v"(t.w[8]), [x10] "v"(a.l[2]), [x11] "v"(t.w[13]), [x12] "v"(a.l[3]), [x13] "v"(t.w[9]), [x14] "v"(a.l[4]), [x15] "v"(t.w[14]), [x16] "v"(a.l[5]), [x17] "v"(t.w[10]), [x18] "v"(a.l[6]), [x19] "v"(t.w[15]), [x20] "v"(a.l[7]), [x21] "v"(t.w[11]));
+    r.l[0] = (uint32_t)lo;
+    lo = (lo >> 32) | ((uint64_t)hi << 32);
+    asm("v_mad_u64_u32 %[lo], %[cy0], %[x0], %[x1], %[lo]\n\t"
+        "v_mad_u64_u32 %[lo], %[cy1], %[x2], %[x3], %[lo]\n\t"
+        "v_mad_u64_u32 %[lo], %[cy2], %[x4], %[x5], %[lo]\n\t"
+        "v_mad_u64_u32 %[lo], %[cy0], %[x6], %[x7], %[lo]\n\t"
+        "v_mad_u64_u32 %[lo], %[cy1], %[x8], %[x9], %[lo]\n\t"
+        "v_cndmask_b32 %[hi], 0, 1, %[cy2]\n\t"
+        "v_addc_co_u32 %[hi], %[cy0], %[hi], 0, %[cy0]\n\t"
+        "v_addc_co_u32 %[hi], %[cy1], %[hi], 0, %[cy1]\n\t"
+        "v_mad_u64_u32 %[lo], %[cy2], %[x10], %[x11], %[lo]\n\t"
+        "v_mad_u64_u32 %[lo], %[cy0], %[x12], %[x13], %[lo]\n\t"
+        "v_mad_u64_u32 %[lo], %[cy1], %[x14], %[x15], %[lo]\n\t"
+        "v_addc_co_u32 %[hi], %[cy2], %[hi], 0, %[cy2]\n\t"
+        "v_addc_co_u32 %[hi], %[cy0], %[hi], 0, %[cy0]\n\t"
+        "v_addc_co_u32 %[hi], %[cy1], %[hi], 0, %[cy1]\n\t"
+        "v_mad_u64_u32 %[lo], %[cy2], %[x16], %[x17], %[lo]\n\t"
+        "v_mad_u64_u32 %[lo], %[cy0], %[x18], %[x19], %[lo]\n\t"
+        "v_mad_u64_u32 %[lo], %[cy1], %[x20], %[x21], %[lo]\n\t"
+        "v_addc_co_u32 %[hi], %[cy2], %[hi], 0, %[cy2]\n\t"
+        "v_addc_co_u32 %[hi], %[cy0], %[hi], 0, %[cy0]\n\t"
+        "v_addc_co_u32 %[hi], %[cy1], %[hi], 0, %[cy1]\n\t"
+        : [lo] "+v"(lo), [hi] "=&v"(hi), [cy0] "=&s"(cy0), [cy1] "=&s"(cy1), [cy2] "=&s"(cy2)
+        : [x0] "v"(m2), [x1] "s"(P::MOD[2]), [x2] "v"(m0), [x3] "s"(P::MOD[4]), [x4] "v"(m1), [x5] "s"(P::MOD[3]), [x6] "v"(a.l[0]), [x7] "v"(t.w[16]), [x8] "v"(a.l[1]), [x9] "v"(t.w[12]), [x10] "v"(a.l[2]), [x11] "v"(t.w[17]), [x12] "v"(a.l[3]), [x13] "v"(t.w[13]), [x14] "v"(a.l[4]), [x15] "v"(t.w[18]), [x16] "v"(a.l[5]), [x17] "v"(t.w[14]), [x18] "v"(a.l[6]), [x19] "v"(t.w[19]), [x20] "v"(a.l[7]), [x21] "v"(t.w[15]));
+    r.l[1] = (uint32_t)lo;
+    lo = (lo >> 32) | ((uint64_t)hi << 32);
+    asm("v_mad_u64_u32 %[lo], %[cy0], %[x0], %[x1], %[lo]\n\t"
+        "v_mad_u64_u32 %[lo], %[cy1], %[x2], %[x3], %[lo]\n\t"
+        "v_mad_u64_u32 %[lo], %[cy2], %[x4], %[x5], %[lo]\n\t"
+        "v_mad_u64_u32 %[lo], %[cy0], %[x6], %[x7], %[lo]\n\t"
+        "v_cndmask_b32 %[hi], 0, 1, %[cy1]\n\t"
+        "v_addc_co_u32 %[hi], %[cy2], %[hi], 0, %[cy2]\n\t"
+        "v_addc_co_u32 %[hi], %[cy0], %[hi], 0, %[cy0]\n\t"
+        "v_mad_u64_u32 %[lo], %[cy1], %[x8], %[x9], %[lo]\n\t"
+        "v_mad_u64_u32 %[lo], %[cy2], %[x10], %[x11], %[lo]\n\t"
+        "v_mad_u64_u32 %[lo], %[cy0], %[x12], %[x13], %[lo]\n\t"
+        "v_addc_co_u32 %[hi], %[cy1], %[hi], 0, %[cy1]\n\t"
+        "v_addc_co_u32 %[hi], %[cy2], %[hi], 0, %[cy2]\n\t"
+        "v_addc_co_u32 %[hi], %[cy0], %[hi], 0, %[cy0]\n\t"
+        "v_mad_u64_u32 %[lo], %[cy1], %[x14], %[x15], %[lo]\n\t"
+        "v_mad_u64_u32 %[lo], %[cy2], %[x16], %[x17], %[lo]\n\t"
+        "v_mad_u64_u32 %[lo], %[cy0], %[x18], %[x19], %[lo]\n\t"
+        "v_addc_co_u32 %[hi], %[cy1], %[hi], 0, %[cy1]\n\t"
+        "v_addc_co_u32 %[hi], %[cy2], %[hi], 0, %[cy2]\n\t"
+        "v_addc_co_u32 %[hi], %[cy0], %[hi], 0, %[cy0]\n\t"
+        "v_mad_u64_u32 %[lo], %[cy1], %[x20], %[x21], %[lo]\n\t"
+        "s_nop 1\n\t"
+        "v_addc_co_u32 %[hi], %[cy1], %[hi], 0, %[cy1]\n\t"
+        : [lo] "+v"(lo), [hi] "=&v"(hi), [cy0] "=&s"(cy0), [cy1] "=&s"(cy1), [cy2] "=&s"(cy2)
+        : [x0] "v"(m1), [x1] "s"(P::MOD[4]), [x2] "v"(m2), [x3] "s"(P::MOD[3]), [x4] "v"(m0), [x5] "s"(P::MOD[5]), [x6] "v"(a.l[0]), [x7] "v"(t.w[20]), [x8] "v"(a.l[1]), [x9] "v"(t.w[16]), [x10] "v"(a.l[2]), [x11] "v"(t.w[21]), [x12] "v"(a.l[3]), [x13] "v"(t.w[17]), [x14] "v"(a.l[4]), [x15] "v"(t.w[22]), [x16] "v"(a.l[5]), [x17] "v"(t.w[18]), [x18] "v"(a.l[6]), [x19] "v"(t.w[23]), [x20] "v"(a.l[7]), [x21] "v"(t.w[19]));
+    r.l[2] = (uint32_t)lo;
+    lo = (lo >> 32) | ((uint64_t)hi << 32);
+    asm("v_mad_u64_u32 %[lo], %[cy0], %[x0], %[x1], %[lo]\n\t"
+        "v_mad_u64_u32 %[lo], %[cy1], %[x2], %[x3], %[lo]\n\t"
+        "v_mad_u64_u32 %[lo], %[cy2], %[x4], %[x5], %[lo]\n\t"
+        "v_mad_u64_u32 %[lo], %[cy0], %[x6], %[x7], %[lo]\n\t"
+        "v_cndmask_b32 %[hi], 0, 1, %[cy1]\n\t"
+        "v_addc_co_u32 %[hi], %[cy2], %[hi], 0, %[cy2]\n\t"
+        "v_addc_co_u32 %[hi], %[cy0], %[hi], 0, %[cy0]\n\t"
+        "v_mad_u64_u32 %[lo], %[cy1], %[x8], %[x9], %[lo]\n\t"
+        "v_mad_u64_u32 %[lo], %[cy2], %[x10], %[x11], %[lo]\n\t"
+        "v_mad_u64_u32 %[lo], %[cy0], %[x12], %[x13], %[lo]\n\t"
+        "v_addc_co_u32 %[hi], %[cy1], %[hi], 0, %[cy1]\n\t"
+        "v_addc_co_u32 %[hi], %[cy2], %[hi], 0, %[cy2]\n\t"
+        "v_addc_co_u32 %[hi], %[cy0], %[hi], 0, %[cy0]\n\t"
+        "v_mad_u64_u32 %[lo], %[cy1], %[x14], %[x15], %[lo]\n\t"
+        "v_mad_u64_u32 %[lo], %[cy2], %[x16], %[x17], %[lo]\n\t"
+        "v_mad_u64_u32 %[lo], %[cy0], %[x18], %[x19], %[lo]\n\t"
+        "v_addc_co_u32 %[hi], %[cy1], %[hi], 0, %[cy1]\n\t"
+        "v_addc_co_u32 %[hi], %[cy2], %[hi], 0, %[cy2]\n\t"
+        "v_addc_co_u32 %[hi], %[cy0], %[hi], 0, %[cy0]\n\t"
+        "v_mad_u64_u32 %[lo], %[cy1], %[x20], %[x21], %[lo]\n\t"
+        "s_nop 1\n\t"
+        "v_addc_co_u32 %[hi], %[cy1], %[hi], 0, %[cy1]\n\t"
+        : [lo] "+v"(lo), [hi] "=&v"(hi), [cy0] "=&s"(cy0), [cy1] "=&s"(cy1), [cy2] "=&s"(cy2)
+        : [x0] "v"(m2), [x1] "s"(P::MOD[4]), [x2] "v"(m1), [x3] "s"(P::MOD[5]), [x4] "v"(m0), [x5] "s"(P::MOD[6]), [x6] "v"(a.l[0]), [x7] "v"(t.w[24]), [x8] "v"(a.l[1]), [x9] "v"(t.w[20]), [x10] "v"(a.l[2]), [x11] "v"(t.w[25]), [x12] "v"(a.l[3]), [x13] "v"(t.w[21]), [x14] "v"(a.l[4]), [x15] "v"(t.w[26]), [x16] "v"(a.l[5]), [x17] "v"(t.w[22]), [x18] "v"(a.l[6]), [x19] "v"(t.w[27]), [x20] "v"(a.l[7]), [x21] "v"(t.w[23]));
+    r.l[3] = (uint32_t)lo;
+    lo = (lo >> 32) | ((uint64_t)hi << 32);
+    asm("v_mad_u64_u32 %[lo], %[cy0], %[x0], %[x1], %[lo]\n\t"
+        "v_mad_u64_u32 %[lo], %[cy1], %[x2], %[x3], %[lo]\n\t"
+        "v_mad_u64_u32 %[lo], %[cy2], %[x4], %[x5], %[lo]\n\t"
+        "v_mad_u64_u32 %[lo], %[cy0], %[x6], %[x7], %[lo]\n\t"
+        "v_mad_u64_u32 %[lo], %[cy1], %[x8], %[x9], %[lo]\n\t"
+        "v_mad_u64_u32 %[lo], %[cy2], %[x10], %[x11], %[lo]\n\t"
+        "v_mad_u64_u32 %[lo], %[cy0], %[x12], %[x13], %[lo]\n\t"
+        "v_mad_u64_u32 %[lo], %[cy1], %[x14], %[x15], %[lo]\n\t"
+        "v_cndmask_b32 %[hi], 0, 1, %[cy2]\n\t"
+        "v_addc_co_u32 %[hi], %[cy0], %[hi], 0, %[cy0]\n\t"
+        "v_addc_co_u32 %[hi], %[cy1], %[hi], 0, %[cy1]\n\t"
+        "v_mad_u64_u32 %[lo], %[cy2], %[x16], %[x17], %[lo]\n\t"
+        "v_mad_u64_u32 %[lo], %[cy0], %[x18], %[x19], %[lo]\n\t"
+        "v_mad_u64_u32 %[lo], %[cy1], %[x20], %[x21], %[lo]\n\t"
+        "v_addc_co_u32 %[hi], %[cy2], %[hi], 0, %[cy2]\n\t"
+        "v_addc_co_u32 %[hi], %[cy0], %[hi], 0, %[cy0]\n\t"
+        "v_addc_co_u32 %[hi], %[cy1], %[hi], 0, %[cy1]\n\t"
+        : [lo] "+v"(lo), [hi] "=&v"(hi), [cy0] "=&s"(cy0), [cy1] "=&s"(cy1), [cy2] "=&s"(cy2)
+        : [x0] "v"(a.l[0]), [x1] "v"(t.w[28]), [x2] "v"(a.l[2]), [x3] "v"(t.w[29]), [x4] "v"(a.l[4]), [x5] "v"(t.w[30]), [x6] "v"(a.l[6]), [x7] "v"(t.w[31]), [x8] "v"(m0), [x9] "s"(P::MOD[7]), [x10] "v"(m2), [x11] "s"(P::MOD[5]), [x12] "v"(m1), [x13] "s"(P::MOD[6]), [x14] "v"(a.l[1]), [x15] "v"(t.w[24]), [x16] "v"(a.l[3]), [x17] "v"(t.w[25]), [x18] "v"(a.l[5]), [x19] "v"(t.w[26]), [x20] "v"(a.l[7]), [x21] "v"(t.w[27]));
+    r.l[4] = (uint32_t)lo;
+    lo = (lo >> 32) | ((uint64_t)hi << 32);
+    asm("v_mad_u64_u32 %[lo], %[cy0], %[x0], %[x1], %[lo]\n\t"
+        "v_mad_u64_u32 %[lo], %[cy1], %[x2], %[x3], %[lo]\n\t"
+        "v_mad_u64_u32 %[lo], %[cy2], %[x4], %[x5], %[lo]\n\t"
+        "v_mad_u64_u32 %[lo], %[cy0], %[x6], %[x7], %[lo]\n\t"
+        "v_mad_u64_u32 %[lo], %[cy1], %[x8], %[x9], %[lo]\n\t"
+        "v_mad_u64_u32 %[lo], %[cy2], %[x10], %[x11], %[lo]\n\t"
+        "s_nop 1\n\t"
+        "v_cndmask_b32 %[hi], 0, 1, %[cy2]\n\t"
+        : [lo] "+v"(lo), [hi] "=&v"(hi), [cy0] "=&s"(cy0), [cy1] "=&s"(cy1), [cy2] "=&s"(cy2)
+        : [x0] "v"(a.l[1]), [x1] "v"(t.w[28]), [x2] "v"(a.l[3]), [x3] "v"(t.w[29]), [x4] "v"(a.l[5]), [x5] "v"(t.w[30]), [x6] "v"(a.l[7]), [x7] "v"(t.w[31]), [x8] "v"(m1), [x9] "s"(P::MOD[7]), [x10] "v"(m2), [x11] "s"(P::MOD[6]));
+    r.l[5] = (uint32_t)lo;
+    lo = (lo >> 32) | ((uint64_t)hi << 32);
+    asm("v_mad_u64_u32 %[lo], %[cy0], %[x0], %[x1], %[lo]\n\t"
+        : [lo] "+v"(lo), [cy0] "=&s"(cy0)
+        : [x0] "v"(m2), [x1] "s"(P::MOD[7]));
+    r.l[6] = (uint32_t)lo;
+    lo >>= 32;
+    r.l[7] = (uint32_t)lo;
+    (void)cy0; (void)cy1; (void)cy2; (void)hi;
+    return r;
+}
diff --git a/halo2-gpu-specific_amd/csrc/ntt.hip b/halo2-gpu-specific_amd/csrc/ntt.hip
--- a/halo2-gpu-specific_amd/csrc/ntt.hip
+++ b/halo2-gpu-specific_amd/csrc/ntt.hip
@@ -9,9 +9,20 @@
 static constexpr int NTT_BATCH_MAX = 16;
 static constexpr int LO_BITS = 12;
 
+using TwChunk = FpChunk<2>;
+static constexpr uint32_t TW_CHUNK_FR = sizeof(TwChunk) / sizeof(Fr);
+static constexpr uint32_t TW_CHUNK_Q = sizeof(TwChunk) / sizeof(uint4);
 __device__ __forceinline__ void tw_store(Fr* out, uint32_t i, const Fr& w_mont, uint32_t pair) {
     if (!pair) {
         fp_store(out + i, w_mont);
+        return;
+    }
+    if (pair == 2) {
+        TwChunk t;
+        fp_chunk_table(w_mont, t);
+        uint4* const q = reinterpret_cast<uint4*>(out) + (size_t)i * TW_CHUNK_Q;
+#pragma unroll
+        for (uint32_t k = 0; k < TW_CHUNK_Q; k++) q[k] = make_uint4(t.w[4 * k], t.w[4 * k + 1], t.w[4 * k + 2], t.w[4 * k + 3]);
         return;
     }
     Fr w, q;
@@ -54,6 +65,7 @@
     const Fr* in;
     Fr* out;
     const Fr* tw_bfly;
+    const Fr* tw_chunk;
     const Fr* tw_lo;
     const Fr* tw_hi;
     const Fr* tw_direct;
@@ -384,32 +396,37 @@
     }
 }
 
+static constexpr uint32_t PASS8_TW_LDS = 32;
+static constexpr uint32_t PASS8_LDS = ((256u << 2) * 2 + PASS8_TW_LDS * TW_CHUNK_Q) * sizeof(uint4);
+static_assert(4 * PASS8_LDS <= 160u * 1024, "four workgroups of k_ntt_pass8 per CU");
 template <bool DP>
 __global__ void __launch_bounds__(256, 4) k_ntt_pass8(PassArgs a) {
     constexpr uint32_t B = 8, R = 1u << B, log_c = 2, C = 1u << log_c;
     auto tmul = [](const Fr& x, const Fr& w) -> Fr { return fp_mul_wide(x, w); };
     uint4* t_lo = h2_smem;
     uint4* t_hi = t_lo + (R << log_c);
-    uint4* w_lo = t_hi + (R << log_c);
-    uint4* w_hi = w_lo + (R >> 1);
-    uint4* q_lo = w_hi + (R >> 1);
-    uint4* q_hi = q_lo + (R >> 1);
-    struct Tw {
-        Fr w, q;
+    uint4* w_pl = t_hi + (R << log_c);
+    const uint4* const tw_tab = reinterpret_cast<const uint4*>(a.tw_chunk);
+    using Tw = TwChunk;
+    auto tw_unpack = [](Tw& t, const uint32_t k, const uint4 v) __attribute__((always_inline)) {
+        t.w[4 * k] = v.x; t.w[4 * k + 1] = v.y; t.w[4 * k + 2] = v.z; t.w[4 * k + 3] = v.w;
     };
-    auto tw_get = [&](uint32_t i) __attribute__((always_inline)) -> Tw {
+    static_assert((R >> 1) / PASS8_TW_LDS == 4, "the stage pairs before the last read the indices that are multiples of 4");
+    auto tw_get = [&](const uint32_t i, const bool mem) __attribute__((always_inline)) -> Tw {
         Tw t;
-        t.w = lds_get(w_lo, w_hi, i);
-        t.q = lds_get(q_lo, q_hi, i);
+#pragma unroll
+        for (uint32_t k = 0; k < TW_CHUNK_Q; k++)
+            tw_unpack(t, k, mem ? tw_tab[(size_t)i * TW_CHUNK_Q + k] : w_pl[k * PASS8_TW_LDS + (i >> 2)]);
         return t;
     };
-    auto bmul = [](const Fr& x, const Tw& t) __attribute__((always_inline)) -> Fr { return fp_mul_const(x, t.w, t.q); };
+    auto bmul = [](const Fr& x, const Tw& t) __attribute__((always_inline)) -> Fr { return fp_mul_chunk(x, t); };
     auto unit4 = [&](Fr& x0, Fr& x1, Fr& x2, Fr& x3, const uint32_t s, const uint32_t r, const bool unit, const Tw* w3 = nullptr) __attribute__((always_inline)) {
         const uint32_t h = 1u << s;
+        const bool mem = s == B - 2;
         x0 = fp_lazy_red2p(x0);
         x2 = fp_lazy_red2p(x2);
         if (!unit) {
-            const Tw wa = tw_get(r << (B - 1 - s));
+            const Tw wa = tw_get(r << (B - 1 - s), mem);
             x1 = bmul(x1, wa);
             x3 = bmul(x3, wa);
         } else {
@@ -418,8 +435,8 @@
         }
         const Fr y0 = fp_lazy_add_red(x0, x1), y1 = fp_lazy_sub_red(x0, x1);
         Fr y2 = fp_lazy_add(x2, x3), y3 = fp_lazy_sub(x2, x3);
-        y2 = unit ? fp_lazy_red2p(y2) : bmul(y2, tw_get(r << (B - 2 - s)));
-        y3 = bmul(y3, w3 ? *w3 : tw_get((r + h) << (B - 2 - s)));
+        y2 = unit ? fp_lazy_red2p(y2) : bmul(y2, tw_get(r << (B - 2 - s), mem));
+        y3 = bmul(y3, w3 ? *w3 : tw_get((r + h) << (B - 2 - s), mem));
         x0 = fp_lazy_add(y0, y2);
         x1 = fp_lazy_add(y1, y3);
         x2 = fp_lazy_sub(y0, y2);
@@ -461,14 +478,13 @@
     const bool is_last = DP ? false : a.is_last != 0;
     const uint32_t n_mask = (a.log_n >= 32) ? 0xffffffffu : ((1u << a.log_n) - 1);
 
-    if (tid < (R >> 1)) {
-        lds_put(w_lo, w_hi, tid, fp_load(a.tw_bfly + 2 * tid));
-        lds_put(q_lo, q_hi, tid, fp_load(a.tw_bfly + 2 * tid + 1));
-    }
+#pragma unroll
+    for (uint32_t g = tid; g < PASS8_TW_LDS * TW_CHUNK_Q; g += 256)
+        w_pl[(g % TW_CHUNK_Q) * PASS8_TW_LDS + g / TW_CHUNK_Q] = tw_tab[(size_t)(g / TW_CHUNK_Q) * 4 * TW_CHUNK_Q + g % TW_CHUNK_Q];
 
     Tw tw64;
-    tw64.w = fp_load(a.tw_bfly + 2 * (R >> 2));
-    tw64.q = fp_load(a.tw_bfly + 2 * (R >> 2) + 1);
+#pragma unroll
+    for (uint32_t k = 0; k < TW_CHUNK_Q; k++) tw_unpack(tw64, k, tw_tab[(R >> 2) * TW_CHUNK_Q + k]);
 
     constexpr uint32_t NE = 4;
     {
@@ -909,19 +925,25 @@
     uint32_t hi_count = log_n > LO_BITS ? (n >> LO_BITS) : 0;
     size_t total = lo_count + hi_count;
     std::vector<uint32_t> bf_off;
+    std::vector<uint8_t> fixed_geom;
     {
         uint32_t consumed = 0;
         for (size_t p = 0; p < pl->bits.size(); p++) {
             const uint32_t B = pl->bits[p];
             const bool last = p + 1 == pl->bits.size();
-            pl->cw.push_back(pass_shape(log_n, B, last ? consumed : log_n - consumed - B).radix4 ? 1 : 0);
+            const PassShape sh = pass_shape(log_n, B, last ? consumed : log_n - consumed - B);
+            pl->cw.push_back(sh.radix4 ? 1 : 0);
+            fixed_geom.push_back(sh.fixed ? 1 : 0);
             consumed += B;
         }
     }
+    std::vector<uint32_t> ch_off;
     for (size_t p = 0; p < pl->bits.size(); p++) {
         const uint32_t b = pl->bits[p];
         bf_off.push_back((uint32_t)total);
         total += ((1u << b) >> 1 ? (1u << b) >> 1 : 1) * (pl->cw[p] ? 2u : 1u);
+        ch_off.push_back(fixed_geom[p] ? (uint32_t)total : 0u);
+        if (fixed_geom[p]) total += ((1u << b) >> 1) * TW_CHUNK_FR;
     }
     H2_HIP(hipMalloc(&pl->tables, total * sizeof(Fr)));
     pl->table_bytes = total * sizeof(Fr);
@@ -937,6 +959,10 @@
         if (half)
             hipLaunchKernelGGL(k_pow_table, dim3((half + 255) / 256), dim3(256), 0, stream, pl->tables + bf_off[p], w,
                                n >> pl->bits[p], half, (uint32_t)pl->cw[p]);
+        pl->tw_chunk.push_back(ch_off[p] ? pl->tables + ch_off[p] : nullptr);
+        if (ch_off[p])
+            hipLaunchKernelGGL(k_pow_table, dim3((half + 255) / 256), dim3(256), 0, stream, pl->tables + ch_off[p], w,
+                               n >> pl->bits[p], half, 2u);
     }
     {
         uint32_t consumed = 0;
@@ -1104,6 +1130,7 @@
             }
         }
         a.tw_bfly = pl->tw_bfly[p];
+        a.tw_chunk = pl->tw_chunk[p];
         a.tw_lo = pl->tw_lo;
         a.tw_hi = pl->tw_hi;
         a.tw_direct = pl->tw_direct[p];
@@ -1168,7 +1195,9 @@
                     if (dev >= 0 && dev < 64) raised[dev] = true;
                 }
             }
-            hipLaunchKernelGGL(pass_fn[pass_kernel(sh, a.zskip, last)], dim3(ntiles, cnt), dim3(threads), lds, stream, a);
+            const NttKernel kernel = pass_kernel(sh, a.zskip, last);
+            const bool pass8 = kernel == NK_PASS8_DP || kernel == NK_PASS8;
+            hipLaunchKernelGGL(pass_fn[kernel], dim3(ntiles, cnt), dim3(threads), pass8 ? (size_t)PASS8_LDS : lds, stream, a);
         }
         consumed += B;
     }
diff --git a/halo2-gpu-specific_amd/csrc/ntt.hpp b/halo2-gpu-specific_amd/csrc/ntt.hpp
--- a/halo2-gpu-specific_amd/csrc/ntt.hpp
+++ b/halo2-gpu-specific_amd/csrc/ntt.hpp
@@ -14,6 +14,7 @@
     const Fr* tw_lo = nullptr;
     const Fr* tw_hi = nullptr;
     std::vector<const Fr*> tw_bfly;
+    std::vector<const Fr*> tw_chunk;
     std::vector<const Fr*> tw_direct;
     std::vector<uint8_t> cw;
     size_t table_bytes = 0;
```

Measured after the change: 417.8 billion (median of 6 runs). 1.07x the previous value.
